# robo-alex/gs-dynamics

Measured on AMD Instinct MI355X. Metric: fwd+bwd Mpix/s at 100k Gaussians, 4x800^2 views, higher is better.
Workload: dtype f32

## Files before the change

### gs-dynamics_amd/csrc/gsr_api.hip

```cpp
#include <atomic>
#include <chrono>
#include <sched.h>
#include <stdarg.h>
#include <stdio.h>
#include <string.h>
#include <vector>
#include "gsr_common.h"

static thread_local char g_err[512] = "";

namespace {
struct ProfRec { const char* name; hipEvent_t a, b; };
bool g_prof_on = false;
std::vector<ProfRec> g_prof;
}
#include <dlfcn.h>
namespace {
typedef int (*roctx_push_fn)(const char*);
typedef int (*roctx_pop_fn)(void);
roctx_push_fn g_roctx_push = nullptr;
roctx_pop_fn g_roctx_pop = nullptr;
bool roctx_ready() {
  static const bool ok = [] {
    const char* e = getenv("GSR_ROCTX");
    if (e && *e && atoi(e) == 0) return false;
    for (const char* lib : {"librocprofiler-sdk-roctx.so", "librocprofiler-sdk-roctx.so.1", "libroctx64.so", "libroctx64.so.4"}) {
      void* h = dlopen(lib, RTLD_LAZY | RTLD_GLOBAL);
      if (!h) continue;
      g_roctx_push = (roctx_push_fn)dlsym(h, "roctxRangePushA");
      g_roctx_pop = (roctx_pop_fn)dlsym(h, "roctxRangePop");
      if (g_roctx_push && g_roctx_pop) return true;
    }
    return false;
  }();
  return ok;
}
}
GsrRange::GsrRange(const char* name) : on(roctx_ready()) { if (on) g_roctx_push(name); }
GsrRange::~GsrRange() { if (on) g_roctx_pop(); }

GsrProfScope::GsrProfScope(const char* name, hipStream_t s) : slot(-1), st(s), range(name) {
  if (!g_prof_on) return;
  ProfRec r; r.name = name;
  if (hipEventCreate(&r.a) != hipSuccess || hipEventCreate(&r.b) != hipSuccess) return;
  (void)hipEventRecord(r.a, st);
  g_prof.push_back(r);
  slot = (int)g_prof.size() - 1;
}
GsrProfScope::~GsrProfScope() {
  if (slot >= 0) (void)hipEventRecord(g_prof[slot].b, st);
}

void gsr_set_error(const char* fmt, ...) {
  va_list ap;
  va_start(ap, fmt);
  vsnprintf(g_err, sizeof g_err, fmt, ap);
  va_end(ap);
}

static int make_cam(const gsr_settings* s, GsrCam* c) {
  if (!s) { gsr_set_error("gsr: settings is NULL"); return -2; }
  if (s->image_height <= 0 || s->image_width <= 0) { gsr_set_error("gsr: image size must be positive"); return -2; }
  if (!s->bg || !s->viewmatrix || !s->projmatrix || !s->campos) {
    gsr_set_error("gsr: bg/viewmatrix/projmatrix/campos must be device pointers");
    return -2;
  }
  c->H = s->image_height; c->W = s->image_width;
  c->gx = (c->W + GSR_TILE - 1) / GSR_TILE; c->gy = (c->H + GSR_TILE - 1) / GSR_TILE;
  c->T = c->gx * c->gy;
  if (c->gx > 65535 || c->gy > 65535) { gsr_set_error("gsr: image too large (tile grid exceeds 65535)"); return -2; }
  c->tanfovx = s->tanfovx; c->tanfovy = s->tanfovy; c->scale_modifier = s->scale_modifier;
  c->sh_degree = s->sh_degree; c->M = s->sh_coeffs;
  c->bg = s->bg; c->view = s->viewmatrix; c->proj = s->projmatrix; c->campos = s->campos;
  if (s->prefiltered & ~(int32_t)(1 | GSR_SETTINGS_ANTIALIASING)) {
    gsr_set_error("gsr: unknown bits 0x%x in settings.prefiltered (bit 0: prefiltered, bit 1: GSR_SETTINGS_ANTIALIASING)", (unsigned)s->prefiltered);
    return -2;
  }
  c->antialiasing = (s->prefiltered & GSR_SETTINGS_ANTIALIASING) ? 1 : 0;
  return 0;
}

extern "C" {

int gsr_version(void) { return GSR_VERSION; }
const char* gsr_last_error(void) { return g_err; }

size_t gsr_geom_bytes(int32_t P) { GeomState g; return gsr_carve_geom(nullptr, P, &g); }
size_t gsr_image_bytes(int32_t H, int32_t W) { ImageState im; return gsr_carve_image(nullptr, H, W, &im); }
size_t gsr_binning_bytes(uint32_t D, int32_t, int32_t) { BinningState b; return gsr_carve_binning(nullptr, D, &b); }
size_t gsr_backward_scratch_bytes(int32_t, uint32_t D) { return gsr_align((size_t)(D ? D : 1) * GSR_PARTIAL_FLOATS * 4); }
size_t gsr_backward_scratch_bytes_depth(int32_t, uint32_t D) { return gsr_depth_scratch_offset(D) + gsr_align((size_t)(D ? D : 1) * 4); }

}
namespace {
void fill_pre_view(GsrPreView& o, const GsrCam& cam, const GeomState& g, int32_t* radii, uint32_t* block_sums,
                   const float* colors) {
  o.colors = colors;
  o.view = cam.view; o.proj = cam.proj; o.campos = cam.campos; o.tanfovx = cam.tanfovx; o.tanfovy = cam.tanfovy;
  o.rec = g.rec; o.rect = g.rect; o.tiles_touched = g.tiles_touched; o.clamped = g.clamped; o.radii = radii;
  o.block_sums = block_sums; o.ekey = g.ekey; o.block_hash = nullptr; o.cmp_rec = nullptr; o.cmp_rect = nullptr; o.cmp_ekey = nullptr; o.cmp_tiles = nullptr; o.skip = 0;
  o.used = g.used; o.tracked = g.counters + 1;
}

struct ArmedCuts { int V = 0; const uint32_t* in[GSR_MAX_BATCH]; uint32_t* out[GSR_MAX_BATCH]; uint32_t* redo = nullptr; float margin = 1.0f; };
thread_local ArmedCuts t_cuts;
void fill_bin_view(GsrBinView& o, int P, uint32_t D, const GeomState& g, const BinningState& bs, const ImageState& im,
                   const uint32_t* block_sums) {
  o.shares_lists = 0; o.fused_alias = 0; o.D_dev = nullptr; o.owner = 0;
  o.ekey = g.ekey; o.rec_w = g.rec; o.tile_rows = nullptr; o.depth_cut = nullptr;
  o.rec = g.rec; o.rect = g.rect; o.tiles_touched = g.tiles_touched; o.block_sums = block_sums;
  o.block_offsets = gsr_host_block_scan(P) ? nullptr : g.block_offsets;
  o.offsets = g.offsets;
  o.tkey[0] = bs.tkey[0]; o.tkey[1] = bs.tkey[1]; o.dg[0] = bs.dg[0]; o.dg[1] = bs.dg[1];
  o.point_list = bs.point_list; o.block_hist = bs.block_hist; o.ranges = im.ranges;
  o.D = D; o.nblocks = D ? gsr_radix_blocks(D) : 0u;
}
void fill_render_view(GsrRenderView& o, const GsrCam& cam, const GeomState& g, const BinningState& bs, const ImageState& im,
                      float* out_color, float* out_depth, const float* dL_dcolor, float4* partials) {
  o.point_list = bs.point_list; o.rec = g.rec; o.bg = cam.bg; o.final_T = im.final_T; o.n_contrib = im.n_contrib;
  o.out_color = out_color; o.out_depth = out_depth; o.dL_dcolor = dL_dcolor; o.rect = g.rect; o.offsets = g.offsets;
  o.partials = partials; o.ranges = im.ranges; o.dL_dalpha = nullptr; o.partner = -1; o.fused_alias = 0; o.colors = nullptr; o.contrib = bs.contrib;
  o.used = g.used; o.tracked = g.counters + 1;
  o.cut_in = nullptr; o.cut_out = nullptr; o.redo = nullptr; o.cut_margin = 1.0f;
}

void pair_up(int V, const int32_t* geometry_of, const uint32_t* num_rendered, int partner[GSR_MAX_BATCH], int fused[GSR_MAX_BATCH]) {
  static const bool off = [] { const char* e = getenv("GSR_NO_PAIR_FUSION"); return e && *e && atoi(e) != 0; }();
  for (int v = 0; v < V; ++v) { partner[v] = -1; fused[v] = 0; }
  if (!geometry_of || off) return;
  for (int v = 0; v < V; ++v) {
    const int u = geometry_of[v];
    if (u != v && partner[u] < 0 && num_rendered[u] > 0) { partner[u] = v; fused[v] = 1; }
  }
}
void skippable_aliases(int V, const int32_t* geometry_of, const float* const* colors_views, int flags, int skip[GSR_MAX_BATCH]) {
  static const bool off = [] { const char* e = getenv("GSR_NO_PAIR_FUSION"); return e && *e && atoi(e) != 0; }();
  int taken[GSR_MAX_BATCH];
  for (int v = 0; v < V; ++v) { skip[v] = 0; taken[v] = 0; }
  if (!geometry_of || !colors_views || off || !(flags & GSR_FORWARD_ONLY)) return;
  for (int v = 0; v < V; ++v) {
    const int u = geometry_of[v];
    if (u != v && !taken[u]) { taken[u] = 1; skip[v] = 1; }
  }
}
void render_header(GsrRenderViews& t, int V, const GsrCam& cam, const uint4* order, uint32_t* queue) {
  t.V = V; t.W = cam.W; t.H = cam.H; t.gx = cam.gx; t.T = cam.T; t.order = order; t.queue = queue; t.no_colour_grad = 0; t.prio_frac256 = 0; t.pc_error_out = nullptr; t.track = 1; t.avg_list = 1u << 20;
}

uint32_t* pinned_sums() {
  static thread_local uint32_t* p = nullptr;
  if (!p && hipHostMalloc((void**)&p, sizeof(uint32_t) * 2 * GSR_MAX_BATCH * GSR_HOST_SCAN_MAX_BLOCKS, hipHostMallocMapped | hipHostMallocCoherent) != hipSuccess)
    p = nullptr;
  return p;
}

int check_inputs(const char* who, const float* means3D, const float* opacities, const float* colors_precomp, const float* shs,
                 const float* scales, const float* rotations, const float* cov3D_precomp, const GsrCam& cam) {
  if (!means3D || !opacities) { gsr_set_error("%s: NULL argument", who); return -2; }
  if ((colors_precomp == nullptr) == (shs == nullptr)) {
    gsr_set_error("%s: provide exactly one of colors_precomp / shs", who);
    return -2;
  }
  if (((scales == nullptr) || (rotations == nullptr)) == (cov3D_precomp == nullptr)) {
    gsr_set_error("%s: provide exactly one of scales+rotations / cov3D_precomp", who);
    return -2;
  }
  if (shs && (cam.M < (cam.sh_degree + 1) * (cam.sh_degree + 1) || cam.sh_degree > 3 || cam.sh_degree < 0 || cam.M > 16)) {
    gsr_set_error("%s: sh_degree %d needs (deg+1)^2 <= sh_coeffs (%d) <= 16", who, cam.sh_degree, cam.M);
    return -2;
  }
  return 0;
}

int stage1(int V, const gsr_settings* s, int32_t P, const float* means3D, const float* scales, const float* rotations,
           const float* opacities, const float* colors_precomp, const float* const* colors_views, const float* shs,
           const float* cov3D_precomp, void* const* geom_states, int32_t* const* radii, uint32_t* sums,
           uint32_t* num_rendered_host, hipStream_t st, const gsr_raw_params* raw = nullptr, int32_t* same_host = nullptr,
           const int* skip = nullptr, const int32_t* geometry_of = nullptr, const void* prev_geom = nullptr,
           uint32_t* differs_pinned = nullptr) {
  if (colors_views) {
    if (shs || colors_precomp) { gsr_set_error("gsr forward: per-view colours exclude colors_precomp / shs"); return -2; }
    for (int v = 0; v < V; ++v) if (!colors_views[v]) { gsr_set_error("gsr forward: NULL per-view colour pointer"); return -2; }
    colors_precomp = colors_views[0];
  }
  GsrPreViews tab;
  tab.V = V;
  tab.raw_rot = tab.raw_op = tab.raw_sc = nullptr;
  tab.rot_out = tab.op_out = tab.sc_out = nullptr;
  if (raw) {
    if (!raw->unnorm_rotations || !raw->logit_opacities || !raw->log_scales || !raw->rotations_out || !raw->opacities_out || !raw->scales_out ||
        raw->rotations_out != rotations || raw->opacities_out != opacities || raw->scales_out != scales || cov3D_precomp) {
      gsr_set_error("gsr forward (raw parameters): NULL pointer, cov3D_precomp given, or rotations / opacities / scales are not the *_out buffers");
      return -2;
    }
    tab.raw_rot = raw->unnorm_rotations; tab.raw_op = raw->logit_opacities; tab.raw_sc = raw->log_scales;
    tab.rot_out = raw->rotations_out; tab.op_out = raw->opacities_out; tab.sc_out = raw->scales_out;
  }
  GsrCam cam0;
  const uint32_t nblk = (uint32_t)((P + GSR_BLOCK - 1) / GSR_BLOCK);
  for (int v = 0; v < V; ++v) {
    GsrCam cam;
    if (int rc = make_cam(&s[v], &cam)) return rc;
    if (v == 0) {
      cam0 = cam;
      if (int rc = check_inputs("gsr forward", means3D, opacities, colors_precomp, shs, scales, rotations, cov3D_precomp, cam)) return rc;
    } else if (cam.W != cam0.W || cam.H != cam0.H || cam.sh_degree != cam0.sh_degree || cam.M != cam0.M ||
               cam.scale_modifier != cam0.scale_modifier) {
      gsr_set_error("gsr batch: all views must share image size, sh_degree and scale_modifier");
      return -2;
    }
    if (!geom_states[v] || !radii[v]) { gsr_set_error("gsr forward: NULL geom_state / radii"); return -2; }
    GeomState g;
    gsr_carve_geom(geom_states[v], P, &g);
    fill_pre_view(tab.v[v], cam, g, radii[v], sums + (size_t)v * nblk, colors_views ? colors_views[v] : nullptr);
    uint32_t* own_words = (num_rendered_host && gsr_host_block_scan(P) && !(skip && skip[v])) ? pinned_sums() : nullptr;
    if (differs_pinned && V == 1 && gsr_host_block_scan(P)) tab.v[v].block_hash = reinterpret_cast<uint2*>(differs_pinned);
    else if (own_words) {
      uint32_t* w = own_words + (size_t)v * 2 * GSR_HOST_SCAN_MAX_BLOCKS;
      for (uint32_t b = 0; b < nblk; ++b) w[2 * b + 1] = 0xffffffffu;
      tab.v[v].block_hash = reinterpret_cast<uint2*>(w);
    }
    if (V == 1 && tab.v[v].block_hash && (differs_pinned || same_host) && prev_geom) {
      {
        GeomState pg;
        gsr_carve_geom(const_cast<void*>(prev_geom), P, &pg);
        tab.v[v].cmp_rec = pg.rec; tab.v[v].cmp_rect = pg.rect; tab.v[v].cmp_ekey = pg.ekey; tab.v[v].cmp_tiles = pg.tiles_touched;
      }
    }
    if (skip && skip[v]) tab.v[v].skip = 1;
  }
  if (int rc = gsr_launch_preprocess(tab, cam0, P, means3D, scales, rotations, opacities, colors_precomp, shs, cov3D_precomp, st))
    return rc;
  if (!num_rendered_host) {
    if (!gsr_host_block_scan(P))
      for (int v = 0; v < V; ++v) {
        GeomState g;
        gsr_carve_geom(geom_states[v], P, &g);
        if (int rc = gsr_launch_scan_exclusive(sums + (size_t)v * nblk, g.block_offsets, nblk, g.counters, st)) return rc;
      }
    return 0;
  }
  uint32_t* host = pinned_sums();
  if (!host) { gsr_set_error("gsr forward: pinned host allocation failed"); return -1; }
  if (same_host) *same_host = 0;
  if (gsr_host_block_scan(P)) {
    for (int v = 0; v < V; ++v) {
      uint64_t tot = 0;
      if (skip && skip[v]) {
        tot = num_rendered_host[geometry_of[v]];
      } else {
        const volatile uint32_t* w = host + (size_t)v * 2 * GSR_HOST_SCAN_MAX_BLOCKS;
        int32_t any = 1;
        int64_t got = gsr_wait_block_counts(w, (int32_t)nblk, 2000, 30ll * 1000 * 1000, &any);
        if (got < 0) {
          GSR_HIP_CHECK(hipStreamSynchronize(st));
          got = gsr_wait_block_counts(w, (int32_t)nblk, 0, 1000, &any);
          if (got < 0) { gsr_set_error("gsr forward: the preprocess kernel's per-block counts never reached the host"); return -1; }
        }
        tot = (uint64_t)got;
        if (v == 0 && same_host && tab.v[0].cmp_rec) *same_host = any ? 0 : 1;
      }
      if (tot > 0xffffffffull) { gsr_set_error("gsr forward: %llu tile entries overflow 32 bits", (unsigned long long)tot); return -3; }
      num_rendered_host[v] = (uint32_t)tot;
    }
  } else {
    for (int v = 0; v < V; ++v) {
      GeomState g;
      gsr_carve_geom(geom_states[v], P, &g);
      if (int rc = gsr_launch_scan_exclusive(sums + (size_t)v * nblk, g.block_offsets, nblk, g.counters, st)) return rc;
      GSR_HIP_CHECK(hipMemcpyAsync(host + v, g.counters, sizeof(uint32_t), hipMemcpyDeviceToHost, st));
    }
    GSR_HIP_CHECK(hipStreamSynchronize(st));
    for (int v = 0; v < V; ++v) num_rendered_host[v] = (skip && skip[v]) ? host[geometry_of[v]] : host[v];
  }
  return 0;
}

int check_geometry_of(int V, const int32_t* geometry_of) {
  if (!geometry_of) return 0;
  for (int v = 0; v < V; ++v) {
    const int u = geometry_of[v];
    if (u < 0 || u > v || geometry_of[u] != u) { gsr_set_error("gsr batch: geometry_of[%d] = %d is not an earlier primary view", v, u); return -2; }
  }
  return 0;
}
int stage2(int V, const gsr_settings* s, int32_t P, const uint32_t* num_rendered, void* const* geom_states,
           void* const* binning_states, void* const* image_states, float* const* out_color, float* const* out_depth,
           const uint32_t* sums, uint4* order, uint32_t* queue, const int32_t* geometry_of, hipStream_t st,
           uint32_t* counts_dev = nullptr, uint32_t* tile_rows = nullptr, int flags = 0, const float* const* colors_views = nullptr) {
  if (int rc = check_geometry_of(V, geometry_of)) return rc;
  GsrBinViews bt;
  bt.vlong_out = nullptr; bt.vlong_launch = 0;
  bt.cut_lds = 0;
  GsrRenderViews rt;
  int partner[GSR_MAX_BATCH], fused[GSR_MAX_BATCH], skip[GSR_MAX_BATCH];
  pair_up(V, geometry_of, num_rendered, partner, fused);
  skippable_aliases(V, geometry_of, colors_views, flags, skip);
  const uint32_t nblk = (uint32_t)(((P > 0 ? P : 1) + GSR_BLOCK - 1) / GSR_BLOCK);
  for (int v = 0; v < V; ++v) {
    GsrCam cam;
    if (int rc = make_cam(&s[v], &cam)) return rc;
    if (!image_states[v] || !out_color[v] || !out_depth[v]) { gsr_set_error("gsr forward render: NULL argument"); return -2; }
    const int owner = geometry_of ? geometry_of[v] : v;
    if (num_rendered[v] > 0 && (!geom_states[v] || !binning_states[owner])) { gsr_set_error("gsr forward render: NULL state"); return -2; }
    if (owner != v && num_rendered[owner] != num_rendered[v]) { gsr_set_error("gsr batch: view %d shares view %d's camera but not its entry count", v, owner); return -2; }
    GeomState g; ImageState im, im_owner; BinningState bs;
    gsr_carve_geom(geom_states[v], P, &g);
    gsr_carve_image(image_states[v], cam.H, cam.W, &im);
    gsr_carve_image(image_states[owner], cam.H, cam.W, &im_owner);
    gsr_carve_binning(binning_states[owner], num_rendered[owner], &bs);
    if (v == 0) {
      bt.V = V; bt.T = cam.T; bt.gx = cam.gx; bt.counts_out = counts_dev; bt.P = P;
      bt.rows = tile_rows ? gsr_bin_rows(P) : 0;
      bt.forward_only = (flags & GSR_FORWARD_ONLY) ? 1 : 0;
      bt.order = order ? order : im.tile_order;
      bt.queue = queue ? queue : im.queue;
      render_header(rt, V, cam, bt.order, bt.queue);
    } else if (cam.W != rt.W || cam.H != rt.H) {
      gsr_set_error("gsr batch: all views must share the image size");
      return -2;
    }
    fill_bin_view(bt.v[v], P, num_rendered[v], g, bs, im, sums ? sums + (size_t)v * nblk : g.block_sums);
    if (tile_rows) bt.v[v].tile_rows = tile_rows + (size_t)v * (gsr_bin_rows(P) + 1) * (size_t)gsr_bin_stride(cam.T);
    bt.v[v].owner = owner;
    fill_render_view(rt.v[v], cam, g, bs, im, out_color[v], out_depth[v], nullptr, nullptr);
    if (owner != v) {
      bt.v[v].shares_lists = 1; bt.v[v].D = 0; bt.v[v].nblocks = 0; bt.v[v].ranges = im_owner.ranges;
      rt.v[v].ranges = im_owner.ranges;
    }
    bt.v[v].fused_alias = (uint32_t)fused[v];
    rt.v[v].partner = partner[v]; rt.v[v].fused_alias = fused[v];
    if (skip[v]) {
      if (!fused[v] && num_rendered[v] > 0) { gsr_set_error("gsr batch: view %d was not preprocessed but is not fused", v); return -2; }
      rt.v[v].colors = colors_views[v];
    }
    if (counts_dev && owner == v) bt.v[v].D_dev = g.offsets + P;
  }
  if (t_cuts.V) {
    const ArmedCuts ac = t_cuts;
    t_cuts.V = 0;
    if (ac.V != V || !(flags & GSR_FORWARD_ONLY) || !tile_rows) {
      gsr_set_error("gsr_arm_depth_cuts: the armed cuts need a forward-only call of %d views on the tile-row binning path", ac.V);
      return -2;
    }
    for (int v = 0; v < V; ++v) {
      if (bt.v[v].shares_lists || rt.v[v].partner >= 0 || rt.v[v].fused_alias) { gsr_set_error("gsr_arm_depth_cuts: views that share tile lists cannot be cut"); return -2; }
      bt.v[v].depth_cut = ac.in[v];
      rt.v[v].cut_in = ac.in[v]; rt.v[v].cut_out = ac.out[v]; rt.v[v].redo = ac.redo ? ac.redo + v : nullptr; rt.v[v].cut_margin = ac.margin;
    }
  }
  if (int rc = gsr_launch_binning(bt, P, st)) return rc;
  rt.track = (flags & GSR_FORWARD_ONLY) ? 0 : 1;
  return gsr_launch_render_fwd(rt, st);
}
}
extern "C" {

int gsr_forward_preprocess(const gsr_settings* s, int32_t P, const float* means3D, const float* scales,
                           const float* rotations, const float* opacities, const float* colors_precomp,
                           const float* shs, const float* cov3D_precomp, void* geom_state, int32_t* radii,
                           uint32_t* num_rendered_host, void* stream) {
  return gsr_forward_preprocess_same(s, P, means3D, scales, rotations, opacities, colors_precomp, shs, cov3D_precomp, geom_state, radii,
                                     num_rendered_host, nullptr, nullptr, stream);
}

int gsr_forward_preprocess_same(const gsr_settings* s, int32_t P, const float* means3D, const float* scales,
                                const float* rotations, const float* opacities, const float* colors_precomp,
                                const float* shs, const float* cov3D_precomp, void* geom_state, int32_t* radii,
                                uint32_t* num_rendered_host, const void* prev_geom_state, int32_t* same_host, void* stream) {
  GsrRange _range("gsr_forward_preprocess");
  if (same_host) *same_host = 0;
  GsrCam cam;
  if (int rc = make_cam(s, &cam)) return rc;
  if (num_rendered_host) *num_rendered_host = 0;
  if (P <= 0) return 0;
  if (!geom_state || !radii) { gsr_set_error("gsr_forward_preprocess: NULL argument"); return -2; }
  if (prev_geom_state == geom_state) { gsr_set_error("gsr_forward_preprocess_same: a forward cannot be compared with the state it writes"); return -2; }
  GeomState g;
  gsr_carve_geom(geom_state, P, &g);
  uint32_t D = 0;
  if (int rc = stage1(1, s, P, means3D, scales, rotations, opacities, colors_precomp, nullptr, shs, cov3D_precomp, &geom_state,
                      &radii, g.block_sums, &D, (hipStream_t)stream, nullptr, same_host, nullptr, nullptr, prev_geom_state))
    return rc;
  if (num_rendered_host) *num_rendered_host = D;
  return 0;
}

int gsr_forward_render(const gsr_settings* s, int32_t P, uint32_t num_rendered, const void* geom_state,
                       void* binning_state, void* image_state, float* out_color, float* out_depth, void* stream) {
  return gsr_forward_render_ex(s, P, num_rendered, geom_state, binning_state, image_state, out_color, out_depth, 0u, stream);
}
int gsr_forward_render_ex(const gsr_settings* s, int32_t P, uint32_t num_rendered, const void* geom_state, void* binning_state,
                          void* image_state, float* out_color, float* out_depth, uint32_t flags, void* stream) {
  GsrRange _range("gsr_forward_render");
  if (!s) { gsr_set_error("gsr: settings is NULL"); return -2; }
  void* geom = const_cast<void*>(geom_state);
  GeomState g;
  gsr_carve_geom(geom, P, &g);
  GsrCam cam;
  if (int rc = make_cam(s, &cam)) return rc;
  return stage2(1, s, P, &num_rendered, &geom, &binning_state, &image_state, &out_color, &out_depth, nullptr, nullptr,
                nullptr, nullptr, (hipStream_t)stream, nullptr, (geom && P > 0 && gsr_rows_path_ok(cam.T)) ? g.tile_rows : nullptr,
                (int)(flags & GSR_FORWARD_ONLY));
}

int gsr_forward_capacity(const gsr_settings* s, int32_t P, const float* means3D, const float* scales, const float* rotations,
                         const float* opacities, const float* colors_precomp, const float* shs, const float* cov3D_precomp,
                         void* geom_state, int32_t* radii, void* binning_state, uint32_t capacity_entries, void* image_state,
                         float* out_color, float* out_depth, const void* prev_geom_state, uint32_t* block_words_pinned,
                         int32_t* count_pinned, uint32_t flags, void* stream) {
  GsrRange _range("gsr_forward_capacity");
  GsrCam cam;
  if (int rc = make_cam(s, &cam)) return rc;
  if (P <= 0) { gsr_set_error("gsr_forward_capacity: P must be positive (use gsr_forward_preprocess / gsr_forward_render)"); return -2; }
  if (!geom_state || !radii || !binning_state || !image_state || !out_color || !out_depth || capacity_entries == 0) {
    gsr_set_error("gsr_forward_capacity: NULL argument or no capacity");
    return -2;
  }
  if (block_words_pinned && (reinterpret_cast<uintptr_t>(block_words_pinned) & 7u)) {
    gsr_set_error("gsr_forward_capacity: block_words_pinned must be 8-byte aligned (every block stores its word pair with one 8-byte store)");
    return -2;
  }
  const bool words = block_words_pinned && gsr_host_block_scan(P);
  if (!count_pinned && !words) { gsr_set_error("gsr_forward_capacity: count_pinned is needed (no block_words_pinned, or P > 512 Ki)"); return -2; }
  if (prev_geom_state == geom_state) { gsr_set_error("gsr_forward_capacity: a forward cannot be compared with the state it writes"); return -2; }
  GeomState g;
  gsr_carve_geom(geom_state, P, &g);
  if (int rc = stage1(1, s, P, means3D, scales, rotations, opacities, colors_precomp, nullptr, shs, cov3D_precomp, &geom_state, &radii,
                      g.block_sums, nullptr, (hipStream_t)stream, nullptr, nullptr, nullptr, nullptr,
                      words ? prev_geom_state : nullptr, words ? block_words_pinned : nullptr))
    return rc;
  uint32_t* late_count = count_pinned ? reinterpret_cast<uint32_t*>(count_pinned) : g.counters + 8;
  return stage2(1, s, P, &capacity_entries, &geom_state, &binning_state, &image_state, &out_color, &out_depth, nullptr, nullptr, nullptr,
                nullptr, (hipStream_t)stream, late_count, gsr_rows_path_ok(cam.T) ? g.tile_rows : nullptr, (int)(flags & GSR_FORWARD_ONLY));
}

int gsr_forward_render_shared_ex(const gsr_settings* s, int32_t P, uint32_t num_rendered, void* geom_state, void* owner_binning_state,
                                 const void* owner_image_state, void* image_state, float* out_color, float* out_depth, uint32_t flags,
                                 void* stream) {
  GsrRange _range("gsr_forward_render_shared");
  GsrCam cam;
  if (int rc = make_cam(s, &cam)) return rc;
  if (P <= 0 || num_rendered == 0 || !geom_state || !owner_binning_state || !owner_image_state || !image_state || !out_color || !out_depth) {
    gsr_set_error("gsr_forward_render_shared: NULL argument, or nothing rendered (use gsr_forward_render)");
    return -2;
  }
  hipStream_t st = (hipStream_t)stream;
  GeomState g; ImageState im, im_owner; BinningState bs;
  gsr_carve_geom(geom_state, P, &g);
  gsr_carve_image(image_state, cam.H, cam.W, &im);
  gsr_carve_image(const_cast<void*>(owner_image_state), cam.H, cam.W, &im_owner);
  gsr_carve_binning(const_cast<void*>(owner_binning_state), num_rendered, &bs);
  GsrBinViews bt;
  bt.vlong_out = nullptr; bt.vlong_launch = 0;
  bt.V = 1; bt.T = cam.T; bt.gx = cam.gx; bt.counts_out = nullptr; bt.P = P; bt.rows = 0; bt.forward_only = 0; bt.wave_cap = 512; bt.cut_lds = 0;
  bt.order = im.tile_order; bt.queue = im.queue;
  fill_bin_view(bt.v[0], P, num_rendered, g, bs, im, g.block_sums);
  if (int rc = gsr_launch_shared_lists(bt, P, num_rendered, im_owner.ranges, im_owner.tile_order, im_owner.queue, im.ranges, im.tile_order,
                                       im.queue, st))
    return rc;
  GsrRenderViews rt;
  render_header(rt, 1, cam, im.tile_order, im.queue);
  rt.track = (flags & GSR_FORWARD_ONLY) ? 0 : 1;
  fill_render_view(rt.v[0], cam, g, bs, im, out_color, out_depth, nullptr, nullptr);
  return gsr_launch_render_fwd(rt, st);
}

}
static void camera_header(GsrCamViews& cv, int V, int32_t P, const GsrCam& cam, const uint32_t* bwd_error, const float* means3D,
                          const float* scales, const float* rotations, const float* cov3D_precomp, const float* shs) {
  cv.V = V; cv.P = P; cv.nblk = gsr_camera_blocks(P, cam.H, cam.W); cv.sh_degree = cam.sh_degree; cv.M = cam.M;
  cv.mod = cam.scale_modifier; cv.bwd_error = bwd_error;
  cv.means3D = means3D; cv.scales = scales; cv.rotations = rotations; cv.cov3D = cov3D_precomp; cv.shs = shs;
}
static void camera_view(GsrCamView& w, const GsrCam& cam, const gsr_camera_grads& cg, double* slab, const int32_t* radii, const GeomState* g,
                        const float4* partials, const float* dL_dz, const float* final_T, const uint32_t* clamped, uint32_t cap,
                        const float* dL_dcolor) {
  w.view = cam.view; w.proj = cam.proj; w.campos = cam.campos;
  w.radii = radii; w.used = g ? g->used : nullptr; w.tracked = g ? g->counters + 1 : nullptr; w.offsets = g ? g->offsets : nullptr;
  w.partials = partials; w.dL_dz = dL_dz; w.rec = g ? g->rec : nullptr; w.clamped = clamped;
  w.final_T = final_T; w.dL_dcolor = cg.dL_dbg ? dL_dcolor : nullptr; w.slab = slab;
  w.out_view = cg.dL_dviewmatrix; w.out_proj = cg.dL_dprojmatrix; w.out_campos = cg.dL_dcampos; w.out_bg = cg.dL_dbg;
  w.cap = cap; w.W = cam.W; w.H = cam.H; w.tanfovx = cam.tanfovx; w.tanfovy = cam.tanfovy;
}
extern "C" size_t gsr_camera_scratch_bytes(int32_t V, int32_t P, int32_t H, int32_t W) {
  return gsr_align((size_t)(V > 0 ? V : 1) * (size_t)gsr_camera_blocks(P, H, W) * GSR_CAM_ROW * sizeof(double));
}

static int check_batch(const char* who, int32_t V, const gsr_settings* s, const void* batch_state) {
  if (V <= 0 || V > GSR_MAX_BATCH) { gsr_set_error("%s: V must be in 1..%d", who, GSR_MAX_BATCH); return -2; }
  if (!s || !batch_state) { gsr_set_error("%s: NULL settings / batch_state", who); return -2; }
  for (int v = 1; v < V; ++v)
    if ((s[v].prefiltered & GSR_SETTINGS_ANTIALIASING) != (s[0].prefiltered & GSR_SETTINGS_ANTIALIASING)) {
      gsr_set_error("%s: view %d's GSR_SETTINGS_ANTIALIASING differs from view 0's: all views of a call must agree", who, v);
      return -2;
    }
  return 0;
}

static const gsr_backward_extras kNoExtras = {};
static int backward_one(const gsr_settings* s, int32_t P, uint32_t num_rendered, const float* means3D,
                        const float* scales, const float* rotations, const float* colors_precomp, const float* shs,
                        const float* cov3D_precomp, const int32_t* radii, const void* geom_state,
                        const void* binning_state, const void* image_state, const float* dL_dcolor, void* scratch,
                        float* dL_dmeans3D, float* dL_dmeans2D, float* dL_dcolors, float* dL_dopacity,
                        float* dL_dscales, float* dL_drotations, float* dL_dcov3D, float* dL_dsh, const gsr_backward_extras& ex,
                        void* stream) {
  GsrRange _range(ex.cam ? "gsr_backward_cam" : (ex.dL_ddepth ? "gsr_backward_depth" : (ex.dL_dalpha ? "gsr_backward_alpha" : "gsr_backward")));
  GsrCam cam;
  if (int rc = make_cam(s, &cam)) return rc;
  hipStream_t st = (hipStream_t)stream;
  if (ex.cam && (!ex.cam_scratch || !dL_dcolor)) { gsr_set_error("gsr_backward (camera gradients): NULL cam_scratch / dL_dcolor"); return -2; }
  if (P <= 0) {
    if (!ex.cam) return 0;
    GsrCamViews cv;
    camera_header(cv, 1, 0, cam, nullptr, nullptr, nullptr, nullptr, nullptr, nullptr);
    camera_view(cv.v[0], cam, *ex.cam, (double*)ex.cam_scratch, nullptr, nullptr, nullptr, nullptr, nullptr, nullptr, 0, dL_dcolor);
    return gsr_launch_camera_bwd(cv, false, st);
  }
  if (!means3D || !radii || !geom_state || !image_state || !dL_dcolor || !dL_dmeans3D || !dL_dmeans2D || !dL_dopacity) {
    gsr_set_error("gsr_backward: NULL argument");
    return -2;
  }
  if (num_rendered > 0 && (!binning_state || !scratch)) { gsr_set_error("gsr_backward: NULL binning/scratch"); return -2; }
  GeomState g; ImageState im; BinningState bs;
  gsr_carve_geom(const_cast<void*>(geom_state), P, &g);
  gsr_carve_image(const_cast<void*>(image_state), cam.H, cam.W, &im);
  gsr_carve_binning(const_cast<void*>(binning_state), num_rendered, &bs);
  float4* partials = (float4*)scratch;
  float* dL_dz = (ex.dL_ddepth && num_rendered > 0) ? (float*)((char*)scratch + gsr_depth_scratch_offset(num_rendered)) : nullptr;
  if (num_rendered > 0) {
    GsrRenderViews rt;
    render_header(rt, 1, cam, im.tile_order, im.queue);
    rt.no_colour_grad = (!shs && !dL_dcolors) ? 1 : 0;
    rt.avg_list = num_rendered / (uint32_t)(cam.T > 0 ? cam.T : 1);
    fill_render_view(rt.v[0], cam, g, bs, im, nullptr, nullptr, dL_dcolor, partials);
    rt.v[0].dL_dalpha = ex.dL_dalpha;
    GsrDepthViews dv;
    if (dL_dz) { dv.dL_ddepth[0] = ex.dL_ddepth; dv.dL_dz[0] = dL_dz; }
    if (int rc = gsr_launch_render_bwd(rt, st, dL_dz ? &dv : nullptr)) return rc;
  }
  const uint32_t* bwd_error = num_rendered > 0 ? im.queue + GSR_QUEUE_BWD_ERROR : nullptr;
  if (int rc = gsr_launch_preprocess_bwd(cam, P, means3D, scales, rotations, colors_precomp, shs, cov3D_precomp, radii, g,
                                         partials, dL_dmeans3D, dL_dmeans2D, dL_dcolors, dL_dopacity, dL_dscales,
                                         dL_drotations, dL_dcov3D, dL_dsh, bwd_error, st, dL_dz))
    return rc;
  if (!ex.cam) return 0;
  GsrCamViews cv;
  camera_header(cv, 1, P, cam, bwd_error, means3D, scales, rotations, cov3D_precomp, shs);
  camera_view(cv.v[0], cam, *ex.cam, (double*)ex.cam_scratch, radii, &g, partials, dL_dz, im.final_T, g.clamped, num_rendered, dL_dcolor);
  return gsr_launch_camera_bwd(cv, cam.antialiasing != 0, st);
}

static const gsr_backward_batch_extras kNoBatchExtras = {};
static int backward_batch(int32_t V, const gsr_settings* s, int32_t P, const uint32_t* num_rendered, const float* means3D,
                          const float* scales, const float* rotations, const float* colors_precomp,
                          const float* cov3D_precomp, const int32_t* const* radii, void* const* geom_states,
                          void* const* binning_states, void* const* image_states, void* batch_state,
                          const int32_t* geometry_of, const float* const* dL_dcolor, void* const* scratch, float* dL_dmeans3D,
                          float* const* dL_dmeans2D, float* dL_dcolors, float* const* dL_dcolors_views, float* dL_dopacity,
                          float* dL_dscales, float* dL_drotations, float* dL_dcov3D, const gsr_backward_batch_extras& ex,
                          void* stream) {
  GsrRange _range(ex.cams ? "gsr_backward_batch_cam" : (ex.dL_ddepth_views ? "gsr_backward_batch_depth"
                                                                     : (ex.dL_dalpha_views ? "gsr_backward_batch_alpha" : "gsr_backward_batch")));
  if (int rc = check_batch("gsr_backward_batch", V, s, batch_state)) return rc;
  if (ex.cams && (!ex.cam_scratch || ex.raw)) { gsr_set_error("gsr_backward_batch (camera gradients): NULL cam_scratch, or raw parameters"); return -2; }
  if (ex.raw && (ex.dL_ddepth_views || ex.dL_dalpha_views)) {
    gsr_set_error("gsr_backward_batch (raw parameters): a depth / alpha gradient table cannot be combined with raw parameters");
    return -2;
  }
  if (int rc = check_geometry_of(V, geometry_of)) return rc;
  if (!num_rendered || !radii || !geom_states || !binning_states || !image_states || !dL_dcolor || !scratch ||
      !dL_dmeans3D || !dL_dmeans2D || (!dL_dopacity && !ex.raw) || !means3D) {
    gsr_set_error("gsr_backward_batch: NULL argument");
    return -2;
  }
  if (ex.raw && (!ex.raw->unnorm_rotations || !ex.raw->d_unnorm_rotations || !ex.raw->d_logit_opacities || !ex.raw->d_log_scales || !scales || !rotations ||
              !ex.raw->opacities_out || cov3D_precomp)) {
    gsr_set_error("gsr_backward_batch (raw parameters): NULL pointer or cov3D_precomp given");
    return -2;
  }
  if (P <= 0) {
// ... 22 lines not shown
  GsrRenderViews rt;
  GsrBinViews bt;
  bt.vlong_out = nullptr; bt.vlong_launch = 0;
  bt.cut_lds = 0;
  bool any = false;
  int partner[GSR_MAX_BATCH], fused[GSR_MAX_BATCH];
  pair_up(V, geometry_of, num_rendered, partner, fused);
  bool pairs_fwd = false;
  for (int v = 0; v < V; ++v) pairs_fwd = pairs_fwd || fused[v];
  bool depth = false;
  for (int v = 0; ex.dL_ddepth_views && v < V; ++v) depth = depth || ex.dL_ddepth_views[v] != nullptr;
  GsrDepthViews dv;
  GsrAaViews av;
  const bool aa = (s[0].prefiltered & GSR_SETTINGS_ANTIALIASING) != 0;
  const bool fuse_bwd = pairs_fwd && !dL_dcolors && !dL_dcolors_views && !depth && !ex.cams;
  if (!fuse_bwd)
    for (int v = 0; v < V; ++v) { partner[v] = -1; fused[v] = 0; }
  for (int v = 0; v < V; ++v) {
    GsrCam cam;
    if (int rc = make_cam(&s[v], &cam)) return rc;
    const int owner = geometry_of ? geometry_of[v] : v;
    GeomState g; ImageState im, im_owner; BinningState bs;
    gsr_carve_geom(geom_states[v], P, &g);
    gsr_carve_image(image_states[v], cam.H, cam.W, &im);
    gsr_carve_image(image_states[owner], cam.H, cam.W, &im_owner);
    gsr_carve_binning(binning_states[owner], num_rendered[owner], &bs);
    if (num_rendered[v] > 0 && (!binning_states[owner] || !scratch[v])) { gsr_set_error("gsr_backward_batch: NULL binning/scratch"); return -2; }
    if (v == 0) { render_header(rt, V, cam, b.order, b.queue); rt.no_colour_grad = (!dL_dcolors && !dL_dcolors_views) ? 1 : 0; }
    fill_render_view(rt.v[v], cam, g, bs, im, nullptr, nullptr, dL_dcolor[v], (float4*)scratch[v]);
    rt.v[v].ranges = im_owner.ranges;
    rt.v[v].dL_dalpha = ex.dL_dalpha_views ? ex.dL_dalpha_views[v] : nullptr;
    rt.v[v].partner = partner[v]; rt.v[v].fused_alias = fused[v];
    if (v == 0) { bt.V = V; bt.T = cam.T; bt.gx = cam.gx; bt.order = b.order; bt.queue = b.queue; bt.counts_out = nullptr; bt.P = P; bt.wave_cap = 512; bt.rows = 0; bt.forward_only = 0; }
    bt.v[v].ranges = im_owner.ranges; bt.v[v].fused_alias = (uint32_t)fused[v]; bt.v[v].shares_lists = owner != v;
    any = any || num_rendered[v] > 0;
    GsrBwdView& w = vw.v[v];
    w.view = cam.view; w.proj = cam.proj; w.radii = radii[v]; w.offsets = g.offsets;
    w.used = g.used; w.tracked = g.counters + 1;
    w.partials = (const float4*)scratch[v]; w.dL_dmeans2D = dL_dmeans2D[v];
    w.dL_dcolors = dL_dcolors_views ? dL_dcolors_views[v] : nullptr;
    w.partner_dL_dmeans2D = partner[v] >= 0 ? dL_dmeans2D[partner[v]] : nullptr;
    w.fused_alias = fused[v];
    w.cap = num_rendered[v];
    w.W = cam.W; w.H = cam.H; w.tanfovx = cam.tanfovx; w.tanfovy = cam.tanfovy;
    av.rec[v] = g.rec;
    if (depth) {
      dv.dL_ddepth[v] = ex.dL_ddepth_views[v];
      dv.dL_dz[v] = num_rendered[v] > 0 ? (float*)((char*)scratch[v] + gsr_depth_scratch_offset(num_rendered[v])) : nullptr;
    }
  }
  GsrDepthViews dvp = dv;
  for (int v = 0; depth && v < V; ++v) if (!dv.dL_ddepth[v]) dvp.dL_dz[v] = nullptr;
  if (any) {
    { uint64_t tot = 0; for (int v = 0; v < V; ++v) tot += num_rendered[v]; rt.avg_list = (uint32_t)(tot / ((uint64_t)V * (uint64_t)(rt.T > 0 ? rt.T : 1))); }
    const bool rebuild = pairs_fwd && !fuse_bwd;
    if (rebuild)
      if (int rc = gsr_launch_tile_order(bt, st)) return rc;
    if (int rc = gsr_launch_render_bwd(rt, st, depth ? &dv : nullptr)) return rc;
    vw.bwd_error = rt.queue + GSR_QUEUE_BWD_ERROR;
    if (rebuild) {
      pair_up(V, geometry_of, num_rendered, partner, fused);
      for (int v = 0; v < V; ++v) bt.v[v].fused_alias = (uint32_t)fused[v];
      if (int rc = gsr_launch_tile_order(bt, st)) return rc;
    }
  }
  (void)colors_precomp;
  if (int rc = gsr_launch_preprocess_bwd_views(vw, P, s[0].scale_modifier, means3D, scales, rotations, cov3D_precomp, dL_dmeans3D,
                                               dL_dcolors, dL_dopacity, dL_dscales, dL_drotations, dL_dcov3D, st,
                                               (depth && any) ? &dvp : nullptr, aa ? &av : nullptr))
    return rc;
  if (!ex.cams) return 0;
  GsrCamViews cv;
  GsrCam cam0;
  if (int rc = make_cam(&s[0], &cam0)) return rc;
  camera_header(cv, V, P, cam0, vw.bwd_error, means3D, scales, rotations, cov3D_precomp, nullptr);
  double* slab = (double*)ex.cam_scratch;
  for (int v = 0; v < V; ++v) {
    GsrCam cam;
    if (int rc = make_cam(&s[v], &cam)) return rc;
    GeomState g; ImageState im;
    gsr_carve_geom(geom_states[v], P, &g);
    gsr_carve_image(image_states[v], cam.H, cam.W, &im);
    camera_view(cv.v[v], cam, ex.cams[v], slab + (size_t)v * cv.nblk * GSR_CAM_ROW, radii[v], &g, vw.v[v].partials,
                depth ? dvp.dL_dz[v] : nullptr, im.final_T, nullptr, num_rendered[v], dL_dcolor[v]);
  }
  return gsr_launch_camera_bwd(cv, aa, st);
}

extern "C" {
int gsr_backward_ex(const gsr_settings* s, int32_t P, uint32_t num_rendered, const float* means3D,
                    const float* scales, const float* rotations, const float* colors_precomp, const float* shs,
                    const float* cov3D_precomp, const int32_t* radii, const void* geom_state,
                    const void* binning_state, const void* image_state, const float* dL_dcolor, void* scratch,
                    float* dL_dmeans3D, float* dL_dmeans2D, float* dL_dcolors, float* dL_dopacity,
                    float* dL_dscales, float* dL_drotations, float* dL_dcov3D, float* dL_dsh, const gsr_backward_extras* ex,
                    void* stream) {
  return backward_one(s, P, num_rendered, means3D, scales, rotations, colors_precomp, shs, cov3D_precomp, radii, geom_state, binning_state,
                      image_state, dL_dcolor, scratch, dL_dmeans3D, dL_dmeans2D, dL_dcolors, dL_dopacity, dL_dscales, dL_drotations,
                      dL_dcov3D, dL_dsh, ex ? *ex : kNoExtras, stream);
}
int gsr_backward(const gsr_settings* s, int32_t P, uint32_t num_rendered, const float* means3D,
                 const float* scales, const float* rotations, const float* colors_precomp, const float* shs,
                 const float* cov3D_precomp, const int32_t* radii, const void* geom_state,
                 const void* binning_state, const void* image_state, const float* dL_dcolor, void* scratch,
                 float* dL_dmeans3D, float* dL_dmeans2D, float* dL_dcolors, float* dL_dopacity,
                 float* dL_dscales, float* dL_drotations, float* dL_dcov3D, float* dL_dsh, void* stream) {
  return gsr_backward_ex(s, P, num_rendered, means3D, scales, rotations, colors_precomp, shs, cov3D_precomp, radii, geom_state, binning_state,
                         image_state, dL_dcolor, scratch, dL_dmeans3D, dL_dmeans2D, dL_dcolors, dL_dopacity, dL_dscales, dL_drotations,
                         dL_dcov3D, dL_dsh, nullptr, stream);
}
int gsr_alpha_views(int32_t V, int32_t H, int32_t W, void* const* image_states, float* out_alpha, void* stream) {
  GsrRange _range("gsr_alpha_views");
  if (V <= 0 || V > GSR_MAX_BATCH || H <= 0 || W <= 0) { gsr_set_error("gsr_alpha_views: V must be in 1..%d and H, W positive", GSR_MAX_BATCH); return -2; }
  if (!image_states || !out_alpha) { gsr_set_error("gsr_alpha_views: NULL argument"); return -2; }
  GsrAlphaViews tab;
  tab.V = V; tab.N = H * W;
  for (int v = 0; v < V; ++v) {
    if (!image_states[v]) { gsr_set_error("gsr_alpha_views: NULL image state"); return -2; }
    ImageState im;
    gsr_carve_image(image_states[v], H, W, &im);
    tab.final_T[v] = im.final_T;
    tab.out[v] = out_alpha + (size_t)v * H * W;
  }
  return gsr_launch_alpha(tab, (hipStream_t)stream);
}

size_t gsr_batch_state_bytes(int32_t V, int32_t P, int32_t H, int32_t W) { BatchState b; return gsr_carve_batch(nullptr, V, P, H, W, &b); }


int gsr_arm_depth_cuts(int32_t V, const uint32_t* const* cut_in, uint32_t* const* cut_out, uint32_t* redo_flags, float margin) {
  if (V == 0) { t_cuts.V = 0; return 0; }
  if (V < 1 || V > GSR_MAX_BATCH || !cut_out || !redo_flags || !(margin >= 1.0f) || !(margin < 1e6f)) { gsr_set_error("gsr_arm_depth_cuts: bad argument (margin >= 1)"); return -2; }
  t_cuts.V = V; t_cuts.redo = redo_flags; t_cuts.margin = margin;
  for (int v = 0; v < V; ++v) {
    if (!cut_out[v]) { t_cuts.V = 0; gsr_set_error("gsr_arm_depth_cuts: cut_out[%d] is NULL", v); return -2; }
    t_cuts.in[v] = cut_in ? cut_in[v] : nullptr;
    t_cuts.out[v] = cut_out[v];
  }
  return 0;
}
int gsr_forward_preprocess_batch(int32_t V, const gsr_settings* s, int32_t P, const float* means3D, const float* scales,
                                 const float* rotations, const float* opacities, const float* colors_precomp,
                                 const float* const* colors_views, const float* shs, const float* cov3D_precomp,
                                 void* const* geom_states,
                                 int32_t* const* radii, void* batch_state, uint32_t* num_rendered_host, void* stream) {
  GsrRange _range("gsr_forward_preprocess_batch");
  if (int rc = check_batch("gsr_forward_preprocess_batch", V, s, batch_state)) return rc;
  if (!geom_states || !radii || !num_rendered_host) { gsr_set_error("gsr_forward_preprocess_batch: NULL argument"); return -2; }
  for (int v = 0; v < V; ++v) num_rendered_host[v] = 0;
  if (P <= 0) return 0;
  BatchState b;
  gsr_carve_batch(batch_state, V, P, s[0].image_height, s[0].image_width, &b);
  return stage1(V, s, P, means3D, scales, rotations, opacities, colors_precomp, colors_views, shs, cov3D_precomp, geom_states,
                radii, b.sums, num_rendered_host, (hipStream_t)stream);
}

int gsr_forward_render_batch(int32_t V, const gsr_settings* s, int32_t P, const uint32_t* num_rendered,
                             void* const* geom_states, void* const* binning_states, void* const* image_states,
                             void* batch_state, const int32_t* geometry_of, const float* const* colors_views, float* const* out_color,
                             float* const* out_depth, int32_t flags, void* stream) {
  GsrRange _range("gsr_forward_render_batch");
  if (int rc = check_batch("gsr_forward_render_batch", V, s, batch_state)) return rc;
  if (!num_rendered || !geom_states || !binning_states || !image_states || !out_color || !out_depth) {
    gsr_set_error("gsr_forward_render_batch: NULL argument");
    return -2;
  }
  BatchState b;
  gsr_carve_batch(batch_state, V, P, s[0].image_height, s[0].image_width, &b);
  return stage2(V, s, P, num_rendered, geom_states, binning_states, image_states, out_color, out_depth, b.sums, b.order,
                b.queue, geometry_of, (hipStream_t)stream, nullptr, b.tile_rows, flags, colors_views);
}

int gsr_forward_batch(int32_t V, const gsr_settings* s, int32_t P, const float* means3D, const float* scales,
                      const float* rotations, const float* opacities, const float* colors_precomp,
                      const float* const* colors_views, const float* shs, const float* cov3D_precomp,
                      void* const* geom_states, int32_t* const* radii,
                      void* const* binning_states, const size_t* binning_bytes, void* const* image_states,
                      void* batch_state, const int32_t* geometry_of, float* const* out_color, float* const* out_depth,
                      uint32_t* num_rendered_host, int32_t flags, void* stream) {
  GsrRange _range("gsr_forward_batch");
  if (int rc = check_batch("gsr_forward_batch", V, s, batch_state)) return rc;
  if (int rc = check_geometry_of(V, geometry_of)) return rc;
  if (!geom_states || !radii || !num_rendered_host || !image_states || !out_color || !out_depth) {
    gsr_set_error("gsr_forward_batch: NULL argument");
    return -2;
  }
  for (int v = 0; v < V; ++v) num_rendered_host[v] = 0;
  if (P <= 0) return 1;
  BatchState b;
  gsr_carve_batch(batch_state, V, P, s[0].image_height, s[0].image_width, &b);
  int skip[GSR_MAX_BATCH];
  skippable_aliases(V, geometry_of, colors_views, flags, skip);
  if (int rc = stage1(V, s, P, means3D, scales, rotations, opacities, colors_precomp, colors_views, shs, cov3D_precomp,
                      geom_states, radii, b.sums, num_rendered_host, (hipStream_t)stream, nullptr, nullptr, skip, geometry_of))
    return rc;
  bool fits = binning_states != nullptr && binning_bytes != nullptr;
  for (int v = 0; fits && v < V; ++v) {
    if (geometry_of && geometry_of[v] != v) continue;
    fits = num_rendered_host[v] == 0 || (binning_states[v] && binning_bytes[v] >= gsr_binning_bytes(num_rendered_host[v], 0, 0));
  }
  if (!fits) return 1;
  return stage2(V, s, P, num_rendered_host, geom_states, binning_states, image_states, out_color, out_depth, b.sums, b.order,
                b.queue, geometry_of, (hipStream_t)stream, nullptr, b.tile_rows, flags, colors_views);
}

int gsr_forward_batch_capacity_raw(int32_t V, const gsr_settings* s, int32_t P, const float* means3D, const float* scales,
                                   const float* rotations, const float* opacities, const float* colors_precomp,
                                   const float* const* colors_views, const float* shs, const float* cov3D_precomp,
                                   void* const* geom_states, int32_t* const* radii, void* const* binning_states,
                                   const uint32_t* capacity_entries, void* const* image_states, void* batch_state,
                                   const int32_t* geometry_of, float* const* out_color, float* const* out_depth,
                                   uint32_t* counts_dev, const gsr_raw_params* raw, void* stream) {
  GsrRange _range("gsr_forward_batch_capacity");
  if (int rc = check_batch("gsr_forward_batch_capacity", V, s, batch_state)) return rc;
  if (int rc = check_geometry_of(V, geometry_of)) return rc;
  if (!geom_states || !radii || !binning_states || !capacity_entries || !image_states || !out_color || !out_depth || !counts_dev) {
    gsr_set_error("gsr_forward_batch_capacity: NULL argument");
    return -2;
  }
  if (P <= 0) { gsr_set_error("gsr_forward_batch_capacity: P must be positive (use gsr_forward_batch)"); return -2; }
  for (int v = 0; v < V; ++v) {
    const bool owner = !geometry_of || geometry_of[v] == v;
    if (capacity_entries[v] == 0 || (owner && !binning_states[v])) { gsr_set_error("gsr_forward_batch_capacity: view %d has no capacity / binning state", v); return -2; }
    if (!owner && capacity_entries[v] != capacity_entries[geometry_of[v]]) { gsr_set_error("gsr_forward_batch_capacity: view %d must have its owner's capacity", v); return -2; }
  }
  BatchState b;
  gsr_carve_batch(batch_state, V, P, s[0].image_height, s[0].image_width, &b);
  if (int rc = stage1(V, s, P, means3D, scales, rotations, opacities, colors_precomp, colors_views, shs, cov3D_precomp,
                      geom_states, radii, b.sums, nullptr, (hipStream_t)stream, raw, nullptr, nullptr, geometry_of))
    return rc;
  return stage2(V, s, P, capacity_entries, geom_states, binning_states, image_states, out_color, out_depth, b.sums, b.order,
                b.queue, geometry_of, (hipStream_t)stream, counts_dev, b.tile_rows);
}

int gsr_backward_batch_ex(int32_t V, const gsr_settings* s, int32_t P, const uint32_t* num_rendered, const float* means3D,
                          const float* scales, const float* rotations, const float* colors_precomp,
                          const float* cov3D_precomp, const int32_t* const* radii, void* const* geom_states,
                          void* const* binning_states, void* const* image_states, void* batch_state,
                          const int32_t* geometry_of, const float* const* dL_dcolor, void* const* scratch, float* dL_dmeans3D,
                          float* const* dL_dmeans2D, float* dL_dcolors, float* const* dL_dcolors_views, float* dL_dopacity,
                          float* dL_dscales, float* dL_drotations, float* dL_dcov3D, const gsr_backward_batch_extras* ex,
                          void* stream) {
  return backward_batch(V, s, P, num_rendered, means3D, scales, rotations, colors_precomp, cov3D_precomp, radii, geom_states,
                        binning_states, image_states, batch_state, geometry_of, dL_dcolor, scratch, dL_dmeans3D, dL_dmeans2D, dL_dcolors,
                        dL_dcolors_views, dL_dopacity, dL_dscales, dL_drotations, dL_dcov3D, ex ? *ex : kNoBatchExtras, stream);
}
int gsr_backward_batch(int32_t V, const gsr_settings* s, int32_t P, const uint32_t* num_rendered, const float* means3D,
                       const float* scales, const float* rotations, const float* colors_precomp,
                       const float* cov3D_precomp, const int32_t* const* radii, void* const* geom_states,
                       void* const* binning_states, void* const* image_states, void* batch_state,
                       const int32_t* geometry_of, const float* const* dL_dcolor, void* const* scratch, float* dL_dmeans3D,
                       float* const* dL_dmeans2D, float* dL_dcolors, float* const* dL_dcolors_views, float* dL_dopacity,
                       float* dL_dscales, float* dL_drotations, float* dL_dcov3D, void* stream) {
  return gsr_backward_batch_ex(V, s, P, num_rendered, means3D, scales, rotations, colors_precomp, cov3D_precomp, radii, geom_states,
                               binning_states, image_states, batch_state, geometry_of, dL_dcolor, scratch, dL_dmeans3D, dL_dmeans2D,
                               dL_dcolors, dL_dcolors_views, dL_dopacity, dL_dscales, dL_drotations, dL_dcov3D, nullptr, stream);
}

int gsr_sh_backward_views(int32_t V, const gsr_settings* s, int32_t P, const float* means3D, const float* shs,
                          const int32_t* const* radii, void* const* geom_states,
                          const float* const* dL_dcolors_views, float* dL_dsh, float* dL_dmeans3D, void* stream) {
  GsrRange _range("gsr_sh_backward_views");
  if (V <= 0 || V > GSR_MAX_BATCH) { gsr_set_error("gsr_sh_backward_views: V must be in 1..%d", GSR_MAX_BATCH); return -2; }
  if (!s) { gsr_set_error("gsr_sh_backward_views: NULL settings"); return -2; }
  const int deg = s[0].sh_degree, M = s[0].sh_coeffs;
  if (deg < 0 || deg > 3 || M < (deg + 1) * (deg + 1) || M > 16) {
    gsr_set_error("gsr_sh_backward_views: sh_degree %d needs (deg+1)^2 <= sh_coeffs (%d) <= 16", deg, M);
    return -2;
  }
  for (int v = 1; v < V; ++v)
    if (s[v].sh_degree != deg || s[v].sh_coeffs != M) {
      gsr_set_error("gsr_sh_backward_views: view %d's sh_degree / sh_coeffs differ from view 0's", v);
      return -2;
    }
  if (P <= 0) return 0;
  if (!means3D || !shs || !radii || !geom_states || !dL_dcolors_views || !dL_dsh || !dL_dmeans3D) {
    gsr_set_error("gsr_sh_backward_views: NULL argument");
    return -2;
  }
  GsrShViews t;
  t.V = V; t.P = P; t.M = M; t.deg = deg;
  t.vec4 = (((uintptr_t)shs | (uintptr_t)dL_dsh) & 15u) == 0 ? 1 : 0;
  t.means3D = means3D; t.shs = shs; t.dL_dsh = dL_dsh; t.dL_dmeans3D = dL_dmeans3D;
  for (int v = 0; v < V; ++v) {
    if (!radii[v] || !geom_states[v] || !dL_dcolors_views[v] || !s[v].campos) {
      gsr_set_error("gsr_sh_backward_views: NULL radii / geom_state / dL_dcolors_views / campos of view %d", v);
      return -2;
    }
    GeomState g;
    gsr_carve_geom(geom_states[v], P, &g);
    t.v[v].campos = s[v].campos; t.v[v].radii = radii[v]; t.v[v].clamped = g.clamped; t.v[v].dcol = dL_dcolors_views[v];
  }
  for (int v = V; v < GSR_MAX_BATCH; ++v) t.v[v] = GsrShView{nullptr, nullptr, nullptr, nullptr};
  return gsr_launch_sh_bwd_views(t, (hipStream_t)stream);
}

int32_t gsr_rigidity_blocks(int32_t n_fg) { return gsr_rigidity_fwd_blocks(n_fg); }

int gsr_rigidity_forward(int32_t n_fg, int32_t K, const float* means3D, const float* rotations, const int64_t* fg_idx,
                         const int64_t* neighbor_indices, const float* neighbor_weight, const float* neighbor_dist,
                         const float* prev_inv_rot_fg, const float* prev_offset, float* block_partials, void* stream) {
  GsrRange _range("gsr_rigidity_forward");
  if (n_fg < 0 || K <= 0 || (n_fg > 0 && (!means3D || !rotations || !fg_idx || !neighbor_indices || !neighbor_weight || !neighbor_dist ||
                                          !prev_inv_rot_fg || !prev_offset || !block_partials))) {
    gsr_set_error("gsr_rigidity_forward: bad argument");
    return -2;
  }
  return gsr_launch_rigidity_fwd(n_fg, K, means3D, rotations, fg_idx, neighbor_indices, neighbor_weight, neighbor_dist, prev_inv_rot_fg,
                                 prev_offset, nullptr, block_partials, (hipStream_t)stream);
}

int gsr_rigidity_backward(int32_t n_fg, int32_t K, const float* means3D, const float* rotations, const int64_t* fg_idx,
                          const int64_t* neighbor_indices, const float* neighbor_weight, const float* neighbor_dist,
                          const float* prev_inv_rot_fg, const float* prev_offset, const float* grad3, const int32_t* rev_ptr,
                          const int32_t* rev_edge, float* scratch, float* d_means3D, float* d_rotations, void* stream) {
  GsrRange _range("gsr_rigidity_backward");
  if (n_fg < 0 || K <= 0 || (n_fg > 0 && (!means3D || !rotations || !fg_idx || !neighbor_indices || !neighbor_weight || !neighbor_dist ||
                                          !prev_inv_rot_fg || !prev_offset || !grad3 || !rev_ptr || !rev_edge || !scratch || !d_means3D ||
                                          !d_rotations))) {
    gsr_set_error("gsr_rigidity_backward: bad argument");
    return -2;
  }
  float* self7 = scratch;
  float* edge7 = scratch + (size_t)7 * n_fg;
  return gsr_launch_rigidity_bwd(n_fg, K, means3D, rotations, fg_idx, neighbor_indices, neighbor_weight, neighbor_dist, prev_inv_rot_fg,
                                 prev_offset, grad3, 1, 1.0f, 1.0f, 1.0f, rev_ptr, rev_edge, nullptr, 0, self7, edge7, d_means3D, d_rotations, 0, (hipStream_t)stream);
}

int gsr_activate_forward(int32_t P, const float* unnorm_rotations, const float* logit_opacities, const float* log_scales,
                         float* rotations, float* opacities, float* scales, void* stream) {
  GsrRange _range("gsr_activate_forward");
  if (P < 0 || (P > 0 && (!unnorm_rotations || !logit_opacities || !log_scales || !rotations || !opacities || !scales))) {
    gsr_set_error("gsr_activate_forward: bad argument");
    return -2;
  }
  return gsr_launch_activate_fwd(P, unnorm_rotations, logit_opacities, log_scales, rotations, opacities, scales, (hipStream_t)stream);
}

int gsr_activate_backward(int32_t P, const float* unnorm_rotations, const float* opacities, const float* scales,
                          const float* d_rotations, const float* d_opacities, const float* d_scales, float* d_unnorm_rotations,
                          float* d_logit_opacities, float* d_log_scales, void* stream) {
  GsrRange _range("gsr_activate_backward");
  if (P < 0 || (P > 0 && (!unnorm_rotations || !opacities || !scales || !d_unnorm_rotations || !d_logit_opacities || !d_log_scales))) {
    gsr_set_error("gsr_activate_backward: bad argument");
    return -2;
  }
  return gsr_launch_activate_bwd(P, unnorm_rotations, opacities, scales, d_rotations, d_opacities, d_scales, d_unnorm_rotations,
                                 d_logit_opacities, d_log_scales, (hipStream_t)stream);
}

int32_t gsr_shared_terms_scratch(int32_t n_fg, int32_t K) {
  const int64_t n = n_fg > 0 ? n_fg : 0;
  return (int32_t)(16 * n + 8 * (n + n * (K > 0 ? K : 0)));
}

int32_t gsr_shared_terms_partials(int32_t n_fg, int32_t n_bg) {
  return 16 * (n_fg > 0 ? n_fg : 0) + 3 * (gsr_rigidity_fwd_blocks(n_fg) + gsr_shared_terms_point_blocks(n_fg, n_bg));
}

static int shared_terms_check(const char* who, int32_t n_fg, int32_t K, int32_t n_bg, const void* const* ptrs, int n) {
  if (n_fg < 0 || n_bg < 0 || K <= 0) { gsr_set_error("%s: bad sizes", who); return -2; }
  const unsigned fg_arrays = 1u << 2 | 1u << 4 | 1u << 5 | 1u << 6 | 1u << 7 | 1u << 8 | (n > 14 ? 1u << 14 : 0u);
  const unsigned bg_arrays = 1u << 3 | 1u << 9 | 1u << 10;
  for (int i = 0; i < n; ++i) {
    if ((n_fg == 0 && (fg_arrays >> i & 1u)) || (n_bg == 0 && (bg_arrays >> i & 1u))) continue;
    if (!ptrs[i]) { gsr_set_error("%s: NULL argument (#%d)", who, i); return -2; }
  }
  return 0;
}

int gsr_shared_terms_forward(int32_t n_fg, int32_t K, int32_t n_bg, const float* means3D, const float* rotations, const int64_t* fg_idx,
                             const int64_t* bg_idx, const int64_t* neighbor_indices, const float* neighbor_weight,
                             const float* neighbor_dist, const float* prev_inv_rot_fg, const float* prev_offset,
                             const float* init_bg_pts, const float* init_bg_rot, const float* weights5_host, float* partials,
                             float* terms6, void* stream) {
  GsrRange _range("gsr_shared_terms_forward");
  const void* ptrs[] = {means3D, rotations, fg_idx, bg_idx, neighbor_indices, neighbor_weight, neighbor_dist, prev_inv_rot_fg,
                        prev_offset, init_bg_pts, init_bg_rot, weights5_host, partials, terms6};
  if (int e = shared_terms_check("gsr_shared_terms_forward", n_fg, K, n_bg, ptrs, 14)) return e;
  return gsr_launch_shared_terms_fwd(n_fg, K, n_bg, means3D, rotations, fg_idx, bg_idx, neighbor_indices, neighbor_weight,
                                     neighbor_dist, prev_inv_rot_fg, prev_offset, init_bg_pts, init_bg_rot, weights5_host, partials,
                                     terms6, (hipStream_t)stream);
// ... 468 lines not shown
```

### gs-dynamics_amd/csrc/gsr_binning.hip

```cpp
#include "gsr_common.h"

namespace gsr_binning {

#define SCAN_THREADS 1024
#define SCAN_ITEMS 8
__global__ __launch_bounds__(SCAN_THREADS) void scan_exclusive_kernel(const uint32_t* __restrict__ in,
                                                                      uint32_t* __restrict__ out, uint32_t n,
                                                                      uint32_t* __restrict__ total_out) {
  __shared__ uint32_t wave_tot[SCAN_THREADS / GSR_WAVE];
  __shared__ uint32_t carry_s;
  const int tid = threadIdx.x, lane = tid & 63, wv = tid >> 6;
  if (tid == 0) carry_s = 0;
  __syncthreads();
  const uint32_t per_round = SCAN_THREADS * SCAN_ITEMS;
  for (uint32_t base = 0; base < n; base += per_round) {
    uint32_t v[SCAN_ITEMS];
    uint32_t first = base + (uint32_t)tid * SCAN_ITEMS;
    uint32_t sum = 0;
#pragma unroll
    for (int k = 0; k < SCAN_ITEMS; ++k) {
      uint32_t idx = first + k;
      v[k] = idx < n ? in[idx] : 0u;
      sum += v[k];
    }
    uint32_t inc = sum;
#pragma unroll
    for (int d = 1; d < 64; d <<= 1) {
      uint32_t o = __shfl_up(inc, d, 64);
      if (lane >= d) inc += o;
    }
    if (lane == 63) wave_tot[wv] = inc;
    __syncthreads();
    uint32_t wave_off = 0;
    for (int w = 0; w < wv; ++w) wave_off += wave_tot[w];
    uint32_t carry = carry_s;
    uint32_t run = carry + wave_off + inc - sum;
#pragma unroll
    for (int k = 0; k < SCAN_ITEMS; ++k) {
      uint32_t idx = first + k;
      if (idx < n) out[idx] = run;
      run += v[k];
    }
    __syncthreads();
    if (tid == SCAN_THREADS - 1) carry_s = run;
    __syncthreads();
  }
  if (tid == 0) {
    uint32_t tot = carry_s;
    out[n] = tot;
    if (total_out) *total_out = tot;
  }
}

__device__ __forceinline__ uint32_t bin_entries(const GsrBinView& vw) { return vw.D_dev ? min(vw.D_dev[0], vw.D) : vw.D; }
__device__ __forceinline__ uint32_t bin_blocks(const GsrBinView& vw, uint32_t D) {
  return vw.D_dev ? (D == 0 ? 1u : (D + GSR_RADIX_EPB - 1) / GSR_RADIX_EPB) : vw.nblocks;
}

#define EMIT_MAX_GBLOCKS GSR_HOST_SCAN_MAX_BLOCKS
#define EMIT_G (4 * GSR_BLOCK)
__global__ __launch_bounds__(GSR_BLOCK) void emit_entries_kernel(int P, GsrBinViews tab, int shift, int bits) {
  const GsrBinView& vw = tab.v[blockIdx.y];
  const int gx = tab.gx, T = tab.T;
  float4* __restrict__ rec = const_cast<float4*>(vw.rec);
  const uint2* __restrict__ rect = vw.rect;
  const uint32_t* __restrict__ tiles_touched = vw.tiles_touched;
  const uint32_t* __restrict__ block_sums = vw.block_sums;
  const uint32_t* __restrict__ block_offsets = vw.block_offsets;
  uint32_t* __restrict__ offsets = vw.offsets;
  uint32_t* __restrict__ tkey = vw.tkey[0];
  uint64_t* __restrict__ dg = vw.dg[0];
  uint2* __restrict__ ranges = vw.ranges;
  __shared__ uint32_t sS[EMIT_MAX_GBLOCKS + 1];
  __shared__ uint32_t soff[EMIT_G + 1];
  __shared__ uint32_t swave[GSR_BLOCK / GSR_WAVE];
  __shared__ uint32_t hist[256];
  const int tid = threadIdx.x, lane = tid & 63, wv = tid >> 6;
  const int nblk = (P + GSR_BLOCK - 1) / GSR_BLOCK;
  for (int t = (int)blockIdx.x * GSR_BLOCK + tid; t < T; t += (int)gridDim.x * GSR_BLOCK) ranges[t] = make_uint2(0xffffffffu, 0u);
  hist[tid] = 0;
  if (!block_offsets) {
    uint32_t v[8], sum = 0;
#pragma unroll
    for (int k = 0; k < 8; ++k) { const int j = tid * 8 + k; v[k] = j < nblk ? block_sums[j] : 0u; sum += v[k]; }
    uint32_t inc = sum;
#pragma unroll
    for (int d = 1; d < 64; d <<= 1) {
      const uint32_t o = __shfl_up(inc, d, 64);
      if (lane >= d) inc += o;
    }
    if (lane == 63) swave[wv] = inc;
    __syncthreads();
    uint32_t run = inc - sum;
    for (int w = 0; w < wv; ++w) run += swave[w];
#pragma unroll
    for (int k = 0; k < 8; ++k) { const int j = tid * 8 + k; if (j <= nblk) sS[j] = run; run += v[k]; }
    if (tid == GSR_BLOCK - 1) sS[8 * GSR_BLOCK] = run;
    __syncthreads();
  }
  auto S = [&](int j) -> uint32_t { return block_offsets ? block_offsets[j] : sS[j]; };
  const uint32_t D_total = S(nblk);
  if (blockIdx.x == 0 && tid == 0) offsets[P] = D_total;
  const uint32_t E0 = blockIdx.x * GSR_RADIX_EPB, Elim = E0 + GSR_RADIX_EPB;
  if (E0 > D_total) return;
  uint32_t E1 = min(D_total, Elim);
  if (vw.D_dev) E1 = min(E1, vw.D);
  int lo = 0, hi = nblk;
  while (lo < hi) { const int mid = (lo + hi) >> 1; if (S(mid + 1) >= E0) hi = mid; else lo = mid + 1; }
  const int jb0 = lo;
  lo = 0; hi = nblk;
  while (lo < hi) { const int mid = (lo + hi) >> 1; if (S(mid) >= Elim) hi = mid; else lo = mid + 1; }
  const int jb1 = lo - 1;
  const uint32_t mask = (1u << bits) - 1u;
  const int g_lo = jb0 * GSR_BLOCK, g_hi = min(P, (min(jb1, nblk - 1) + 1) * GSR_BLOCK);
  uint32_t chunk_base = S(jb0);
  for (int g0 = g_lo; g0 < g_hi; g0 += EMIT_G) {
    uint32_t mine[4], sum = 0;
#pragma unroll
    for (int q = 0; q < 4; ++q) { const int g = g0 + tid * 4 + q; mine[q] = g < g_hi ? tiles_touched[g] : 0u; sum += mine[q]; }
    uint32_t inc = sum;
#pragma unroll
    for (int d = 1; d < 64; d <<= 1) {
      const uint32_t o = __shfl_up(inc, d, 64);
      if (lane >= d) inc += o;
    }
    __syncthreads();
    if (lane == 63) swave[wv] = inc;
    __syncthreads();
    uint32_t run = chunk_base + inc - sum;
    for (int w = 0; w < wv; ++w) run += swave[w];
    const uint32_t chunk_total = swave[0] + swave[1] + swave[2] + swave[3];
#pragma unroll
    for (int q = 0; q < 4; ++q) {
      const int g = g0 + tid * 4 + q;
      soff[tid * 4 + q] = run;
      if (g < g_hi && run >= E0 && run < Elim) {
        offsets[g] = run;
        reinterpret_cast<uint32_t*>(rec + GSR_REC_F4 * (size_t)g + 3)[2] = run;
      }
      run += mine[q];
    }
    if (tid == GSR_BLOCK - 1) soff[EMIT_G] = run;
    __syncthreads();
    chunk_base += chunk_total;
    if (vw.shares_lists) continue;
    const uint32_t begin = max(soff[0], E0), end = min(soff[EMIT_G], E1);
    for (uint32_t e = begin + tid; e < end; e += GSR_BLOCK) {
      int l2 = 0, h2 = EMIT_G;
#pragma unroll
      for (int it = 0; it < 10; ++it) {
        const int mid = (l2 + h2) >> 1;
        if (soff[mid] <= e) l2 = mid; else h2 = mid;
      }
      const int g = g0 + l2;
      const uint32_t k = e - soff[l2];
      const uint2 r = rect[g];
      const uint32_t minx = r.x & 0xffffu, miny = r.x >> 16, maxx = r.y & 0xffffu, maxy = r.y >> 16;
      const uint32_t w = maxx - minx;
      uint32_t b = k;
      if (w * (maxy - miny) <= 32u) {
        uint32_t m = __float_as_uint(rec[GSR_REC_F4 * g + 3].w);
        for (uint32_t t = 0; t < k; ++t) m &= m - 1u;
        b = (uint32_t)__ffs((int)m) - 1u;
      }
      const uint32_t ty = miny + b / w, tx = minx + b % w;
      const uint32_t key = ty * (uint32_t)gx + tx;
      tkey[e] = key;
      dg[e] = ((uint64_t)__float_as_uint(rec[GSR_REC_F4 * g + 2].y) << 32) | (uint32_t)g;
      atomicAdd(&hist[(key >> shift) & mask], 1u);
    }
  }
  __syncthreads();
  if (!vw.shares_lists && E0 < E1 && tid < (1 << bits)) vw.block_hist[blockIdx.x * (uint32_t)(1 << bits) + tid] = hist[tid];
}

__device__ __forceinline__ uint64_t match_peers(uint32_t digit, bool valid, int bits) {
  uint64_t peers = __ballot(valid);
  for (int b = 0; b < bits; ++b) {
    const bool bit = (digit >> b) & 1u;
    const uint64_t m = __ballot(valid && bit);
    peers &= bit ? m : ~m;
  }
  return peers;
}

__global__ __launch_bounds__(GSR_BLOCK) void radix_hist_kernel(GsrBinViews tab, int cur, int shift, int bits) {
  const GsrBinView& vw = tab.v[blockIdx.y];
  if (vw.D == 0) return;
  const uint32_t D = bin_entries(vw);
  if (D == 0 || blockIdx.x >= bin_blocks(vw, D)) return;
  const uint32_t* __restrict__ tkey = vw.tkey[cur];
  uint32_t* __restrict__ block_hist = vw.block_hist;
  __shared__ uint32_t hist[256];
  const int tid = threadIdx.x;
  hist[tid] = 0;
  __syncthreads();
  const uint32_t mask = (1u << bits) - 1u;
  const uint32_t start = blockIdx.x * GSR_RADIX_EPB;
  const uint32_t stop = min(D, start + GSR_RADIX_EPB);
  uint32_t k[GSR_RADIX_ITEMS];
#pragma unroll
  for (int u = 0; u < GSR_RADIX_ITEMS; ++u) { const uint32_t i = start + (uint32_t)u * GSR_BLOCK + tid; k[u] = i < stop ? tkey[i] : 0u; }
#pragma unroll
  for (int u = 0; u < GSR_RADIX_ITEMS; ++u)
    if (start + (uint32_t)u * GSR_BLOCK + tid < stop) atomicAdd(&hist[(k[u] >> shift) & mask], 1u);
  __syncthreads();
  if (tid < (1 << bits)) block_hist[blockIdx.x * (uint32_t)(1 << bits) + tid] = hist[tid];
}

// ... 37 lines not shown
  if (D == 0 || blockIdx.x >= nblocks) return;
  const uint32_t* __restrict__ tkey_in = vw.tkey[cur];
  const uint64_t* __restrict__ dg_in = vw.dg[cur];
  uint32_t* __restrict__ tkey_out = vw.tkey[cur ^ 1];
  uint64_t* __restrict__ dg_out = vw.dg[cur ^ 1];
  const uint32_t* __restrict__ block_hist = vw.block_hist;
  __shared__ uint32_t wcount[4][256];
  __shared__ uint32_t s_tot[4][256];
  __shared__ uint32_t s_pre[4][256];
  __shared__ uint32_t s_binbase[256];
  __shared__ uint32_t s_local[256];
  __shared__ uint32_t s_delta[256];
  __shared__ uint32_t s_key[GSR_RADIX_EPB];
  __shared__ uint64_t s_pay[GSR_RADIX_EPB];
  volatile uint32_t(*wbase)[256] = wcount;
  const int tid = threadIdx.x, lane = tid & 63, wv = tid >> 6;
  const uint32_t mask = (1u << bits) - 1u;
  const int nb = 1 << bits;
  for (int i = tid; i < 4 * 256; i += GSR_BLOCK) (&wcount[0][0])[i] = 0;
  const uint32_t chunk0 = blockIdx.x * GSR_RADIX_EPB;
  constexpr uint32_t per_wave = GSR_RADIX_EPB / 4;
  constexpr int STEPS = per_wave / 64;
  const uint32_t wstart = chunk0 + wv * per_wave;
  const uint32_t wstop = min(D, wstart + per_wave);
  uint32_t key[STEPS];
  uint64_t pay[STEPS];
#pragma unroll
  for (int k = 0; k < STEPS; ++k) {
    const uint32_t i = wstart + (uint32_t)k * 64u + lane;
    key[k] = 0; pay[k] = 0;
    if (i < wstop) { key[k] = tkey_in[i]; pay[k] = dg_in[i]; }
  }
  for (int bin = lane; bin < nb; bin += 64) {
    uint32_t tot = 0, pre = 0;
    uint32_t b = wv;
    if (prescanned) {
      if (wv == 0) { tot = block_hist[(size_t)nblocks * nb + bin]; pre = block_hist[(size_t)blockIdx.x * nb + bin]; }
      b = nblocks;
    }
    for (; b + 28 < nblocks; b += 32) {
      uint32_t v[8];
#pragma unroll
      for (int u = 0; u < 8; ++u) v[u] = block_hist[(b + 4 * u) * (uint32_t)nb + bin];
#pragma unroll
      for (int u = 0; u < 8; ++u) { tot += v[u]; pre += (b + 4 * u < blockIdx.x) ? v[u] : 0u; }
    }
    for (; b < nblocks; b += 4) {
      const uint32_t v = block_hist[b * (uint32_t)nb + bin];
      tot += v;
      pre += (b < blockIdx.x) ? v : 0u;
    }
    s_tot[wv][bin] = tot;
    s_pre[wv][bin] = pre;
  }
  __syncthreads();
  if (wv == 0) {
    uint32_t t4[4], sum = 0;
#pragma unroll
    for (int q = 0; q < 4; ++q) {
      const int bin = lane * 4 + q;
      t4[q] = bin < nb ? (s_tot[0][bin] + s_tot[1][bin] + s_tot[2][bin] + s_tot[3][bin]) : 0u;
      sum += t4[q];
    }
    uint32_t inc = sum;
#pragma unroll
    for (int d = 1; d < 64; d <<= 1) {
      const uint32_t o = __shfl_up(inc, d, 64);
      if (lane >= d) inc += o;
    }
    uint32_t run = inc - sum;
#pragma unroll
    for (int q = 0; q < 4; ++q) {
      const int bin = lane * 4 + q;
      if (bin < nb) s_binbase[bin] = run;
      run += t4[q];
    }
  }
#pragma unroll
  for (int k = 0; k < STEPS; ++k)
    if (wstart + (uint32_t)k * 64u + lane < wstop) atomicAdd(&wcount[wv][(key[k] >> shift) & mask], 1u);
  __syncthreads();
  if (wv == 0) {
    uint32_t t4[4], sum = 0;
#pragma unroll
    for (int q = 0; q < 4; ++q) {
      const int bin = lane * 4 + q;
      t4[q] = bin < nb ? (wcount[0][bin] + wcount[1][bin] + wcount[2][bin] + wcount[3][bin]) : 0u;
      sum += t4[q];
    }
    uint32_t inc = sum;
#pragma unroll
    for (int d = 1; d < 64; d <<= 1) {
      const uint32_t o = __shfl_up(inc, d, 64);
      if (lane >= d) inc += o;
    }
    uint32_t run = inc - sum;
#pragma unroll
    for (int q = 0; q < 4; ++q) {
      const int bin = lane * 4 + q;
      if (bin < nb) s_local[bin] = run;
      run += t4[q];
    }
  }
  __syncthreads();
  if (tid < nb) {
    const uint32_t gbase = s_binbase[tid] + s_pre[0][tid] + s_pre[1][tid] + s_pre[2][tid] + s_pre[3][tid];
    uint32_t lbase = s_local[tid];
    s_delta[tid] = gbase - lbase;
#pragma unroll
    for (int w = 0; w < 4; ++w) {
      const uint32_t c = wcount[w][tid];
      wcount[w][tid] = lbase;
      lbase += c;
    }
  }
  __syncthreads();
#pragma unroll
  for (int k = 0; k < STEPS; ++k) {
    const bool valid = wstart + (uint32_t)k * 64u + lane < wstop;
    const uint32_t digit = (key[k] >> shift) & mask;
    const uint64_t peers = match_peers(digit, valid, bits);
    const uint32_t rank = (uint32_t)__popcll(peers & gsr_lanemask_lt());
    uint32_t pos = 0;
    if (valid) pos = wbase[wv][digit] + rank;
    __builtin_amdgcn_wave_barrier();
    if (valid && rank == 0) wbase[wv][digit] = pos + (uint32_t)__popcll(peers);
    __builtin_amdgcn_wave_barrier();
    if (valid) { s_key[pos] = key[k]; s_pay[pos] = pay[k]; }
  }
  __syncthreads();
  const uint32_t nvalid = min(D, chunk0 + GSR_RADIX_EPB) - chunk0;
#pragma unroll
  for (int j = 0; j < GSR_RADIX_ITEMS; ++j) {
    const uint32_t l = (uint32_t)j * GSR_BLOCK + tid;
    if (l < nvalid) {
      const uint32_t kk = s_key[l];
      const uint32_t pos = l + s_delta[(kk >> shift) & mask];
      dg_out[pos] = s_pay[l];
      if (last_pass) {
        if (l == 0 || s_key[l - 1] != kk) atomicMin(&vw.ranges[kk].x, pos);
        if (l + 1 == nvalid || s_key[l + 1] != kk) atomicMax(&vw.ranges[kk].y, pos + 1u);
      } else {
        tkey_out[pos] = kk;
      }
    }
  }
}


#define GSR_COLSCAN_MIN_BLOCKS 768u
#define ORD_CHUNK 12
#define ORD_WAVES 16
#define ORD_MAX_WG 32
struct TileOrderLds {
  uint32_t h_before[ORD_WAVES][256];
  uint32_t h_rest[ORD_WAVES][256];
  uint32_t start[256];
  uint32_t empty_before_s, n_busy_s, n_long_s, n_empty_s;
};
__device__ __forceinline__ void tile_order_body(const GsrBinViews& tab, int items_per_wg, int bid, TileOrderLds& L) {
  auto& h_before = L.h_before; auto& h_rest = L.h_rest; auto& start = L.start;
  uint32_t& empty_before_s = L.empty_before_s; uint32_t& n_busy_s = L.n_busy_s; uint32_t& n_long_s = L.n_long_s; uint32_t& n_empty_s = L.n_empty_s;
  const int tid = threadIdx.x, lane = tid & 63, wv = tid >> 6;
  const int T = tab.T;
  uint4* __restrict__ tile_order = tab.order;
  uint32_t* __restrict__ queue = tab.queue;
  for (int i = tid; i < ORD_WAVES * 256; i += 1024) { (&h_before[0][0])[i] = 0; (&h_rest[0][0])[i] = 0; }
  if (tid == 0) { empty_before_s = 0; n_empty_s = 0; }
  if (bid == 0) {
    if (tid < 9) queue[tid] = 0;
    if (tab.counts_out && tid < tab.V)
      __hip_atomic_store(&tab.counts_out[tid], tab.v[tid].offsets[tab.P], __ATOMIC_RELAXED, __HIP_MEMORY_SCOPE_SYSTEM);
  }
  __syncthreads();
  const int n_it = (T + 1023) / 1024, n_items = tab.V * n_it;
  const int k_lo = bid * items_per_wg, k_hi = min(n_items, k_lo + items_per_wg);
  uint32_t empties_before = 0, empties_all = 0;
  for (int k0 = 0; k0 < n_items; k0 += ORD_CHUNK) {
    uint2 r[ORD_CHUNK];
    bool live[ORD_CHUNK];
#pragma unroll
    for (int u = 0; u < ORD_CHUNK; ++u) {
      const int k = k0 + u, t = (k % n_it) * 1024 + tid;
      r[u] = make_uint2(0u, 0u);
      live[u] = k < n_items && t < T && !tab.v[k / n_it].fused_alias;
      if (live[u]) r[u] = tab.v[k / n_it].ranges[t];
    }
#pragma unroll
    for (int u = 0; u < ORD_CHUNK; ++u) {
      const int k = k0 + u;
      const uint32_t len = r[u].y > r[u].x ? r[u].y - r[u].x : 0u;
      const uint32_t bucket = 255u - min((len + 7u) >> 3, 255u);
      if (bucket != 255u) atomicAdd(k < k_lo ? &h_before[wv][bucket] : &h_rest[wv][bucket], 1u);
      const uint32_t ne = (uint32_t)__popcll(__ballot(live[u] && bucket == 255u));
      empties_all += ne;
      if (k < k_lo) empties_before += ne;
    }
  }
  if (lane == 0) { atomicAdd(&empty_before_s, empties_before); atomicAdd(&n_empty_s, empties_all); }
  __syncthreads();
  uint32_t tot = 0, bef = 0;
  if (tid < 256) {
#pragma unroll
    for (int w = 0; w < ORD_WAVES; ++w) { bef += h_before[w][tid]; tot += h_rest[w][tid]; }
    tot += bef;
  }
  __syncthreads();
  if (tid < 256) { h_rest[0][tid] = tot; h_before[0][tid] = bef; }
  __syncthreads();
  if (tid < 64) {
    uint32_t c4[4], sum = 0;
#pragma unroll
    for (int q = 0; q < 4; ++q) { c4[q] = h_rest[0][lane * 4 + q]; sum += c4[q]; }
    uint32_t inc = sum;
#pragma unroll
    for (int d = 1; d < 64; d <<= 1) {
      const uint32_t o = __shfl_up(inc, d, 64);
      if (lane >= d) inc += o;
    }
    uint32_t run = inc - sum;
    uint32_t st4[4];
#pragma unroll
    for (int q = 0; q < 4; ++q) { st4[q] = run; run += c4[q]; }
    if (lane == 63) n_busy_s = run;
    if (bid == 0 && lane == 32) {
      queue[2] = st4[0];
      if (tab.vlong_out) __hip_atomic_store(tab.vlong_out, st4[0], __ATOMIC_RELAXED, __HIP_MEMORY_SCOPE_SYSTEM);
    }
    if (tab.wave_cap == 2048) {
      if (lane == 0) n_long_s = st4[0] + c4[0];
      if (bid == 0 && lane == 31) queue[3] = st4[0] + c4[0] + c4[1] + c4[2];
    } else if (lane == (tab.wave_cap == 1024 ? 31 : 47)) n_long_s = st4[0] + c4[0] + c4[1] + c4[2];
#pragma unroll
    for (int q = 0; q < 4; ++q) start[lane * 4 + q] = st4[q] + h_before[0][lane * 4 + q];
  }
  __syncthreads();
  const uint32_t n_busy = n_busy_s;
  if (tid == 0) start[255] = n_busy + empty_before_s;
  __syncthreads();
  for (int k0 = k_lo; k0 < k_hi; k0 += ORD_CHUNK) {
    uint2 r[ORD_CHUNK];
#pragma unroll
    for (int u = 0; u < ORD_CHUNK; ++u) {
      const int k = k0 + u, t = (k % n_it) * 1024 + tid;
      r[u] = make_uint2(0u, 0u);
      if (k < k_hi && t < T && !tab.v[k / n_it].fused_alias) r[u] = tab.v[k / n_it].ranges[t];
    }
#pragma unroll
    for (int u = 0; u < ORD_CHUNK; ++u) {
      const int k = k0 + u, t = (k % n_it) * 1024 + tid;
      if (k < k_hi && t < T && !tab.v[k / n_it].fused_alias) {
        if (r[u].y <= r[u].x) {
          r[u] = make_uint2(0u, 0u);
          if (!tab.v[k / n_it].shares_lists) tab.v[k / n_it].ranges[t] = r[u];
        }
        const uint32_t bucket = 255u - min((r[u].y - r[u].x + 7u) >> 3, 255u);
        uint32_t slot;
        if (bucket != 255u) slot = atomicAdd(&start[bucket], 1u);
        else {
          const uint64_t m = __ballot(1);
          const int leader = __ffsll((long long)m) - 1;
          uint32_t base = 0;
          if (lane == leader) base = atomicAdd(&start[255], (uint32_t)__popcll(m));
          base = __shfl(base, leader, 64);
          slot = base + (uint32_t)__popcll(m & gsr_lanemask_lt());
        }
        tile_order[slot] = make_uint4((uint32_t)t, r[u].x, r[u].y, (uint32_t)(k / n_it));
      }
    }
  }
  if (bid == 0 && tid == 0) { queue[4] = n_busy; queue[6] = n_long_s; queue[7] = n_busy + n_empty_s; }
}

__global__ __launch_bounds__(1024) void tile_order_kernel(GsrBinViews tab, int items_per_wg) {
  __shared__ TileOrderLds L;
  tile_order_body(tab, items_per_wg, (int)blockIdx.x, L);
}

__global__ __launch_bounds__(BIN_THREADS) void bin_count_kernel(int P, GsrBinViews tab) {
  extern __shared__ uint32_t s_cnt[];
  __shared__ uint32_t s_red[BIN_THREADS / 64];
  __shared__ uint32_t s_wave[BIN_THREADS / 64];
  __shared__ uint2 s_big[BIN_BIG_MAX];
  __shared__ uint32_t s_bigdepth[BIN_BIG_MAX];
  __shared__ uint32_t s_nbig;
  const GsrBinView& vw = tab.v[blockIdx.y];
  const int T = tab.T, Ts = gsr_bin_stride(T), gx = tab.gx, tid = threadIdx.x, lane = tid & 63, wv = tid >> 6;
  const int g0 = (int)blockIdx.x * GSR_BIN_G;
  const bool lists = !vw.shares_lists;
  const uint32_t* __restrict__ cut = vw.depth_cut;
  const bool cut_l = cut && tab.cut_lds;
  const uint32_t* s_cut = s_cnt + T;
  const uint32_t* s_cc = s_cnt + 2 * T;
  const int gxc = (gx + 3) >> 2;
  if (cut_l)
    for (int t = tid; t < T; t += BIN_THREADS) s_cnt[T + t] = cut[t];
  auto cut_at = [&](uint32_t t) { return cut_l ? s_cut[t] : cut[t]; };
  auto behind_all = [&](uint2 r, uint32_t dbits) {
    const uint32_t x0 = (r.x & 0xffffu) >> 2, y0 = (r.x >> 16) >> 2, x1 = ((r.y & 0xffffu) - 1u) >> 2, y1 = ((r.y >> 16) - 1u) >> 2;
    uint32_t m = 0u;
    for (uint32_t y = y0; y <= y1; ++y)
      for (uint32_t x = x0; x <= x1; ++x) m = max(m, s_cc[y * gxc + x]);
    return dbits > m;
  };
  const bool want_offsets = !tab.forward_only;
  if (!lists && !want_offsets) {
    if (blockIdx.x == 0 && tid == 0) vw.offsets[P] = 0;
    return;
  }
  uint32_t tt[BIN_PER_THREAD];
  uint2 rc[BIN_PER_THREAD], ek[BIN_PER_THREAD];
#pragma unroll
  for (int q = 0; q < BIN_PER_THREAD; ++q) {
    const int g = g0 + tid * BIN_PER_THREAD + q;
    tt[q] = 0; rc[q] = make_uint2(0u, 0u); ek[q] = rc[q];
    if (g < P) { tt[q] = vw.tiles_touched[g]; if (lists) { rc[q] = vw.rect[g]; ek[q] = vw.ekey[g]; } }
  }
  const int jb = g0 / GSR_BLOCK;
  uint32_t part = 0;
  if (vw.block_offsets) { if (tid == 0) part = vw.block_offsets[jb]; }
  else for (int j = tid; j < jb; j += BIN_THREADS) part += vw.block_sums[j];
  if (lists) for (int t = tid; t < T; t += BIN_THREADS) s_cnt[t] = 0;
  if (tid == 0) s_nbig = 0;
  uint32_t sum = 0;
#pragma unroll
  for (int q = 0; q < BIN_PER_THREAD; ++q) sum += tt[q];
  uint32_t inc = sum;
#pragma unroll
  for (int d = 1; d < 64; d <<= 1) {
    const uint32_t o = __shfl_up(inc, d, 64);
    if (lane >= d) inc += o;
  }
#pragma unroll
  for (int m = 32; m >= 1; m >>= 1) part += __shfl_xor(part, m, 64);
  if (lane == 63) s_wave[wv] = inc;
  if (lane == 0) s_red[wv] = part;
  __syncthreads();
  uint32_t run = inc - sum;
#pragma unroll
  for (int w = 0; w < BIN_THREADS / 64; ++w) { run += s_red[w]; if (w < wv) run += s_wave[w]; }
#pragma unroll
  for (int q = 0; q < BIN_PER_THREAD; ++q) {
    const int g = g0 + tid * BIN_PER_THREAD + q;
    if (g < P && want_offsets) {
      vw.offsets[g] = run;
      reinterpret_cast<uint32_t*>(vw.rec_w + GSR_REC_F4 * (size_t)g + 3)[2] = run;
    }
    run += tt[q];
  }
  if (g0 + GSR_BIN_G >= P && tid == BIN_THREADS - 1) vw.offsets[P] = run;
  if (!lists) return;
  if (cut_l) {
    const int gyc = (T / gx + 3) >> 2;
    for (int c = tid; c < gxc * gyc; c += BIN_THREADS) {
      const int cx = c % gxc, cy = c / gxc;
      uint32_t m = 0u;
      for (int y = 4 * cy; y < min(4 * cy + 4, T / gx); ++y)
        for (int x = 4 * cx; x < min(4 * cx + 4, gx); ++x) m = max(m, s_cut[y * gx + x]);
      s_cnt[2 * T + c] = m;
    }
    __syncthreads();
  }
#pragma unroll
  for (int q = 0; q < BIN_PER_THREAD; ++q) {
    if (!tt[q]) continue;
    if (cut_l && behind_all(rc[q], ek[q].x)) continue;
    const BinGauss b = bin_gauss(rc[q], ek[q].y);
    if (b.area > BIN_BIG_AREA) {
      const uint32_t slot = atomicAdd(&s_nbig, 1u);
      if (slot < BIN_BIG_MAX) { s_big[slot] = rc[q]; s_bigdepth[slot] = ek[q].x; continue; }
    }
    const uint32_t dbits = ek[q].x;
    if (cut) bin_for_tiles(b, gx, [&](uint32_t t) { if (dbits <= cut_at(t)) atomicAdd(&s_cnt[t], 1u); });
    else bin_for_tiles(b, gx, [&](uint32_t t) { atomicAdd(&s_cnt[t], 1u); });
  }
  __syncthreads();
  const uint32_t nbig = min(s_nbig, (uint32_t)BIN_BIG_MAX);
  for (uint32_t i = wv; i < nbig; i += BIN_THREADS / 64) {
    const BinGauss b = bin_gauss(s_big[i], 0u);
    const uint32_t dbits = s_bigdepth[i];
    for (uint32_t k = lane; k < b.area; k += 64) {
      const uint32_t t = bin_tile_of(b, k, gx);
      if (!cut || dbits <= cut_at(t)) atomicAdd(&s_cnt[t], 1u);
    }
  }
  if (nbig) __syncthreads();
  uint32_t* __restrict__ row = vw.tile_rows + (size_t)blockIdx.x * Ts;
  for (int t = tid; t < Ts; t += BIN_THREADS) row[t] = t < T ? s_cnt[t] : 0u;
  if (blockIdx.x == 0 && tid < 64) vw.block_hist[tid] = 0u;
}

__global__ __launch_bounds__(GSR_BLOCK) void bin_colprefix_kernel(GsrBinViews tab) {
  const GsrBinView& vw = tab.v[blockIdx.y];
  if (vw.shares_lists) return;
  const int Ts = gsr_bin_stride(tab.T), rows = tab.rows, t = blockIdx.x * GSR_BLOCK + threadIdx.x;
  if (t >= Ts) return;
  uint32_t* __restrict__ m = vw.tile_rows;
  uint32_t run = 0;
  int r = 0;
  for (; r + 8 <= rows; r += 8) {
    uint32_t v[8];
#pragma unroll
    for (int u = 0; u < 8; ++u) v[u] = m[(size_t)(r + u) * Ts + t];
#pragma unroll
    for (int u = 0; u < 8; ++u) { m[(size_t)(r + u) * Ts + t] = run; run += v[u]; }
  }
  for (; r < rows; ++r) { const uint32_t v = m[(size_t)r * Ts + t]; m[(size_t)r * Ts + t] = run; run += v; }
  m[(size_t)rows * Ts + t] = run;
}

__global__ __launch_bounds__(GSR_BLOCK) void bin_colprefix_scan_kernel(GsrBinViews tab) {
  const GsrBinView& vw = tab.v[blockIdx.y];
  if (vw.shares_lists) return;
  __shared__ uint32_t s_w[GSR_BLOCK / 64];
  __shared__ uint32_t s_base;
  const int T = tab.T, Ts = gsr_bin_stride(T), rows = tab.rows, tid = threadIdx.x, lane = tid & 63, wv = tid >> 6;
  const int t = blockIdx.x * GSR_BLOCK + tid;
  uint32_t* __restrict__ m = vw.tile_rows;
  uint32_t run = 0;
  if (t < Ts) {
    int r = 0;
    for (; r + 8 <= rows; r += 8) {
      uint32_t v[8];
#pragma unroll
      for (int u = 0; u < 8; ++u) v[u] = m[(size_t)(r + u) * Ts + t];
#pragma unroll
      for (int u = 0; u < 8; ++u) { m[(size_t)(r + u) * Ts + t] = run; run += v[u]; }
    }
    for (; r < rows; ++r) { const uint32_t v = m[(size_t)r * Ts + t]; m[(size_t)r * Ts + t] = run; run += v; }
    m[(size_t)rows * Ts + t] = run;
  }
  uint32_t inc = run;
#pragma unroll
  for (int d = 1; d < 64; d <<= 1) {
    const uint32_t o = __shfl_up(inc, d, 64);
    if (lane >= d) inc += o;
  }
  if (lane == 63) s_w[wv] = inc;
  __syncthreads();
  uint32_t before = 0, total = 0;
#pragma unroll
  for (int w = 0; w < GSR_BLOCK / 64; ++w) { if (w < wv) before += s_w[w]; total += s_w[w]; }
  uint32_t* __restrict__ words = vw.block_hist;
  if (tid == 0) __hip_atomic_store(&words[blockIdx.x], 0x80000000u | total, __ATOMIC_RELAXED, __HIP_MEMORY_SCOPE_AGENT);
  if (wv == 0) {
    uint32_t mine = 0;
    if (lane < (int)blockIdx.x) {
      uint32_t w;
      do { w = __hip_atomic_load(&words[lane], __ATOMIC_RELAXED, __HIP_MEMORY_SCOPE_AGENT); } while (!(w & 0x80000000u));
      mine = w & 0x7fffffffu;
    }
#pragma unroll
    for (int k = 32; k >= 1; k >>= 1) mine += __shfl_xor(mine, k, 64);
    if (lane == 0) s_base = mine;
  }
  __syncthreads();
  const uint32_t start = s_base + before + inc - run, cap = vw.D;
  if (t < T) vw.ranges[t] = make_uint2(min(start, cap), min(start + run, cap));
}

__device__ __forceinline__ void bin_scan_view(const GsrBinViews& tab, const GsrBinView& vw, int prefixed, uint32_t* s_wave, uint32_t* s_carry) {
  const int T = tab.T, Ts = gsr_bin_stride(T), rows = tab.rows, tid = threadIdx.x, lane = tid & 63, wv = tid >> 6;
  uint32_t* __restrict__ m = vw.tile_rows;
  const uint32_t cap = vw.D;
  if (tid == 0) *s_carry = 0;
  __syncthreads();
  for (int q0 = 0; q0 < Ts / 4; q0 += BIN_THREADS) {
    const int q = q0 + tid;
    const bool live = q < Ts / 4;
    uint4 tot = make_uint4(0u, 0u, 0u, 0u);
    if (live) {
      if (prefixed) tot = *reinterpret_cast<const uint4*>(m + (size_t)rows * Ts + 4 * q);
      else {
        for (int r0 = 0; r0 < rows; r0 += BIN_ROW_CHUNK) {
          uint4 v[BIN_ROW_CHUNK];
#pragma unroll
          for (int r = 0; r < BIN_ROW_CHUNK; ++r)
            v[r] = r0 + r < rows ? *reinterpret_cast<const uint4*>(m + (size_t)(r0 + r) * Ts + 4 * q) : make_uint4(0u, 0u, 0u, 0u);
#pragma unroll
          for (int r = 0; r < BIN_ROW_CHUNK; ++r)
            if (r0 + r < rows) {
              *reinterpret_cast<uint4*>(m + (size_t)(r0 + r) * Ts + 4 * q) = tot;
              tot.x += v[r].x; tot.y += v[r].y; tot.z += v[r].z; tot.w += v[r].w;
            }
        }
      }
    }
    const uint32_t mine = tot.x + tot.y + tot.z + tot.w;
    uint32_t inc = mine;
#pragma unroll
    for (int d = 1; d < 64; d <<= 1) {
      const uint32_t o = __shfl_up(inc, d, 64);
      if (lane >= d) inc += o;
    }
    if (lane == 63) s_wave[wv] = inc;
    __syncthreads();
    uint32_t start = *s_carry + inc - mine;
    for (int w = 0; w < wv; ++w) start += s_wave[w];
    if (live) {
      const uint32_t c[4] = {tot.x, tot.y, tot.z, tot.w};
      uint32_t st_ = start;
#pragma unroll
      for (int k = 0; k < 4; ++k) {
        if (4 * q + k < T) vw.ranges[4 * q + k] = make_uint2(min(st_, cap), min(st_ + c[k], cap));
        st_ += c[k];
      }
    }
    __syncthreads();
    if (tid == BIN_THREADS - 1) *s_carry = start + mine;
    __syncthreads();
  }
}

__global__ __launch_bounds__(BIN_THREADS) void bin_scan_kernel(GsrBinViews tab, int prefixed) {
  __shared__ uint32_t s_wave[BIN_THREADS / 64];
  __shared__ uint32_t s_carry;
  const GsrBinView& vw = tab.v[blockIdx.x];
  if (vw.shares_lists) return;
  bin_scan_view(tab, vw, prefixed, s_wave, &s_carry);
}

__global__ __launch_bounds__(BIN_THREADS) void bin_emit_kernel(int P, GsrBinViews tab, int order_wgs, int items_per_wg) {
  extern __shared__ uint32_t s_cur[];
  if ((int)blockIdx.x >= tab.rows) {
    __shared__ TileOrderLds L;
    if (blockIdx.y == 0) tile_order_body(tab, items_per_wg, (int)blockIdx.x - tab.rows, L);
    return;
  }
  (void)order_wgs;
  __shared__ uint2 s_big[BIN_BIG_MAX];
  __shared__ uint64_t s_bigkey[BIN_BIG_MAX];
  __shared__ uint32_t s_nbig;
  const GsrBinView& vw = tab.v[blockIdx.y];
  const int T = tab.T, Ts = gsr_bin_stride(T), gx = tab.gx, tid = threadIdx.x, lane = tid & 63, wv = tid >> 6;
  const int g0 = (int)blockIdx.x * GSR_BIN_G;
  if (vw.shares_lists) return;
  const uint32_t cap = vw.D;
  const uint32_t* __restrict__ row = vw.tile_rows + (size_t)blockIdx.x * Ts;
  const uint32_t* __restrict__ cut = vw.depth_cut;
  const bool cut_l = cut && tab.cut_lds;
  const uint32_t* s_cut = s_cur + T;
  const uint32_t* s_cc = s_cur + 2 * T;
  const int gxc = (gx + 3) >> 2;
  if (cut_l)
    for (int t = tid; t < T; t += BIN_THREADS) s_cur[T + t] = cut[t];
  auto cut_at = [&](uint32_t t) { return cut_l ? s_cut[t] : cut[t]; };
  auto behind_all = [&](uint2 r, uint32_t dbits) {
    const uint32_t x0 = (r.x & 0xffffu) >> 2, y0 = (r.x >> 16) >> 2, x1 = ((r.y & 0xffffu) - 1u) >> 2, y1 = ((r.y >> 16) - 1u) >> 2;
    uint32_t m = 0u;
    for (uint32_t y = y0; y <= y1; ++y)
      for (uint32_t x = x0; x <= x1; ++x) m = max(m, s_cc[y * gxc + x]);
    return dbits > m;
  };
  uint64_t* __restrict__ dg = vw.dg[0];
  uint2 rc[BIN_PER_THREAD], ek[BIN_PER_THREAD];
#pragma unroll
  for (int q = 0; q < BIN_PER_THREAD; ++q) {
    const int g = g0 + tid * BIN_PER_THREAD + q;
    rc[q] = make_uint2(0u, 0u); ek[q] = rc[q];
    if (g < P) { rc[q] = vw.rect[g]; ek[q] = vw.ekey[g]; }
  }
  if (tid == 0) s_nbig = 0;
  for (int t = tid; t < T; t += BIN_THREADS) s_cur[t] = vw.ranges[t].x + row[t];
  __syncthreads();
  if (cut_l) {
    const int gyc = (T / gx + 3) >> 2;
    for (int c = tid; c < gxc * gyc; c += BIN_THREADS) {
      const int cx = c % gxc, cy = c / gxc;
      uint32_t m = 0u;
      for (int y = 4 * cy; y < min(4 * cy + 4, T / gx); ++y)
        for (int x = 4 * cx; x < min(4 * cx + 4, gx); ++x) m = max(m, s_cut[y * gx + x]);
      s_cur[2 * T + c] = m;
    }
    __syncthreads();
  }
#pragma unroll
  for (int q = 0; q < BIN_PER_THREAD; ++q) {
    const BinGauss b = bin_gauss(rc[q], ek[q].y);
    if (b.area == 0u) continue;
    if (cut_l && behind_all(rc[q], ek[q].x)) continue;
    const uint64_t key = ((uint64_t)ek[q].x << 32) | (uint32_t)(g0 + tid * BIN_PER_THREAD + q);
    if (b.area > BIN_BIG_AREA) {
      const uint32_t slot = atomicAdd(&s_nbig, 1u);
      if (slot < BIN_BIG_MAX) { s_big[slot] = rc[q]; s_bigkey[slot] = key; continue; }
    }
    const uint32_t dbits = ek[q].x;
    bin_for_tiles(b, gx, [&](uint32_t t) {
      if (cut && dbits > cut_at(t)) return;
      const uint32_t slot = atomicAdd(&s_cur[t], 1u);
      if (slot < cap) dg[slot] = key;
    });
  }
  __syncthreads();
  const uint32_t nbig = min(s_nbig, (uint32_t)BIN_BIG_MAX);
  for (uint32_t i = wv; i < nbig; i += BIN_THREADS / 64) {
    const BinGauss b = bin_gauss(s_big[i], 0u);
    const uint64_t key = s_bigkey[i];
    for (uint32_t k = lane; k < b.area; k += 64) {
      const uint32_t t = bin_tile_of(b, k, gx);
      if (cut && (uint32_t)(key >> 32) > cut_at(t)) continue;
      const uint32_t slot = atomicAdd(&s_cur[t], 1u);
      if (slot < cap) dg[slot] = key;
    }
  }
}

__global__ __launch_bounds__(GSR_BLOCK) void tile_ranges_kernel(GsrBinViews tab, int cur) {
  const GsrBinView& vw = tab.v[blockIdx.y];
  const uint32_t* __restrict__ tkey = vw.tkey[cur];
  uint2* __restrict__ ranges = vw.ranges;
  const uint32_t D = bin_entries(vw);
  uint32_t i = blockIdx.x * GSR_BLOCK + threadIdx.x;
  if (i >= D) return;
  uint32_t t = tkey[i];
  if (i == 0) ranges[t].x = 0;
  else {
    uint32_t pt = tkey[i - 1];
    if (pt != t) { ranges[pt].y = i; ranges[t].x = i; }
  }
  if (i == D - 1) ranges[t].y = D;
}


template <typename PTR>
__device__ __forceinline__ void tile_sort_network(PTR a, uint32_t n, int tid, const uint32_t NT = GSR_BLOCK) {
  uint32_t lg = 1;
  while ((1u << lg) < n) ++lg;
  const uint32_t npairs = (1u << lg) >> 1;
  for (uint32_t lk = 1; lk <= lg; ++lk) {
    const uint32_t k = 1u << lk, hk = k >> 1;
    for (uint32_t p = tid; p < npairs; p += NT) {
      const uint32_t base = (p >> (lk - 1)) << lk, off = p & (hk - 1);
      const uint32_t l = base + off, r = base + (k - 1 - off);
      if (r < n) {
        uint64_t x = a[l], y = a[r];
        if (y < x) { a[l] = y; a[r] = x; }
      }
    }
    __syncthreads();
    for (int lj = (int)lk - 2; lj >= 0; --lj) {
      const uint32_t j = 1u << lj;
      for (uint32_t p = tid; p < npairs; p += NT) {
        const uint32_t l = ((p >> lj) << (lj + 1)) + (p & (j - 1)), r = l + j;
        if (r < n) {
          uint64_t x = a[l], y = a[r];
          if (y < x) { a[l] = y; a[r] = x; }
        }
      }
      __syncthreads();
    }
  }
}

template <int M>
__device__ __forceinline__ uint32_t gsr_lane_xor(uint32_t v) {
  if constexpr (M == 1) return (uint32_t)__builtin_amdgcn_update_dpp(0, (int)v, 0xB1, 0xf, 0xf, true);
  else if constexpr (M == 2) return (uint32_t)__builtin_amdgcn_update_dpp(0, (int)v, 0x4E, 0xf, 0xf, true);
  else if constexpr (M == 3) return (uint32_t)__builtin_amdgcn_update_dpp(0, (int)v, 0x1B, 0xf, 0xf, true);
  else if constexpr (M == 7) return (uint32_t)__builtin_amdgcn_update_dpp(0, (int)v, 0x141, 0xf, 0xf, true);
  else if constexpr (M == 15) return (uint32_t)__builtin_amdgcn_update_dpp(0, (int)v, 0x140, 0xf, 0xf, true);
  else if constexpr (M == 8) return (uint32_t)__builtin_amdgcn_update_dpp(0, (int)v, 0x128, 0xf, 0xf, true);
  else if constexpr (M < 32) return (uint32_t)__builtin_amdgcn_ds_swizzle((int)v, (M << 10) | 0x1F);
  else return (uint32_t)__shfl_xor((int)v, M, 64);
}
template <int V> struct gsr_log2 { static constexpr int value = 1 + gsr_log2<(V >> 1)>::value; };
template <> struct gsr_log2<1> { static constexpr int value = 0; };
template <int MASK, int NR>
__device__ __forceinline__ void wave_sort_step(uint64_t (&x)[NR], int lane) {
  constexpr int LR = gsr_log2<NR>::value;
  constexpr int R = MASK & (NR - 1), L = MASK >> LR;
  constexpr int HB = MASK >= 1024 ? 1024 : MASK >= 512 ? 512 : MASK >= 256 ? 256 : MASK >= 128 ? 128 : MASK >= 64 ? 64 : MASK >= 32 ? 32 : MASK >= 16 ? 16 : MASK >= 8 ? 8 : MASK >= 4 ? 4 : MASK >= 2 ? 2 : 1;
  if constexpr (L == 0) {
#pragma unroll
    for (int r = 0; r < NR; ++r) {
      if ((r & HB) == 0) {
        const uint64_t a = x[r], b = x[r ^ R];
        const bool sw = b < a;
        x[r] = sw ? b : a;
        x[r ^ R] = sw ? a : b;
      }
    }
  } else {
    uint64_t y[NR];
#pragma unroll
    for (int r = 0; r < NR; ++r) {
      const uint64_t src = x[r ^ R];
      y[r] = ((uint64_t)gsr_lane_xor<L>((uint32_t)(src >> 32)) << 32) | gsr_lane_xor<L>((uint32_t)src);
    }
    const bool upper = (lane & (HB >> LR)) != 0;
#pragma unroll
    for (int r = 0; r < NR; ++r) {
      const bool take = (y[r] < x[r]) != upper;
      x[r] = take ? y[r] : x[r];
    }
  }
}
template <int LK, int NR>
__device__ __forceinline__ void wave_sort_stage(uint64_t (&x)[NR], int lane) {
  static_assert(LK <= 11, "the half-cleaner steps below stop at stride 512");
  wave_sort_step<(1 << LK) - 1, NR>(x, lane);
  if constexpr (LK >= 11) wave_sort_step<512, NR>(x, lane);
  if constexpr (LK >= 10) wave_sort_step<256, NR>(x, lane);
  if constexpr (LK >= 9) wave_sort_step<128, NR>(x, lane);
  if constexpr (LK >= 8) wave_sort_step<64, NR>(x, lane);
  if constexpr (LK >= 7) wave_sort_step<32, NR>(x, lane);
  if constexpr (LK >= 6) wave_sort_step<16, NR>(x, lane);
  if constexpr (LK >= 5) wave_sort_step<8, NR>(x, lane);
  if constexpr (LK >= 4) wave_sort_step<4, NR>(x, lane);
  if constexpr (LK >= 3) wave_sort_step<2, NR>(x, lane);
  if constexpr (LK >= 2) wave_sort_step<1, NR>(x, lane);
}
template <int NR>
__device__ __forceinline__ void wave_sort_tile(const uint64_t* __restrict__ seg, uint32_t* __restrict__ out, uint32_t n, int lane) {
  uint64_t x[NR];
#pragma unroll
  for (int r = 0; r < NR; ++r) { const uint32_t e = (uint32_t)(r * 64 + lane); x[r] = e < n ? seg[e] : ~0ull; }
// ... 161 lines not shown
  if (n == 1) {
    if (tid == 0) point_list[rg.x] = (uint32_t)seg[0];
  } else if (n <= (uint32_t)RCAP) {
    if (tid == 0) L.diff = 0;
    __syncthreads();
    const uint32_t k0 = (uint32_t)(seg[0] >> 32);
    uint32_t d = 0;
    for (uint32_t i = tid; i < n; i += NT) {
      const uint64_t e = seg[i];
      const uint32_t k = (uint32_t)(e >> 32);
      L.r.key[0][i] = k; L.r.val[0][i] = (uint32_t)e;
      d |= k ^ k0;
    }
    if (d) atomicOr(&L.diff, d);
    __syncthreads();
    const int cur = tile_radix_sort(L, n, tid);
    {
      uint32_t* __restrict__ kk = L.r.key[cur];
      uint32_t* __restrict__ vv = L.r.val[cur];
      bool long_run = false;
      for (uint32_t i = tid; i + 1 < n; i += NT) {
        if (kk[i] == kk[i + 1] && (i == 0 || kk[i - 1] != kk[i])) {
          uint32_t j = i + 1;
          while (j + 1 < n && kk[j + 1] == kk[i] && j - i < 32u) ++j;
          if (j + 1 < n && kk[j + 1] == kk[i]) { long_run = true; continue; }
          for (uint32_t a = i + 1; a <= j; ++a) {
            const uint32_t x = vv[a];
            uint32_t b = a;
            while (b > i && vv[b - 1] > x) { vv[b] = vv[b - 1]; --b; }
            vv[b] = x;
          }
        }
      }
      if (__syncthreads_or(long_run ? 1 : 0)) {
        uint64_t e[(RCAP + NT - 1) / NT];
#pragma unroll
        for (int u = 0; u < (RCAP + NT - 1) / NT; ++u) {
          const uint32_t i = (uint32_t)u * NT + tid;
          e[u] = i < n ? (((uint64_t)kk[i] << 32) | vv[i]) : 0ull;
        }
        __syncthreads();
#pragma unroll
        for (int u = 0; u < (RCAP + NT - 1) / NT; ++u) {
          const uint32_t i = (uint32_t)u * NT + tid;
          if (i < n) L.net[i] = e[u];
        }
        __syncthreads();
        tile_sort_network(L.net, n, tid, NT);
        for (uint32_t i = tid; i < n; i += NT) point_list[rg.x + i] = (uint32_t)L.net[i];
        return;
      }
    }
    for (uint32_t i = tid; i < n; i += NT) point_list[rg.x + i] = L.r.val[cur][i];
  } else if (n <= 2u * (uint32_t)RCAP) {
    for (uint32_t i = tid; i < n; i += NT) L.net[i] = seg[i];
    __syncthreads();
    tile_sort_network(L.net, n, tid, NT);
    for (uint32_t i = tid; i < n; i += NT) point_list[rg.x + i] = (uint32_t)L.net[i];
  } else {
    __syncthreads();
    tile_sort_network((volatile uint64_t*)seg, n, tid, NT);
    for (uint32_t i = tid; i < n; i += NT) point_list[rg.x + i] = (uint32_t)seg[i];
  }
}

__global__ __launch_bounds__(GSR_BLOCK) void copy_tile_state_kernel(int T, int n_order, const uint2* __restrict__ src_ranges,
                                                                    const uint4* __restrict__ src_order, const uint32_t* __restrict__ src_queue,
                                                                    uint2* __restrict__ ranges, uint4* __restrict__ order, uint32_t* __restrict__ queue) {
  const int i = blockIdx.x * GSR_BLOCK + threadIdx.x;
  if (i < T) ranges[i] = src_ranges[i];
  if (i < n_order) order[i] = src_order[i];
  if (i < 9) queue[i] = (i == 4 || i == 6 || i == 7) ? src_queue[i] : 0u;
}

}
using namespace gsr_binning;

int gsr_launch_shared_lists(const GsrBinViews& tab_in, int P, uint32_t D, const uint2* owner_ranges, const uint4* owner_order,
                            const uint32_t* owner_queue, uint2* ranges, uint4* order, uint32_t* queue, hipStream_t st) {
  GsrBinViews tab = tab_in;
  tab.v[0].shares_lists = 1;
  { GSR_PROF("emit_entries", st);
    hipLaunchKernelGGL(emit_entries_kernel, dim3(D / GSR_RADIX_EPB + 1u, 1), dim3(GSR_BLOCK), 0, st, P, tab, 0, 1); }
  GSR_HIP_CHECK(hipGetLastError());
  { GSR_PROF("copy_tile_state", st);
    hipLaunchKernelGGL(copy_tile_state_kernel, dim3((tab.T + GSR_BLOCK - 1) / GSR_BLOCK), dim3(GSR_BLOCK), 0, st, tab.T, tab.T, owner_ranges,
                       owner_order, owner_queue, ranges, order, queue); }
  GSR_HIP_CHECK(hipGetLastError());
  return 0;
}

int gsr_launch_scan_exclusive(const uint32_t* in, uint32_t* out, uint32_t n, uint32_t* total_out, hipStream_t st) {
  { GSR_PROF("scan", st);
  hipLaunchKernelGGL(scan_exclusive_kernel, dim3(1), dim3(SCAN_THREADS), 0, st, in, out, n, total_out); }
  GSR_HIP_CHECK(hipGetLastError());
  return 0;
}

static int ceil_log2_u32(uint32_t n) {
  int b = 0;
  while (((uint64_t)1 << b) < n) ++b;
  return b;
}

static size_t bin_lds_limit() {
  static const size_t v = [] {
    int dev = 0, a = 0;
    if (hipGetDevice(&dev) == hipSuccess && hipDeviceGetAttribute(&a, hipDeviceAttributeMaxSharedMemoryPerBlock, dev) == hipSuccess && a > 0) return (size_t)a;
    return (size_t)(64 << 10);
  }();
  return v;
}
static size_t bin_lds_static() {
  static const size_t v = [] {
    hipFuncAttributes a{}, b{};
    size_t m = 0;
    if (hipFuncGetAttributes(&a, reinterpret_cast<const void*>(bin_emit_kernel)) == hipSuccess) m = a.sharedSizeBytes;
    if (hipFuncGetAttributes(&b, reinterpret_cast<const void*>(bin_count_kernel)) == hipSuccess && b.sharedSizeBytes > m) m = b.sharedSizeBytes;
    return m ? m : (size_t)(52 << 10);
  }();
  return v;
}
bool gsr_rows_path_ok(int T) {
  const char* e = getenv("GSR_RADIX_BINNING");
  const bool radix_only = e && *e && atoi(e) != 0;
  return !radix_only && T > 0 && T <= GSR_BIN_MAX_T && bin_lds_static() + sizeof(uint32_t) * (size_t)T <= bin_lds_limit();
}
int gsr_launch_binning(const GsrBinViews& tab_in, int P, hipStream_t st) {
  if (tab_in.V <= 0 || tab_in.T <= 0) return 0;
  GsrBinViews tab = tab_in;
  uint32_t maxD = 0, maxblk = 0;
  for (int v = 0; v < tab.V; ++v) { maxD = tab.v[v].D > maxD ? tab.v[v].D : maxD; maxblk = tab.v[v].nblocks > maxblk ? tab.v[v].nblocks : maxblk; }
  const char* force = getenv("GSR_TILE_SORT_RCAP");
  const bool big = force ? (force[0] == '4') : (maxD / (uint32_t)tab.T > 600u);
  tab.wave_cap = big ? 2048 : 512;
  {
    static uint32_t* hint = [] { uint32_t* p = nullptr; if (hipHostMalloc((void**)&p, 64, hipHostMallocMapped | hipHostMallocCoherent) != hipSuccess) return (uint32_t*)nullptr; *p = 1u; return p; }();
    tab.vlong_out = hint;
    tab.vlong_launch = (!hint || __atomic_load_n(hint, __ATOMIC_RELAXED) != 0u) ? 1 : 0;
  }
  int cur = 0;
  bool order_done = false;
  bool any_cut = false;
  for (int v = 0; v < tab.V; ++v) any_cut = any_cut || tab.v[v].depth_cut != nullptr;
  const size_t coarse = (size_t)((tab.gx + 3) / 4) * (size_t)((tab.T / tab.gx + 3) / 4);
  tab.cut_lds = (any_cut && bin_lds_static() + sizeof(uint32_t) * (2 * (size_t)tab.T + coarse) <= bin_lds_limit()) ? 1 : 0;
  const size_t lds = sizeof(uint32_t) * (tab.cut_lds ? 2 * (size_t)tab.T + coarse : (size_t)tab.T);
  const bool rows_path = tab.rows > 0 && gsr_rows_path_ok(tab.T) && maxD > 0 && P > 0;
  if (rows_path) {
    { GSR_PROF("bin_count", st);
      hipLaunchKernelGGL(bin_count_kernel, dim3(tab.rows, tab.V), dim3(BIN_THREADS), lds, st, P, tab);
    }
    GSR_HIP_CHECK(hipGetLastError());
    const int prefixed = tab.rows > BIN_DIRECT_ROWS ? 1 : 0;
    const int col_wgs = (gsr_bin_stride(tab.T) + GSR_BLOCK - 1) / GSR_BLOCK;
    const bool chained = prefixed && col_wgs <= 64;
    if (chained) {
      GSR_PROF("bin_colprefix", st);
      hipLaunchKernelGGL(bin_colprefix_scan_kernel, dim3(col_wgs, tab.V), dim3(GSR_BLOCK), 0, st, tab);
    } else if (prefixed) {
      GSR_PROF("bin_colprefix", st);
      hipLaunchKernelGGL(bin_colprefix_kernel, dim3(col_wgs, tab.V), dim3(GSR_BLOCK), 0, st, tab);
    }
    GSR_HIP_CHECK(hipGetLastError());
    const int n_items = tab.V * ((tab.T + 1023) / 1024);
    if (!chained) {
      GSR_PROF("bin_scan", st);
      hipLaunchKernelGGL(bin_scan_kernel, dim3(tab.V), dim3(BIN_THREADS), 0, st, tab, prefixed);
    }
    GSR_HIP_CHECK(hipGetLastError());
    int order_wgs = 0, per_wg = 1;
    {
      order_wgs = n_items < ORD_MAX_WG ? n_items : ORD_MAX_WG;
      if (order_wgs < 1) order_wgs = 1;
      per_wg = (n_items + order_wgs - 1) / order_wgs;
      if (per_wg < 1) per_wg = 1;
      order_wgs = (n_items + per_wg - 1) / per_wg;
      if (order_wgs < 1) order_wgs = 1;
      order_done = true;
    }
    { GSR_PROF("bin_emit", st);
      hipLaunchKernelGGL(bin_emit_kernel, dim3(tab.rows + order_wgs, tab.V), dim3(BIN_THREADS), lds, st, P, tab, order_wgs, per_wg); }
    GSR_HIP_CHECK(hipGetLastError());
  } else if (maxD == 0 || P <= 0) {
    for (int v = 0; v < tab.V; ++v) GSR_HIP_CHECK(hipMemsetAsync(tab.v[v].ranges, 0, sizeof(uint2) * (size_t)tab.T, st));
  } else {
    const int tbits = ceil_log2_u32((uint32_t)tab.T);
    const int npass = (tbits + 7) / 8;
    const int bpp = npass ? (tbits + npass - 1) / npass : 0;
    { GSR_PROF("emit_entries", st);
    const int bits0 = npass ? (tbits < bpp ? tbits : bpp) : 1;
    hipLaunchKernelGGL(emit_entries_kernel, dim3(maxD / GSR_RADIX_EPB + 1u, tab.V), dim3(GSR_BLOCK), 0, st, P, tab, 0, bits0); }
    GSR_HIP_CHECK(hipGetLastError());
    for (int pass = 0; pass < npass; ++pass) {
      const int shift = pass * bpp;
      const int bits = (tbits - shift) < bpp ? (tbits - shift) : bpp;
      if (pass > 0) {
        GSR_PROF("radix_hist", st);
        hipLaunchKernelGGL(radix_hist_kernel, dim3(maxblk, tab.V), dim3(GSR_BLOCK), 0, st, tab, cur, shift, bits);
      }
      GSR_HIP_CHECK(hipGetLastError());
      const int prescanned = maxblk >= GSR_COLSCAN_MIN_BLOCKS ? 1 : 0;
      if (prescanned) {
        GSR_PROF("radix_colscan", st);
        hipLaunchKernelGGL(radix_colscan_kernel, dim3(1u << bits, tab.V), dim3(1024), 0, st, tab, bits);
      }
      GSR_HIP_CHECK(hipGetLastError());
      { GSR_PROF("radix_scatter", st);
      hipLaunchKernelGGL(radix_scatter_kernel, dim3(maxblk, tab.V), dim3(GSR_BLOCK), 0, st, tab, cur, shift, bits, prescanned,
                         pass == npass - 1 ? 1 : 0); }
      GSR_HIP_CHECK(hipGetLastError());
      cur ^= 1;
    }
    if (npass == 0) {
      GSR_PROF("tile_ranges", st);
      hipLaunchKernelGGL(tile_ranges_kernel, dim3((maxD + GSR_BLOCK - 1) / GSR_BLOCK, tab.V), dim3(GSR_BLOCK), 0, st, tab, cur);
    }
    GSR_HIP_CHECK(hipGetLastError());
  }
  if (!order_done)
    if (int rc = gsr_launch_tile_order(tab, st)) return rc;
  if (maxD > 0 && P > 0) {
    { GSR_PROF("tile_sort", st);
    if (big) {
      hipLaunchKernelGGL((tile_sort_kernel<2048, 2>), dim3((tab.V * tab.T + 3) / 4), dim3(GSR_BLOCK), 0, st, tab, cur);
      if (tab.wave_cap == 2048) hipLaunchKernelGGL((tile_sort_kernel<2048, 3>), dim3((tab.V * tab.T + 3) / 4), dim3(GSR_BLOCK), 0, st, tab, cur);
      const int g1 = tab.V * tab.T < 512 ? tab.V * tab.T : 512;
      hipLaunchKernelGGL((tile_sort_kernel<4096, 1, 8>), dim3(g1), dim3(512), 0, st, tab, cur);
    } else
      {
        const bool small_lds = !(force && force[0] == '2');
        if (small_lds) {
          hipLaunchKernelGGL(tile_sort_kernel<1024>, dim3(tab.V * tab.T), dim3(GSR_BLOCK), 0, st, tab, cur);
          if (tab.vlong_launch) hipLaunchKernelGGL((tile_sort_kernel<4096, 1, 16>), dim3(64), dim3(1024), 0, st, tab, cur);
        } else hipLaunchKernelGGL(tile_sort_kernel<2048>, dim3(tab.V * tab.T), dim3(GSR_BLOCK), 0, st, tab, cur);
      } }
    GSR_HIP_CHECK(hipGetLastError());
  }
  return 0;
}

int gsr_launch_tile_order(const GsrBinViews& tab, hipStream_t st) {
  { GSR_PROF("tile_order", st);
    const int n_items = tab.V * ((tab.T + 1023) / 1024);
    int wgs = n_items < ORD_MAX_WG ? n_items : ORD_MAX_WG;
    if (wgs < 1) wgs = 1;
    const int per_wg = (n_items + wgs - 1) / wgs;
    wgs = per_wg > 0 ? (n_items + per_wg - 1) / per_wg : 1;
    hipLaunchKernelGGL(tile_order_kernel, dim3(wgs < 1 ? 1 : wgs), dim3(1024), 0, st, tab, per_wg > 0 ? per_wg : 1); }
  GSR_HIP_CHECK(hipGetLastError());
  return 0;
}
```

### gs-dynamics_amd/csrc/gsr_common.h

```cpp
#pragma once
#include <hip/hip_runtime.h>
#include <stdint.h>
#include <stddef.h>
#include "../../include/gsr.h"

#define GSR_WAVE 64
#define GSR_BLOCK 256
#define GSR_NEAR_Z 0.2f
#define GSR_ALPHA_MIN (1.0f / 255.0f)
#define GSR_ALPHA_MAX 0.99f
#define GSR_T_EPS 0.0001f

#define GSR_REC_F4 4
#ifndef GSR_BIN_G
#define GSR_BIN_G 2048
#endif
#define GSR_BIN_MAX_T 10240
struct GeomState {
  float4* rec;
  uint2* rect;
  uint32_t* tiles_touched;
  uint32_t* offsets;
  uint32_t* block_sums;
  uint32_t* block_offsets;
  uint32_t* clamped;
  uint32_t* counters;
  uint2* ekey;
  uint2* block_hash;
  uint32_t* tile_rows;
  uint8_t* used;
};
struct ImageState {
  float* final_T;
  uint32_t* n_contrib;
  uint2* ranges;
  uint4* tile_order;
  uint32_t* queue;
};
struct BinningState {
  uint32_t* tkey[2];
  uint64_t* dg[2];
  uint32_t* point_list;
  uint32_t* block_hist;
  uint8_t* contrib;
};

static inline __host__ __device__ size_t gsr_align(size_t x, size_t a = 256) { return (x + a - 1) / a * a; }

#define GSR_RADIX_ITEMS 8
#define GSR_RADIX_EPB (GSR_BLOCK * GSR_RADIX_ITEMS)

static inline uint32_t gsr_radix_blocks(uint32_t D) { return D == 0 ? 1u : (D + GSR_RADIX_EPB - 1) / GSR_RADIX_EPB; }

static inline size_t gsr_carve_geom(void* base, int32_t P, GeomState* g) {
  size_t off = 0, Pn = (size_t)(P > 0 ? P : 1);
  char* b = (char*)base;
  auto take = [&](size_t bytes) { char* p = b ? b + off : nullptr; off += gsr_align(bytes); return p; };
  g->rec = (float4*)take(Pn * 16 * GSR_REC_F4);
  g->rect = (uint2*)take(Pn * 8);
  g->tiles_touched = (uint32_t*)take(Pn * 4);
  g->offsets = (uint32_t*)take((Pn + 1) * 4);
  const size_t nblk = (Pn + GSR_BLOCK - 1) / GSR_BLOCK;
  g->block_sums = (uint32_t*)take(nblk * 4);
  g->block_offsets = (uint32_t*)take((nblk + 1) * 4);
  g->clamped = (uint32_t*)take(Pn * 4);
  g->counters = (uint32_t*)take(64);
  g->ekey = (uint2*)take(Pn * 8);
  g->block_hash = (uint2*)take(nblk * 8);
  g->tile_rows = (uint32_t*)take(((Pn + GSR_BIN_G - 1) / GSR_BIN_G + 1) * (size_t)GSR_BIN_MAX_T * 4);
  g->used = (uint8_t*)take(Pn);
  return off;
}
static inline size_t gsr_carve_image(void* base, int32_t H, int32_t W, ImageState* im) {
  size_t off = 0, N = (size_t)H * W;
  size_t T = (size_t)((H + GSR_TILE - 1) / GSR_TILE) * ((W + GSR_TILE - 1) / GSR_TILE);
  char* b = (char*)base;
  auto take = [&](size_t bytes) { char* p = b ? b + off : nullptr; off += gsr_align(bytes); return p; };
  im->final_T = (float*)take((N ? N : 1) * 4);
  im->n_contrib = (uint32_t*)take((N ? N : 1) * 4);
  im->ranges = (uint2*)take((T ? T : 1) * 8);
  im->tile_order = (uint4*)take((T ? T : 1) * 16);
  im->queue = (uint32_t*)take(64);
  return off;
}
static inline size_t gsr_carve_binning(void* base, uint32_t D, BinningState* bs) {
  size_t off = 0, Dn = D ? D : 1;
  size_t nb = gsr_radix_blocks(D);
  char* b = (char*)base;
  auto take = [&](size_t bytes) { char* p = b ? b + off : nullptr; off += gsr_align(bytes); return p; };
  bs->tkey[0] = (uint32_t*)take(Dn * 4);
  bs->tkey[1] = (uint32_t*)take(Dn * 4);
  bs->dg[0] = (uint64_t*)take(Dn * 8);
  bs->dg[1] = (uint64_t*)take(Dn * 8);
  bs->point_list = (uint32_t*)take(Dn * 4);
  bs->block_hist = (uint32_t*)take(256 * (nb + 1) * 4);
  bs->contrib = (uint8_t*)take(Dn);
  return off;
}

#define GSR_PARTIAL_FLOATS 9
#define GSR_HOST_SCAN_MAX_BLOCKS 2048
static inline bool gsr_host_block_scan(int P) { return (P + GSR_BLOCK - 1) / GSR_BLOCK <= GSR_HOST_SCAN_MAX_BLOCKS; }

int gsr_launch_gnn_aggregate(int N, int n_sum, int H, const float* rew1, const float* a23, const long long* send, const long long* row_start, float* agg, hipStream_t st,
                             const float* res_a = nullptr, const float* res_b = nullptr, float* res_out = nullptr);
int gsr_launch_gnn_rel_inputs(int E, int A, int G, int S, const float* nodes, const long long* recv, const long long* send, float* out, hipStream_t st);

void gsr_set_error(const char* fmt, ...);
#define GSR_HIP_CHECK(expr)                                                                   \
  do {                                                                                        \
    hipError_t _e = (expr);                                                                   \
    if (_e != hipSuccess) {                                                                   \
      gsr_set_error("%s failed: %s (%s:%d)", #expr, hipGetErrorString(_e), __FILE__, __LINE__); \
      return (int)_e ? (int)_e : -1;                                                          \
    }                                                                                         \
  } while (0)

struct GsrRange {
  explicit GsrRange(const char* name);
  ~GsrRange();
  bool on;
};
struct GsrProfScope {
  GsrProfScope(const char* name, hipStream_t st);
  ~GsrProfScope();
  int slot;
  hipStream_t st;
  GsrRange range;
};
#define GSR_PROF_CAT2(a, b) a##b
#define GSR_PROF_CAT(a, b) GSR_PROF_CAT2(a, b)
#define GSR_PROF(name, st) GsrProfScope GSR_PROF_CAT(_gsr_prof_, __LINE__)(name, st)

struct GsrCam {
  int H, W, gx, gy, T;
  float tanfovx, tanfovy, scale_modifier;
  int sh_degree, M;
  const float *bg, *view, *proj, *campos;
  int antialiasing;
};

struct GsrPreView {
  const float *view, *proj, *campos;
  const float* colors;
  float tanfovx, tanfovy;
  float4* rec; uint2* rect; uint32_t* tiles_touched; uint32_t* clamped; int32_t* radii; uint32_t* block_sums;
  uint2* ekey;
  uint2* block_hash;
  const float4* cmp_rec; const uint2* cmp_rect; const uint2* cmp_ekey; const uint32_t* cmp_tiles;
  uint8_t* used; uint32_t* tracked;
  int skip;
};
struct GsrPreViews {
  int V;
  const float *raw_rot, *raw_op, *raw_sc;
  float *rot_out, *op_out, *sc_out;
  GsrPreView v[GSR_MAX_BATCH];
};
struct GsrBinView {
  const float4* rec; const uint2* rect; const uint32_t* tiles_touched;
  const uint32_t* block_sums; const uint32_t* block_offsets;
  uint32_t* offsets;
  uint32_t* tkey[2]; uint64_t* dg[2]; uint32_t* point_list; uint32_t* block_hist;
  uint2* ranges;
  uint32_t D, nblocks;
  const uint32_t* D_dev;
  uint32_t shares_lists;
  int32_t owner;
  uint32_t fused_alias;
  const uint2* ekey;
  float4* rec_w;
  uint32_t* tile_rows;
  const uint32_t* depth_cut;
};
struct GsrBinViews {
  int V, T, gx; uint4* order; uint32_t* queue;
  uint32_t* counts_out; int P;
  int wave_cap;
  int rows;
  uint32_t* vlong_out;
  int vlong_launch;
  int forward_only;
  int cut_lds;
  GsrBinView v[GSR_MAX_BATCH];
};
struct GsrRenderView {
  const uint32_t* point_list; const float4* rec; const float* bg;
  float* final_T; uint32_t* n_contrib; float* out_color; float* out_depth;
  const float* dL_dcolor; const uint2* rect; const uint32_t* offsets; float4* partials;
  const uint2* ranges;
  const float* dL_dalpha;
  const float* colors;
  uint8_t* contrib;
  uint8_t* used; uint32_t* tracked;
  int partner;
  int fused_alias;
  float cut_margin;
  const uint32_t* cut_in; uint32_t* cut_out; uint32_t* redo;
};
struct GsrRenderViews {
  int V, W, H, gx, T; const uint4* order; uint32_t* queue;
  int no_colour_grad;
  uint32_t* pc_error_out;
  int prio_frac256;
  int track;
  uint32_t avg_list;
  GsrRenderView v[GSR_MAX_BATCH];
};

static inline int gsr_bin_rows(int P) { return ((P > 0 ? P : 1) + GSR_BIN_G - 1) / GSR_BIN_G; }
static inline __host__ __device__ int gsr_bin_stride(int T) { return (T + 3) & ~3; }
struct BatchState {
  uint32_t* sums;
  uint4* order;
  uint32_t* queue;
  uint32_t* tile_rows;
};
static inline size_t gsr_carve_batch(void* base, int V, int32_t P, int32_t H, int32_t W, BatchState* b) {
  size_t off = 0;
  const size_t nblk = ((size_t)(P > 0 ? P : 1) + GSR_BLOCK - 1) / GSR_BLOCK;
  const size_t T = (size_t)((H + GSR_TILE - 1) / GSR_TILE) * ((W + GSR_TILE - 1) / GSR_TILE);
  char* p0 = (char*)base;
  auto take = [&](size_t bytes) { char* p = p0 ? p0 + off : nullptr; off += gsr_align(bytes); return p; };
  b->sums = (uint32_t*)take((size_t)V * nblk * 4);
  b->order = (uint4*)take((size_t)V * (T ? T : 1) * 16);
  b->queue = (uint32_t*)take(64);
  b->tile_rows = nullptr;
  if (T <= GSR_BIN_MAX_T) b->tile_rows = (uint32_t*)take((size_t)V * (gsr_bin_rows(P) + 1) * (size_t)gsr_bin_stride((int)(T ? T : 1)) * 4);
  return off;
}

int gsr_launch_preprocess(const GsrPreViews& tab, const GsrCam& cam, int P, const float* means3D, const float* scales,
                          const float* rotations, const float* opacities, const float* colors_precomp,
                          const float* shs, const float* cov3D_precomp, hipStream_t st);
bool gsr_rows_path_ok(int T);
int gsr_launch_scan_exclusive(const uint32_t* in, uint32_t* out, uint32_t n, uint32_t* total_out, hipStream_t st);
int gsr_launch_binning(const GsrBinViews& tab, int P, hipStream_t st);
int gsr_launch_tile_order(const GsrBinViews& tab, hipStream_t st);
int gsr_launch_shared_lists(const GsrBinViews& tab, int P, uint32_t D, const uint2* owner_ranges, const uint4* owner_order,
                            const uint32_t* owner_queue, uint2* ranges, uint4* order, uint32_t* queue, hipStream_t st);
int gsr_launch_gather_counts(const GsrBinViews& tab, int P, uint32_t* counts_dev, hipStream_t st);
int gsr_launch_render_fwd(const GsrRenderViews& tab, hipStream_t st);
struct GsrDepthViews { const float* dL_ddepth[GSR_MAX_BATCH]; float* dL_dz[GSR_MAX_BATCH]; };
static inline size_t gsr_depth_scratch_offset(uint32_t D) { return gsr_align((size_t)(D ? D : 1) * GSR_PARTIAL_FLOATS * 4); }
int gsr_launch_render_bwd(const GsrRenderViews& tab, hipStream_t st, const GsrDepthViews* depth = nullptr);
static_assert(sizeof(GsrRenderViews) + sizeof(GsrDepthViews) <= 4096, "render_bwd kernel arguments above 4 KB");
struct GsrAlphaViews { int V, N; const float* final_T[GSR_MAX_BATCH]; float* out[GSR_MAX_BATCH]; };
int gsr_launch_alpha(const GsrAlphaViews& tab, hipStream_t st);
int gsr_launch_preprocess_bwd(const GsrCam& cam, int P, const float* means3D, const float* scales,
                              const float* rotations, const float* colors_precomp, const float* shs,
                              const float* cov3D_precomp, const int32_t* radii, const GeomState& g,
                              const float4* partials, float* dL_dmeans3D, float* dL_dmeans2D, float* dL_dcolors,
                              float* dL_dopacity, float* dL_dscales, float* dL_drotations, float* dL_dcov3D,
                              float* dL_dsh, const uint32_t* bwd_error, hipStream_t st, const float* dL_dz = nullptr);
struct GsrBwdView {
  const float *view, *proj;
  const int32_t* radii;
  const uint8_t* used; const uint32_t* tracked;
  const uint32_t* offsets;
  const float4* partials;
  float* dL_dmeans2D;
  float* dL_dcolors;
  float* partner_dL_dmeans2D;
  int fused_alias;
  uint32_t cap;
  int W, H;
  float tanfovx, tanfovy;
};
#define GSR_QUEUE_BWD_ERROR 8
struct GsrBwdViews {
  int V;
  const uint32_t* bwd_error;
  const float *raw_rot, *act_op, *act_sc;
  float *d_raw_rot, *d_raw_op, *d_raw_sc;
  GsrBwdView v[GSR_MAX_BATCH];
};
struct GsrAaViews { const float4* rec[GSR_MAX_BATCH]; };
static_assert(sizeof(GsrBwdViews) + sizeof(GsrDepthViews) + sizeof(GsrAaViews) + 128 <= 4096, "preprocess_bwd_views kernel arguments above 4 KB");
int gsr_launch_preprocess_bwd_views(const GsrBwdViews& vw, int P, float scale_modifier, const float* means3D,
                                    const float* scales, const float* rotations, const float* cov3D_precomp,
                                    float* dL_dmeans3D, float* dL_dcolors, float* dL_dopacity, float* dL_dscales,
                                    float* dL_drotations, float* dL_dcov3D, hipStream_t st, const GsrDepthViews* depth = nullptr,
                                    const GsrAaViews* aa = nullptr);
struct GsrCamView {
  const float *view, *proj, *campos;
  const int32_t* radii;
  const uint8_t* used; const uint32_t* tracked;
  const uint32_t* offsets;
  const float4* partials;
  const float* dL_dz;
  const float4* rec;
  const uint32_t* clamped;
  const float* final_T;
  const float* dL_dcolor;
  double* slab;
  float *out_view, *out_proj, *out_campos, *out_bg;
  uint32_t cap;
  int W, H;
  float tanfovx, tanfovy;
};
struct GsrCamViews {
  int V, P, nblk, sh_degree, M;
  float mod;
  const uint32_t* bwd_error;
  const float *means3D, *scales, *rotations, *cov3D, *shs;
  GsrCamView v[GSR_MAX_BATCH];
};
static_assert(sizeof(GsrCamViews) + 64 <= 4096, "camera_bwd kernel arguments above 4 KB");
#define GSR_CAM_ROW 32
static inline int gsr_camera_blocks(int P, int H, int W) {
  const long long g = ((long long)(P > 0 ? P : 0) + GSR_BLOCK - 1) / GSR_BLOCK;
  long long px = ((long long)(H > 0 ? H : 0) * (W > 0 ? W : 0) + GSR_BLOCK - 1) / GSR_BLOCK;
  if (px > 256) px = 256;
  const long long n = g > px ? g : px;
  return (int)(n > 0 ? n : 1);
}
int gsr_launch_camera_bwd(const GsrCamViews& cv, bool antialiasing, hipStream_t st);
struct GsrShView {
  const float* campos;
  const int32_t* radii;
  const uint32_t* clamped;
  const float* dcol;
};
struct GsrShViews {
  int V, P, M, deg;
// ... 135 lines not shown
                                                      float v6, float v7, float v8) {
  const int lane = gsr_lane();
  const bool b0 = lane & 1, b1 = lane & 2;
  float r01, r23, r45, r67;
  asm("s_nop 4\n\t"
      "v_add_f32_dpp %0, %4, %4 row_shl:4 row_mask:0xf bank_mask:0x5\n\t"
      "v_add_f32_dpp %1, %6, %6 row_shl:4 row_mask:0xf bank_mask:0x5\n\t"
      "v_add_f32_dpp %2, %8, %8 row_shl:4 row_mask:0xf bank_mask:0x5\n\t"
      "v_add_f32_dpp %3, %10, %10 row_shl:4 row_mask:0xf bank_mask:0x5\n\t"
      "v_add_f32_dpp %0, %5, %5 row_shr:4 row_mask:0xf bank_mask:0xa\n\t"
      "v_add_f32_dpp %1, %7, %7 row_shr:4 row_mask:0xf bank_mask:0xa\n\t"
      "v_add_f32_dpp %2, %9, %9 row_shr:4 row_mask:0xf bank_mask:0xa\n\t"
      "v_add_f32_dpp %3, %11, %11 row_shr:4 row_mask:0xf bank_mask:0xa"
      : "=&v"(r01), "=&v"(r23), "=&v"(r45), "=&v"(r67)
      : "v"(v0), "v"(v4), "v"(v1), "v"(v5), "v"(v2), "v"(v6), "v"(v3), "v"(v7));
  const float r8 = v8 + gsr_swz_xor4(v8);
  const float q03 = (b0 ? r23 : r01) + gsr_dpp_get<0xB1>(b0 ? r01 : r23);
  const float q47 = (b0 ? r67 : r45) + gsr_dpp_get<0xB1>(b0 ? r45 : r67);
  const float q8 = r8 + gsr_dpp_get<0xB1>(r8);
  const float p07 = (b1 ? q47 : q03) + gsr_dpp_get<0x4E>(b1 ? q03 : q47);
  const float p8 = q8 + gsr_dpp_get<0x4E>(q8);
  float z;
  asm("s_nop 1\n\t"
      "v_add_f32_dpp %0, %1, %1 row_ror:8 row_mask:0xf bank_mask:0x3\n\t"
      "v_add_f32_dpp %0, %2, %2 row_ror:8 row_mask:0xf bank_mask:0xc"
      : "=&v"(z) : "v"(p07), "v"(p8));
  return gsr_rows_sum<PERM>(z);
}


__device__ __forceinline__ float gsr_wave_sum8_packed(float v0, float v1, float v2, float v3, float v4, float v5,
                                                      float v6, float v7) {
  const int lane = gsr_lane();
  const bool b0 = lane & 1, b1 = lane & 2;
  float r01, r23, r45, r67;
  asm("s_nop 4\n\t"
      "v_add_f32_dpp %0, %4, %4 row_shl:4 row_mask:0xf bank_mask:0x5\n\t"
      "v_add_f32_dpp %1, %6, %6 row_shl:4 row_mask:0xf bank_mask:0x5\n\t"
      "v_add_f32_dpp %2, %8, %8 row_shl:4 row_mask:0xf bank_mask:0x5\n\t"
      "v_add_f32_dpp %3, %10, %10 row_shl:4 row_mask:0xf bank_mask:0x5\n\t"
      "v_add_f32_dpp %0, %5, %5 row_shr:4 row_mask:0xf bank_mask:0xa\n\t"
      "v_add_f32_dpp %1, %7, %7 row_shr:4 row_mask:0xf bank_mask:0xa\n\t"
      "v_add_f32_dpp %2, %9, %9 row_shr:4 row_mask:0xf bank_mask:0xa\n\t"
      "v_add_f32_dpp %3, %11, %11 row_shr:4 row_mask:0xf bank_mask:0xa"
      : "=&v"(r01), "=&v"(r23), "=&v"(r45), "=&v"(r67)
      : "v"(v0), "v"(v4), "v"(v1), "v"(v5), "v"(v2), "v"(v6), "v"(v3), "v"(v7));
  const float q03 = (b0 ? r23 : r01) + gsr_dpp_get<0xB1>(b0 ? r01 : r23);
  const float q47 = (b0 ? r67 : r45) + gsr_dpp_get<0xB1>(b0 ? r45 : r67);
  float z = (b1 ? q47 : q03) + gsr_dpp_get<0x4E>(b1 ? q03 : q47);
  z += gsr_dpp_get<0x128>(z);
  return gsr_rows_sum<false>(z);
}

__device__ __forceinline__ int gsr_sum6_slot(int lane) {
  if (lane & 2) return -1;
  if (!(lane & 1)) return 2 * ((lane >> 3) & 1) + ((lane >> 2) & 1);
  return (lane & 8) ? -1 : 4 + ((lane >> 2) & 1);
}
__device__ __forceinline__ float gsr_wave_sum6_packed(float v0, float v1, float v2, float v3, float v4, float v5) {
  const bool b0 = gsr_lane() & 1;
  float r01, r23, r45, q03, q45;
  asm("s_nop 4\n\t"
      "v_add_f32_dpp %0, %3, %3 row_shl:4 row_mask:0xf bank_mask:0x5\n\t"
      "v_add_f32_dpp %1, %5, %5 row_shl:4 row_mask:0xf bank_mask:0x5\n\t"
      "v_add_f32_dpp %2, %7, %7 row_shl:4 row_mask:0xf bank_mask:0x5\n\t"
      "v_add_f32_dpp %0, %4, %4 row_shr:4 row_mask:0xf bank_mask:0xa\n\t"
      "v_add_f32_dpp %1, %6, %6 row_shr:4 row_mask:0xf bank_mask:0xa\n\t"
      "v_add_f32_dpp %2, %8, %8 row_shr:4 row_mask:0xf bank_mask:0xa"
      : "=&v"(r01), "=&v"(r23), "=&v"(r45)
      : "v"(v0), "v"(v1), "v"(v2), "v"(v3), "v"(v4), "v"(v5));
  asm("s_nop 1\n\t"
      "v_add_f32_dpp %0, %2, %2 row_ror:8 row_mask:0xf bank_mask:0x3\n\t"
      "v_add_f32_dpp %1, %4, %4 row_ror:8 row_mask:0xf bank_mask:0xf\n\t"
      "v_add_f32_dpp %0, %3, %3 row_ror:8 row_mask:0xf bank_mask:0xc"
      : "=&v"(q03), "=&v"(q45) : "v"(r01), "v"(r23), "v"(r45));
  float z = (b0 ? q45 : q03) + gsr_dpp_get<0xB1>(b0 ? q03 : q45);
  z += gsr_dpp_get<0x4E>(z);
  return gsr_rows_sum<false>(z);
}

__device__ __forceinline__ float gsr_quat_norm(float4 q) { return sqrtf(fmaf(q.w, q.w, fmaf(q.z, q.z, fmaf(q.y, q.y, q.x * q.x)))); }
__device__ __forceinline__ float4 gsr_act_rotation(float4 q) {
  const float d = fmaxf(gsr_quat_norm(q), 1e-12f);
  return make_float4(q.x / d, q.y / d, q.z / d, q.w / d);
}
__device__ __forceinline__ float gsr_act_opacity(float logit) { return 1.0f / (1.0f + expf(-logit)); }
__device__ __forceinline__ float gsr_act_scale(float logs) { return expf(logs); }
__device__ __forceinline__ float4 gsr_act_rotation_bwd(float4 q, float4 dr) {
  const float n = gsr_quat_norm(q);
  if (n > 1e-12f) {
    const float inv = 1.0f / n;
    const float rx = q.x * inv, ry = q.y * inv, rz = q.z * inv, rw = q.w * inv;
    const float dot = fmaf(rw, dr.w, fmaf(rz, dr.z, fmaf(ry, dr.y, rx * dr.x)));
    return make_float4(fmaf(-rx, dot, dr.x) * inv, fmaf(-ry, dot, dr.y) * inv, fmaf(-rz, dot, dr.z) * inv, fmaf(-rw, dot, dr.w) * inv);
  }
  return make_float4(dr.x * 1e12f, dr.y * 1e12f, dr.z * 1e12f, dr.w * 1e12f);
}

#define GSR_AA_FLOOR 2.5e-5f
__device__ __forceinline__ float gsr_aa_ratio(float A, float B, float C, float det1) {
  const float w = B * B;
  const float e = fmaf(-B, B, w);
  return (fmaf(A, C, -w) + e) / det1;
}
__device__ __forceinline__ float gsr_aa_comp(float r) { return sqrtf(fmaxf(r, GSR_AA_FLOOR)); }

__device__ __forceinline__ float gsr_exp(float x) { return __builtin_amdgcn_exp2f(x * 1.44269502162933349609375f); }
struct GsrF3 { float x, y, z; };
__device__ __forceinline__ void gsr_store_partial(float4* base, size_t e, float4 r0, float4 r1, float r2x) {
  GsrF3* p = reinterpret_cast<GsrF3*>(reinterpret_cast<float*>(base) + e * GSR_PARTIAL_FLOATS);
  p[0] = GsrF3{r0.x, r0.y, r0.z}; p[1] = GsrF3{r0.w, r1.x, r1.y}; p[2] = GsrF3{r1.z, r1.w, r2x};
}
__device__ __forceinline__ void gsr_store_partial6(float4* base, size_t e, float4 r0, float r1x, float r1y) {
  GsrF3* p = reinterpret_cast<GsrF3*>(reinterpret_cast<float*>(base) + e * GSR_PARTIAL_FLOATS);
  p[0] = GsrF3{r0.x, r0.y, r0.z}; p[1] = GsrF3{r0.w, r1x, r1y};
}
__device__ __forceinline__ void gsr_load_partial6(const float4* base, size_t e, float4& r0, float& r1x, float& r1y) {
  const GsrF3* p = reinterpret_cast<const GsrF3*>(reinterpret_cast<const float*>(base) + e * GSR_PARTIAL_FLOATS);
  const GsrF3 a = p[0], b = p[1];
  r0 = make_float4(a.x, a.y, a.z, b.x); r1x = b.y; r1y = b.z;
}
__device__ __forceinline__ void gsr_load_partial(const float4* base, size_t e, float4& r0, float4& r1, float& r2x) {
  const GsrF3* p = reinterpret_cast<const GsrF3*>(reinterpret_cast<const float*>(base) + e * GSR_PARTIAL_FLOATS);
  const GsrF3 a = p[0], b = p[1], c = p[2];
  r0 = make_float4(a.x, a.y, a.z, b.x); r1 = make_float4(b.y, b.z, c.x, c.y); r2x = c.z;
}
__device__ __forceinline__ float qmin_on_vertical_edge(float A, float B, float C, float invC, float dx, float dylo, float dyhi) {
  const float dy = fminf(fmaxf(-B * dx * invC, dylo), dyhi);
  return A * dx * dx + (2.0f * B * dx + C * dy) * dy;
}
__device__ __forceinline__ float qmin_on_horizontal_edge(float A, float B, float C, float invA, float dy, float dxlo, float dxhi) {
  const float dx = fminf(fmaxf(-B * dy * invA, dxlo), dxhi);
  return C * dy * dy + (2.0f * B * dy + A * dx) * dx;
}
__device__ __forceinline__ float gsr_qmin_facing_edges(float A, float B, float C, float invA, float invC, float dxlo, float dxhi, float dylo, float dyhi) {
  const bool in_x = dxlo <= 0.0f && dxhi >= 0.0f, in_y = dylo <= 0.0f && dyhi >= 0.0f;
  const float dxe = dxlo > 0.0f ? dxlo : dxhi, dye = dylo > 0.0f ? dylo : dyhi;
  const float qv = qmin_on_vertical_edge(A, B, C, invC, dxe, dylo, dyhi);
  const float qh = qmin_on_horizontal_edge(A, B, C, invA, dye, dxlo, dxhi);
  const float inf = __builtin_inff();
  return fminf(in_x ? inf : qv, in_y ? inf : qh);
}
__device__ __forceinline__ bool gsr_rect_reachable(float mx, float my, float A, float B, float C, float invA, float invC, float tau2,
                                                   int x0, int y0, int x1, int y1) {
  const float dxlo = (float)x0 - mx, dxhi = (float)x1 - mx, dylo = (float)y0 - my, dyhi = (float)y1 - my;
  if (dxlo <= 0.0f && dxhi >= 0.0f && dylo <= 0.0f && dyhi >= 0.0f) return true;
  return gsr_qmin_facing_edges(A, B, C, invA, invC, dxlo, dxhi, dylo, dyhi) <= tau2;
}
__device__ __forceinline__ uint32_t gsr_tile_rank(uint32_t mask, uint32_t area, uint32_t r) {
  return area <= 32u ? (uint32_t)__popc(mask & ((1u << r) - 1u)) : r;
}
#define BIN_THREADS 1024
#define BIN_PER_THREAD (GSR_BIN_G / BIN_THREADS)
#ifndef BIN_DIRECT_ROWS
#define BIN_DIRECT_ROWS 32
#endif
#ifndef BIN_ROW_CHUNK
#define BIN_ROW_CHUNK 16
#endif
#define BIN_BIG_AREA 64
#define BIN_BIG_MAX 1024

struct BinGauss { uint32_t minx, miny, w, area, mask; float rw; };
__device__ __forceinline__ BinGauss bin_gauss(uint2 r, uint32_t mask) {
  BinGauss b;
  b.minx = r.x & 0xffffu; b.miny = r.x >> 16;
  const uint32_t maxx = r.y & 0xffffu, maxy = r.y >> 16;
  b.w = maxx - b.minx; b.area = b.w * (maxy - b.miny); b.mask = mask;
  b.rw = __builtin_amdgcn_rcpf((float)b.w);
  return b;
}
__device__ __forceinline__ uint32_t bin_tile_of(const BinGauss& b, uint32_t k, int gx) {
  const uint32_t ky = (uint32_t)(((float)k + 0.5f) * b.rw);
  return (b.miny + ky) * (uint32_t)gx + b.minx + (k - ky * b.w);
}
template <typename F>
__device__ __forceinline__ void bin_for_tiles(const BinGauss& b, int gx, F f) {
  if (b.area <= 32u) {
    uint32_t m = b.mask;
    while (m) {
      const uint32_t k = (uint32_t)__ffs((int)m) - 1u;
      m &= m - 1u;
      f(bin_tile_of(b, k, gx));
    }
  } else {
    for (uint32_t k = 0; k < b.area; ++k) f(bin_tile_of(b, k, gx));
  }
}

__device__ __forceinline__ float gsr_wave_sum_shfl(float v) {
  for (int m = 32; m >= 1; m >>= 1) v += __shfl_xor(v, m, 64);
  return v;
}
#endif
```

### gs-dynamics_amd/csrc/gsr_preprocess_fwd_kernel.inc

```
#if GSR_PFWD_AA
#define GSR_PFWD_NAME(k) k##_aa_kernel
#else
#define GSR_PFWD_NAME(k) k##_kernel
#endif

__global__ __launch_bounds__(GSR_BLOCK) void GSR_PFWD_NAME(preprocess_fwd)(
    GsrPreViews tab, int P, int W, int H, int gx, int gy, float mod, int sh_degree, int M,
    const float* __restrict__ means3D, const float* __restrict__ scales, const float* __restrict__ rotations,
    const float* __restrict__ opacities, const float* __restrict__ colors_precomp,
    const float* __restrict__ shs, const float* __restrict__ cov3D_precomp, int tight_lists) {
  const GsrPreView& vw = tab.v[blockIdx.y];
  if (vw.skip) return;
  if (vw.colors) colors_precomp = vw.colors;
  uint32_t* __restrict__ block_sums = vw.block_sums;
  __shared__ uint32_t s_wave_sum[GSR_BLOCK / GSR_WAVE];
  const int i = blockIdx.x * GSR_BLOCK + threadIdx.x;
  __shared__ float4 s_rec[GSR_BLOCK / GSR_WAVE][256];
  const PreOut po = preprocess_gaussian<GSR_PFWD_AA>(tab, vw, i, P, s_rec[threadIdx.x >> 6], blockIdx.y == 0, W, H, gx, gy, mod, sh_degree, M, means3D, scales, rotations,
                                        opacities, colors_precomp, shs, cov3D_precomp, tight_lists);
  const uint32_t tiles = po.tiles;
  const int any = vw.block_hash ? __syncthreads_or(po.differs ? 1 : 0) : 0;
  uint32_t wsum = tiles;
#pragma unroll
  for (int m = 32; m >= 1; m >>= 1) wsum += __shfl_xor(wsum, m, 64);
  if ((threadIdx.x & 63) == 0) s_wave_sum[threadIdx.x >> 6] = wsum;
  __syncthreads();
  if (threadIdx.x == 0) {
    const uint32_t total = s_wave_sum[0] + s_wave_sum[1] + s_wave_sum[2] + s_wave_sum[3];
    block_sums[blockIdx.x] = total;
    if (vw.block_hash) vw.block_hash[blockIdx.x] = make_uint2(any ? 1u : 0u, total);
  }
}

#undef GSR_PFWD_NAME
```

Baseline: 5620.

## Replace binning column-prefix and scan kernels with atomic per-tile totals

bin_count now reserves per-row offsets with atomic fetch-add into a per-tile totals row, which preprocess zeroes beforehand. This removes the separate column-prefix and scan kernel launches. Each emit block then rescans the totals in LDS with DPP wave scans to get tile starts, and block 0 writes the ranges. The tile-order pass derives its ranges from the totals, with a recount fallback when a list overflows its capacity. This cuts launches and passes over the row matrix, but makes row offsets depend on atomic order and repeats the totals scan in every emit block.

```diff
diff --git a/gs-dynamics_amd/csrc/gsr_api.hip b/gs-dynamics_amd/csrc/gsr_api.hip
--- a/gs-dynamics_amd/csrc/gsr_api.hip
+++ b/gs-dynamics_amd/csrc/gsr_api.hip
@@ -99,6 +99,7 @@
   o.view = cam.view; o.proj = cam.proj; o.campos = cam.campos; o.tanfovx = cam.tanfovx; o.tanfovy = cam.tanfovy;
   o.rec = g.rec; o.rect = g.rect; o.tiles_touched = g.tiles_touched; o.clamped = g.clamped; o.radii = radii;
   o.block_sums = block_sums; o.ekey = g.ekey; o.block_hash = nullptr; o.cmp_rec = nullptr; o.cmp_rect = nullptr; o.cmp_ekey = nullptr; o.cmp_tiles = nullptr; o.skip = 0;
+  o.bin_totals = nullptr; o.bin_T = 0;
   o.used = g.used; o.tracked = g.counters + 1;
 }
 
@@ -113,7 +114,7 @@
   o.offsets = g.offsets;
   o.tkey[0] = bs.tkey[0]; o.tkey[1] = bs.tkey[1]; o.dg[0] = bs.dg[0]; o.dg[1] = bs.dg[1];
   o.point_list = bs.point_list; o.block_hist = bs.block_hist; o.ranges = im.ranges;
-  o.D = D; o.nblocks = D ? gsr_radix_blocks(D) : 0u;
+  o.D = D; o.nblocks = D ? gsr_radix_blocks(D) : 0u; o.list_cap = D;
 }
 void fill_render_view(GsrRenderView& o, const GsrCam& cam, const GeomState& g, const BinningState& bs, const ImageState& im,
                       float* out_color, float* out_depth, const float* dL_dcolor, float4* partials) {
@@ -175,7 +176,7 @@
 int stage1(int V, const gsr_settings* s, int32_t P, const float* means3D, const float* scales, const float* rotations,
            const float* opacities, const float* colors_precomp, const float* const* colors_views, const float* shs,
            const float* cov3D_precomp, void* const* geom_states, int32_t* const* radii, uint32_t* sums,
-           uint32_t* num_rendered_host, hipStream_t st, const gsr_raw_params* raw = nullptr, int32_t* same_host = nullptr,
+           uint32_t* num_rendered_host, hipStream_t st, uint32_t* tile_rows, const gsr_raw_params* raw = nullptr, int32_t* same_host = nullptr,
            const int* skip = nullptr, const int32_t* geometry_of = nullptr, const void* prev_geom = nullptr,
            uint32_t* differs_pinned = nullptr) {
   if (colors_views) {
@@ -228,6 +229,11 @@
       }
     }
     if (skip && skip[v]) tab.v[v].skip = 1;
+    if (tile_rows && cam.T <= GSR_BIN_MAX_T && !(geometry_of && geometry_of[v] != v)) {
+      const size_t Ts = (size_t)gsr_bin_stride(cam.T), rows = (size_t)gsr_bin_rows(P);
+      tab.v[v].bin_totals = tile_rows + ((size_t)v * (rows + 1) + rows) * Ts;
+      tab.v[v].bin_T = (int)Ts;
+    }
   }
   if (int rc = gsr_launch_preprocess(tab, cam0, P, means3D, scales, rotations, opacities, colors_precomp, shs, cov3D_precomp, st))
     return rc;
@@ -321,11 +327,11 @@
       return -2;
     }
     fill_bin_view(bt.v[v], P, num_rendered[v], g, bs, im, sums ? sums + (size_t)v * nblk : g.block_sums);
-    if (tile_rows) bt.v[v].tile_rows = tile_rows + (size_t)v * (gsr_bin_rows(P) + 1) * (size_t)gsr_bin_stride(cam.T);
+    if (tile_rows) bt.v[v].tile_rows = tile_rows + (size_t)owner * (gsr_bin_rows(P) + 1) * (size_t)gsr_bin_stride(cam.T);
     bt.v[v].owner = owner;
     fill_render_view(rt.v[v], cam, g, bs, im, out_color[v], out_depth[v], nullptr, nullptr);
     if (owner != v) {
-      bt.v[v].shares_lists = 1; bt.v[v].D = 0; bt.v[v].nblocks = 0; bt.v[v].ranges = im_owner.ranges;
+      bt.v[v].shares_lists = 1; bt.v[v].D = 0; bt.v[v].nblocks = 0; bt.v[v].ranges = im_owner.ranges; bt.v[v].list_cap = num_rendered[owner];
       rt.v[v].ranges = im_owner.ranges;
     }
     bt.v[v].fused_alias = (uint32_t)fused[v];
@@ -380,7 +386,7 @@
   gsr_carve_geom(geom_state, P, &g);
   uint32_t D = 0;
   if (int rc = stage1(1, s, P, means3D, scales, rotations, opacities, colors_precomp, nullptr, shs, cov3D_precomp, &geom_state,
-                      &radii, g.block_sums, &D, (hipStream_t)stream, nullptr, same_host, nullptr, nullptr, prev_geom_state))
+                      &radii, g.block_sums, &D, (hipStream_t)stream, gsr_rows_path_ok(cam.T) ? g.tile_rows : nullptr, nullptr, same_host, nullptr, nullptr, prev_geom_state))
     return rc;
   if (num_rendered_host) *num_rendered_host = D;
   return 0;
@@ -427,7 +433,7 @@
   GeomState g;
   gsr_carve_geom(geom_state, P, &g);
   if (int rc = stage1(1, s, P, means3D, scales, rotations, opacities, colors_precomp, nullptr, shs, cov3D_precomp, &geom_state, &radii,
-                      g.block_sums, nullptr, (hipStream_t)stream, nullptr, nullptr, nullptr, nullptr,
+                      g.block_sums, nullptr, (hipStream_t)stream, gsr_rows_path_ok(cam.T) ? g.tile_rows : nullptr, nullptr, nullptr, nullptr, nullptr,
                       words ? prev_geom_state : nullptr, words ? block_words_pinned : nullptr))
     return rc;
   uint32_t* late_count = count_pinned ? reinterpret_cast<uint32_t*>(count_pinned) : g.counters + 8;
@@ -756,7 +762,7 @@
   BatchState b;
   gsr_carve_batch(batch_state, V, P, s[0].image_height, s[0].image_width, &b);
   return stage1(V, s, P, means3D, scales, rotations, opacities, colors_precomp, colors_views, shs, cov3D_precomp, geom_states,
-                radii, b.sums, num_rendered_host, (hipStream_t)stream);
+                radii, b.sums, num_rendered_host, (hipStream_t)stream, b.tile_rows);
 }
 
 int gsr_forward_render_batch(int32_t V, const gsr_settings* s, int32_t P, const uint32_t* num_rendered,
@@ -796,7 +802,7 @@
   int skip[GSR_MAX_BATCH];
   skippable_aliases(V, geometry_of, colors_views, flags, skip);
   if (int rc = stage1(V, s, P, means3D, scales, rotations, opacities, colors_precomp, colors_views, shs, cov3D_precomp,
-                      geom_states, radii, b.sums, num_rendered_host, (hipStream_t)stream, nullptr, nullptr, skip, geometry_of))
+                      geom_states, radii, b.sums, num_rendered_host, (hipStream_t)stream, b.tile_rows, nullptr, nullptr, skip, geometry_of))
     return rc;
   bool fits = binning_states != nullptr && binning_bytes != nullptr;
   for (int v = 0; fits && v < V; ++v) {
@@ -831,7 +837,7 @@
   BatchState b;
   gsr_carve_batch(batch_state, V, P, s[0].image_height, s[0].image_width, &b);
   if (int rc = stage1(V, s, P, means3D, scales, rotations, opacities, colors_precomp, colors_views, shs, cov3D_precomp,
-                      geom_states, radii, b.sums, nullptr, (hipStream_t)stream, raw, nullptr, nullptr, geometry_of))
+                      geom_states, radii, b.sums, nullptr, (hipStream_t)stream, b.tile_rows, raw, nullptr, nullptr, geometry_of))
     return rc;
   return stage2(V, s, P, capacity_entries, geom_states, binning_states, image_states, out_color, out_depth, b.sums, b.order,
                 b.queue, geometry_of, (hipStream_t)stream, counts_dev, b.tile_rows);
diff --git a/gs-dynamics_amd/csrc/gsr_binning.hip b/gs-dynamics_amd/csrc/gsr_binning.hip
--- a/gs-dynamics_amd/csrc/gsr_binning.hip
+++ b/gs-dynamics_amd/csrc/gsr_binning.hip
@@ -55,6 +55,21 @@
 __device__ __forceinline__ uint32_t bin_entries(const GsrBinView& vw) { return vw.D_dev ? min(vw.D_dev[0], vw.D) : vw.D; }
 __device__ __forceinline__ uint32_t bin_blocks(const GsrBinView& vw, uint32_t D) {
   return vw.D_dev ? (D == 0 ? 1u : (D + GSR_RADIX_EPB - 1) / GSR_RADIX_EPB) : vw.nblocks;
+}
+
+#define BIN_SCAN_MAX (GSR_BIN_MAX_T / BIN_THREADS)
+template <int CTRL, int ROW_MASK = 0xf>
+__device__ __forceinline__ uint32_t bin_dpp_add(uint32_t v) {
+  return v + (uint32_t)__builtin_amdgcn_update_dpp(0, (int)v, CTRL, ROW_MASK, 0xf, false);
+}
+__device__ __forceinline__ uint32_t bin_wave_scan_incl(uint32_t v) {
+  v = bin_dpp_add<0x111>(v);
+  v = bin_dpp_add<0x112>(v);
+  v = bin_dpp_add<0x114>(v);
+  v = bin_dpp_add<0x118>(v);
+  v = bin_dpp_add<0x142, 0xA>(v);
+  v = bin_dpp_add<0x143, 0xC>(v);
+  return v;
 }
 
 #define EMIT_MAX_GBLOCKS GSR_HOST_SCAN_MAX_BLOCKS
@@ -398,12 +413,17 @@
 #define ORD_CHUNK 12
 #define ORD_WAVES 16
 #define ORD_MAX_WG 32
+#define ORD_KEEP 2
+#define ORD_MAX_ITEMS (GSR_MAX_BATCH * (GSR_BIN_MAX_T / 1024))
 struct TileOrderLds {
   uint32_t h_before[ORD_WAVES][256];
   uint32_t h_rest[ORD_WAVES][256];
   uint32_t start[256];
   uint32_t empty_before_s, n_busy_s, n_long_s, n_empty_s;
+  uint32_t overflow_s;
+  uint32_t wt[ORD_MAX_ITEMS][ORD_WAVES];
 };
+template <bool FROM_TOTALS>
 __device__ __forceinline__ void tile_order_body(const GsrBinViews& tab, int items_per_wg, int bid, TileOrderLds& L) {
   auto& h_before = L.h_before; auto& h_rest = L.h_rest; auto& start = L.start;
   uint32_t& empty_before_s = L.empty_before_s; uint32_t& n_busy_s = L.n_busy_s; uint32_t& n_long_s = L.n_long_s; uint32_t& n_empty_s = L.n_empty_s;
@@ -412,7 +432,7 @@
   uint4* __restrict__ tile_order = tab.order;
   uint32_t* __restrict__ queue = tab.queue;
   for (int i = tid; i < ORD_WAVES * 256; i += 1024) { (&h_before[0][0])[i] = 0; (&h_rest[0][0])[i] = 0; }
-  if (tid == 0) { empty_before_s = 0; n_empty_s = 0; }
+  if (tid == 0) { empty_before_s = 0; n_empty_s = 0; L.overflow_s = 0; }
   if (bid == 0) {
     if (tid < 9) queue[tid] = 0;
     if (tab.counts_out && tid < tab.V)
@@ -422,15 +442,93 @@
   const int n_it = (T + 1023) / 1024, n_items = tab.V * n_it;
   const int k_lo = bid * items_per_wg, k_hi = min(n_items, k_lo + items_per_wg);
   uint32_t empties_before = 0, empties_all = 0;
-  for (int k0 = 0; k0 < n_items; k0 += ORD_CHUNK) {
+  const int Ts = gsr_bin_stride(T);
+  const size_t tot_off = (size_t)tab.rows * Ts;
+  auto range_of = [&L, wv](int k, uint32_t cap, uint32_t c) -> uint2 {
+    const uint32_t s = L.wt[k][wv] + bin_wave_scan_incl(c) - c;
+    const uint32_t a = min(s, cap), b = min(s + c, cap);
+    return b > a ? make_uint2(a, b) : make_uint2(0u, 0u);
+  };
+  uint2 mine[ORD_KEEP];
+  uint32_t mine_e[ORD_KEEP], mine_c[ORD_KEEP];
+#pragma unroll
+  for (int j = 0; j < ORD_KEEP; ++j) { mine[j] = make_uint2(0u, 0u); mine_e[j] = 0u; mine_c[j] = 0u; }
+  const bool kept = FROM_TOTALS && k_hi - k_lo <= ORD_KEEP;
+  bool recount = true;
+  if constexpr (FROM_TOTALS) {
+    for (int k0 = 0; k0 < n_items; k0 += ORD_CHUNK) {
+      uint32_t c[ORD_CHUNK];
+#pragma unroll
+      for (int u = 0; u < ORD_CHUNK; ++u) {
+        const int k = k0 + u, t = (k % n_it) * 1024 + tid;
+        c[u] = 0u;
+        if (k < n_items && t < T && !tab.v[k / n_it].fused_alias) c[u] = tab.v[k / n_it].tile_rows[tot_off + t];
+      }
+#pragma unroll
+      for (int u = 0; u < ORD_CHUNK; ++u) {
+        if (k0 + u >= n_items) break;
+        const int k = k0 + u, t = (k % n_it) * 1024 + tid;
+        const uint32_t inc = bin_wave_scan_incl(c[u]);
+        if (lane == 63) L.wt[k][wv] = inc;
+#pragma unroll
+        for (int j = 0; j < ORD_KEEP; ++j) if (k == k_lo + j) { mine_e[j] = inc - c[u]; mine_c[j] = c[u]; }
+        const uint32_t bucket = 255u - min((c[u] + 7u) >> 3, 255u);
+        if (bucket != 255u) atomicAdd(k < k_lo ? &h_before[wv][bucket] : &h_rest[wv][bucket], 1u);
+        const uint32_t ne = (uint32_t)__popcll(__ballot(t < T && !tab.v[k / n_it].fused_alias && bucket == 255u));
+        empties_all += ne;
+        if (k < k_lo) empties_before += ne;
+      }
+    }
+    __syncthreads();
+    uint32_t* wtf = &L.wt[0][0];
+    const int per_view = n_it * ORD_WAVES;
+    for (int vi = wv; vi < tab.V; vi += ORD_WAVES) {
+      uint32_t carry = 0;
+      for (int e0 = 0; e0 < per_view; e0 += 64) {
+        const int e = e0 + lane;
+        const uint32_t x = e < per_view ? wtf[vi * per_view + e] : 0u;
+        const uint32_t inc = bin_wave_scan_incl(x);
+        if (e < per_view) wtf[vi * per_view + e] = carry + inc - x;
+        carry += (uint32_t)__builtin_amdgcn_readlane((int)inc, 63);
+      }
+      if (lane == 0 && carry > tab.v[vi].list_cap) L.overflow_s = 1u;
+    }
+    __syncthreads();
+    recount = L.overflow_s != 0u;
+    if (recount) {
+      for (int i = tid; i < ORD_WAVES * 256; i += 1024) { (&h_before[0][0])[i] = 0; (&h_rest[0][0])[i] = 0; }
+      empties_before = 0; empties_all = 0;
+      __syncthreads();
+    } else {
+#pragma unroll
+      for (int j = 0; j < ORD_KEEP; ++j)
+        if (k_lo + j < k_hi) {
+          const uint32_t cap = tab.v[(k_lo + j) / n_it].list_cap, s = L.wt[k_lo + j][wv] + mine_e[j];
+          const uint32_t a = min(s, cap), b = min(s + mine_c[j], cap);
+          mine[j] = b > a ? make_uint2(a, b) : make_uint2(0u, 0u);
+        }
+    }
+  }
+  for (int k0 = 0; recount && k0 < n_items; k0 += ORD_CHUNK) {
     uint2 r[ORD_CHUNK];
     bool live[ORD_CHUNK];
+    uint32_t c[ORD_CHUNK];
 #pragma unroll
     for (int u = 0; u < ORD_CHUNK; ++u) {
       const int k = k0 + u, t = (k % n_it) * 1024 + tid;
-      r[u] = make_uint2(0u, 0u);
+      r[u] = make_uint2(0u, 0u); c[u] = 0u;
       live[u] = k < n_items && t < T && !tab.v[k / n_it].fused_alias;
-      if (live[u]) r[u] = tab.v[k / n_it].ranges[t];
+      if constexpr (FROM_TOTALS) { if (live[u]) c[u] = tab.v[k / n_it].tile_rows[tot_off + t]; }
+      else if (live[u]) r[u] = tab.v[k / n_it].ranges[t];
+    }
+    if constexpr (FROM_TOTALS) {
+#pragma unroll
+      for (int u = 0; u < ORD_CHUNK; ++u)
+        if (k0 + u < n_items) {
+          r[u] = range_of(k0 + u, tab.v[(k0 + u) / n_it].list_cap, c[u]);
+#pragma unroll
+          for (int j = 0; j < ORD_KEEP; ++j) if (k0 + u == k_lo + j) mine[j] = r[u];
+        }
     }
 #pragma unroll
     for (int u = 0; u < ORD_CHUNK; ++u) {
@@ -486,11 +584,22 @@
   __syncthreads();
   for (int k0 = k_lo; k0 < k_hi; k0 += ORD_CHUNK) {
     uint2 r[ORD_CHUNK];
+    uint32_t c[ORD_CHUNK];
 #pragma unroll
     for (int u = 0; u < ORD_CHUNK; ++u) {
       const int k = k0 + u, t = (k % n_it) * 1024 + tid;
-      r[u] = make_uint2(0u, 0u);
-      if (k < k_hi && t < T && !tab.v[k / n_it].fused_alias) r[u] = tab.v[k / n_it].ranges[t];
+      r[u] = make_uint2(0u, 0u); c[u] = 0u;
+      if (!kept && k < k_hi && t < T && !tab.v[k / n_it].fused_alias) {
+        if constexpr (FROM_TOTALS) c[u] = tab.v[k / n_it].tile_rows[tot_off + t];
+        else r[u] = tab.v[k / n_it].ranges[t];
+      }
+    }
+    if constexpr (FROM_TOTALS) {
+#pragma unroll
+      for (int u = 0; u < ORD_CHUNK; ++u) {
+        if (kept) { if (u < ORD_KEEP) r[u] = mine[u]; }
+        else if (k0 + u < k_hi) r[u] = range_of(k0 + u, tab.v[(k0 + u) / n_it].list_cap, c[u]);
+      }
     }
 #pragma unroll
     for (int u = 0; u < ORD_CHUNK; ++u) {
@@ -498,7 +607,7 @@
       if (k < k_hi && t < T && !tab.v[k / n_it].fused_alias) {
         if (r[u].y <= r[u].x) {
           r[u] = make_uint2(0u, 0u);
-          if (!tab.v[k / n_it].shares_lists) tab.v[k / n_it].ranges[t] = r[u];
+          if (!FROM_TOTALS && !tab.v[k / n_it].shares_lists) tab.v[k / n_it].ranges[t] = r[u];
         }
         const uint32_t bucket = 255u - min((r[u].y - r[u].x + 7u) >> 3, 255u);
         uint32_t slot;
@@ -520,7 +629,7 @@
 
 __global__ __launch_bounds__(1024) void tile_order_kernel(GsrBinViews tab, int items_per_wg) {
   __shared__ TileOrderLds L;
-  tile_order_body(tab, items_per_wg, (int)blockIdx.x, L);
+  tile_order_body<false>(tab, items_per_wg, (int)blockIdx.x, L);
 }
 
 __global__ __launch_bounds__(BIN_THREADS) void bin_count_kernel(int P, GsrBinViews tab) {
@@ -632,157 +741,67 @@
   }
   if (nbig) __syncthreads();
   uint32_t* __restrict__ row = vw.tile_rows + (size_t)blockIdx.x * Ts;
-  for (int t = tid; t < Ts; t += BIN_THREADS) row[t] = t < T ? s_cnt[t] : 0u;
-  if (blockIdx.x == 0 && tid < 64) vw.block_hist[tid] = 0u;
-}
-
-__global__ __launch_bounds__(GSR_BLOCK) void bin_colprefix_kernel(GsrBinViews tab) {
-  const GsrBinView& vw = tab.v[blockIdx.y];
-  if (vw.shares_lists) return;
-  const int Ts = gsr_bin_stride(tab.T), rows = tab.rows, t = blockIdx.x * GSR_BLOCK + threadIdx.x;
-  if (t >= Ts) return;
-  uint32_t* __restrict__ m = vw.tile_rows;
-  uint32_t run = 0;
-  int r = 0;
-  for (; r + 8 <= rows; r += 8) {
-    uint32_t v[8];
-#pragma unroll
-    for (int u = 0; u < 8; ++u) v[u] = m[(size_t)(r + u) * Ts + t];
-#pragma unroll
-    for (int u = 0; u < 8; ++u) { m[(size_t)(r + u) * Ts + t] = run; run += v[u]; }
-  }
-  for (; r < rows; ++r) { const uint32_t v = m[(size_t)r * Ts + t]; m[(size_t)r * Ts + t] = run; run += v; }
-  m[(size_t)rows * Ts + t] = run;
-}
-
-__global__ __launch_bounds__(GSR_BLOCK) void bin_colprefix_scan_kernel(GsrBinViews tab) {
-  const GsrBinView& vw = tab.v[blockIdx.y];
-  if (vw.shares_lists) return;
-  __shared__ uint32_t s_w[GSR_BLOCK / 64];
-  __shared__ uint32_t s_base;
-  const int T = tab.T, Ts = gsr_bin_stride(T), rows = tab.rows, tid = threadIdx.x, lane = tid & 63, wv = tid >> 6;
-  const int t = blockIdx.x * GSR_BLOCK + tid;
-  uint32_t* __restrict__ m = vw.tile_rows;
-  uint32_t run = 0;
-  if (t < Ts) {
-    int r = 0;
-    for (; r + 8 <= rows; r += 8) {
-      uint32_t v[8];
-#pragma unroll
-      for (int u = 0; u < 8; ++u) v[u] = m[(size_t)(r + u) * Ts + t];
-#pragma unroll
-      for (int u = 0; u < 8; ++u) { m[(size_t)(r + u) * Ts + t] = run; run += v[u]; }
-    }
-    for (; r < rows; ++r) { const uint32_t v = m[(size_t)r * Ts + t]; m[(size_t)r * Ts + t] = run; run += v; }
-    m[(size_t)rows * Ts + t] = run;
-  }
-  uint32_t inc = run;
-#pragma unroll
-  for (int d = 1; d < 64; d <<= 1) {
-    const uint32_t o = __shfl_up(inc, d, 64);
-    if (lane >= d) inc += o;
-  }
-  if (lane == 63) s_w[wv] = inc;
-  __syncthreads();
-  uint32_t before = 0, total = 0;
-#pragma unroll
-  for (int w = 0; w < GSR_BLOCK / 64; ++w) { if (w < wv) before += s_w[w]; total += s_w[w]; }
-  uint32_t* __restrict__ words = vw.block_hist;
-  if (tid == 0) __hip_atomic_store(&words[blockIdx.x], 0x80000000u | total, __ATOMIC_RELAXED, __HIP_MEMORY_SCOPE_AGENT);
-  if (wv == 0) {
-    uint32_t mine = 0;
-    if (lane < (int)blockIdx.x) {
-      uint32_t w;
-      do { w = __hip_atomic_load(&words[lane], __ATOMIC_RELAXED, __HIP_MEMORY_SCOPE_AGENT); } while (!(w & 0x80000000u));
-      mine = w & 0x7fffffffu;
-    }
-#pragma unroll
-    for (int k = 32; k >= 1; k >>= 1) mine += __shfl_xor(mine, k, 64);
-    if (lane == 0) s_base = mine;
-  }
-  __syncthreads();
-  const uint32_t start = s_base + before + inc - run, cap = vw.D;
-  if (t < T) vw.ranges[t] = make_uint2(min(start, cap), min(start + run, cap));
-}
-
-__device__ __forceinline__ void bin_scan_view(const GsrBinViews& tab, const GsrBinView& vw, int prefixed, uint32_t* s_wave, uint32_t* s_carry) {
-  const int T = tab.T, Ts = gsr_bin_stride(T), rows = tab.rows, tid = threadIdx.x, lane = tid & 63, wv = tid >> 6;
-  uint32_t* __restrict__ m = vw.tile_rows;
-  const uint32_t cap = vw.D;
-  if (tid == 0) *s_carry = 0;
-  __syncthreads();
-  for (int q0 = 0; q0 < Ts / 4; q0 += BIN_THREADS) {
-    const int q = q0 + tid;
-    const bool live = q < Ts / 4;
-    uint4 tot = make_uint4(0u, 0u, 0u, 0u);
-    if (live) {
-      if (prefixed) tot = *reinterpret_cast<const uint4*>(m + (size_t)rows * Ts + 4 * q);
-      else {
-        for (int r0 = 0; r0 < rows; r0 += BIN_ROW_CHUNK) {
-          uint4 v[BIN_ROW_CHUNK];
-#pragma unroll
-          for (int r = 0; r < BIN_ROW_CHUNK; ++r)
-            v[r] = r0 + r < rows ? *reinterpret_cast<const uint4*>(m + (size_t)(r0 + r) * Ts + 4 * q) : make_uint4(0u, 0u, 0u, 0u);
-#pragma unroll
-          for (int r = 0; r < BIN_ROW_CHUNK; ++r)
-            if (r0 + r < rows) {
-              *reinterpret_cast<uint4*>(m + (size_t)(r0 + r) * Ts + 4 * q) = tot;
-              tot.x += v[r].x; tot.y += v[r].y; tot.z += v[r].z; tot.w += v[r].w;
-            }
-        }
-      }
-    }
-    const uint32_t mine = tot.x + tot.y + tot.z + tot.w;
-    uint32_t inc = mine;
-#pragma unroll
-    for (int d = 1; d < 64; d <<= 1) {
-      const uint32_t o = __shfl_up(inc, d, 64);
-      if (lane >= d) inc += o;
-    }
-    if (lane == 63) s_wave[wv] = inc;
-    __syncthreads();
-    uint32_t start = *s_carry + inc - mine;
-    for (int w = 0; w < wv; ++w) start += s_wave[w];
-    if (live) {
-      const uint32_t c[4] = {tot.x, tot.y, tot.z, tot.w};
-      uint32_t st_ = start;
-#pragma unroll
-      for (int k = 0; k < 4; ++k) {
-        if (4 * q + k < T) vw.ranges[4 * q + k] = make_uint2(min(st_, cap), min(st_ + c[k], cap));
-        st_ += c[k];
-      }
-    }
-    __syncthreads();
-    if (tid == BIN_THREADS - 1) *s_carry = start + mine;
-    __syncthreads();
-  }
-}
-
-__global__ __launch_bounds__(BIN_THREADS) void bin_scan_kernel(GsrBinViews tab, int prefixed) {
-  __shared__ uint32_t s_wave[BIN_THREADS / 64];
-  __shared__ uint32_t s_carry;
-  const GsrBinView& vw = tab.v[blockIdx.x];
-  if (vw.shares_lists) return;
-  bin_scan_view(tab, vw, prefixed, s_wave, &s_carry);
+  uint32_t* __restrict__ total = vw.tile_rows + (size_t)tab.rows * Ts;
+  uint32_t base[BIN_SCAN_MAX];
+#pragma unroll
+  for (int j = 0; j < BIN_SCAN_MAX; ++j) {
+    const int t = j * BIN_THREADS + tid;
+    const uint32_t cnt = t < T ? s_cnt[t] : 0u;
+    base[j] = cnt ? __hip_atomic_fetch_add(&total[t], cnt, __ATOMIC_RELAXED, __HIP_MEMORY_SCOPE_AGENT) : 0u;
+  }
+#pragma unroll
+  for (int j = 0; j < BIN_SCAN_MAX; ++j) { const int t = j * BIN_THREADS + tid; if (t < Ts) row[t] = base[j]; }
+}
+
+__device__ __forceinline__ void bin_scan_totals(uint32_t* s, int T, uint32_t cap, uint2* __restrict__ ranges, uint32_t* s_wave) {
+  const int tid = threadIdx.x, lane = tid & 63, wv = tid >> 6;
+  const int c = (T + BIN_THREADS - 1) / BIN_THREADS;
+  __syncthreads();
+  uint32_t v[BIN_SCAN_MAX], sum = 0;
+#pragma unroll
+  for (int k = 0; k < BIN_SCAN_MAX; ++k) {
+    const int t = tid * c + k;
+    v[k] = (k < c && t < T) ? s[t] : 0u;
+    sum += v[k];
+  }
+  const uint32_t inc = bin_wave_scan_incl(sum);
+  if (lane == 63) s_wave[wv] = inc;
+  __syncthreads();
+  const uint32_t winc = bin_wave_scan_incl(lane < BIN_THREADS / 64 ? s_wave[lane] : 0u);
+  const int wvu = __builtin_amdgcn_readfirstlane(wv);
+  uint32_t run = inc - sum + (wvu ? (uint32_t)__builtin_amdgcn_readlane((int)winc, wvu - 1) : 0u);
+#pragma unroll
+  for (int k = 0; k < BIN_SCAN_MAX; ++k) {
+    const int t = tid * c + k;
+    if (k < c && t < T) {
+      const uint32_t a = min(run, cap), b = min(run + v[k], cap);
+      s[t] = a;
+      if (ranges) ranges[t] = b > a ? make_uint2(a, b) : make_uint2(0u, 0u);
+      run += v[k];
+    }
+  }
+  __syncthreads();
 }
 
 __global__ __launch_bounds__(BIN_THREADS) void bin_emit_kernel(int P, GsrBinViews tab, int order_wgs, int items_per_wg) {
   extern __shared__ uint32_t s_cur[];
   if ((int)blockIdx.x >= tab.rows) {
     __shared__ TileOrderLds L;
-    if (blockIdx.y == 0) tile_order_body(tab, items_per_wg, (int)blockIdx.x - tab.rows, L);
+    if (blockIdx.y == 0) tile_order_body<true>(tab, items_per_wg, (int)blockIdx.x - tab.rows, L);
     return;
   }
   (void)order_wgs;
   __shared__ uint2 s_big[BIN_BIG_MAX];
   __shared__ uint64_t s_bigkey[BIN_BIG_MAX];
   __shared__ uint32_t s_nbig;
+  __shared__ uint32_t s_wave[BIN_THREADS / 64];
   const GsrBinView& vw = tab.v[blockIdx.y];
   const int T = tab.T, Ts = gsr_bin_stride(T), gx = tab.gx, tid = threadIdx.x, lane = tid & 63, wv = tid >> 6;
   const int g0 = (int)blockIdx.x * GSR_BIN_G;
   if (vw.shares_lists) return;
   const uint32_t cap = vw.D;
   const uint32_t* __restrict__ row = vw.tile_rows + (size_t)blockIdx.x * Ts;
+  const uint32_t* __restrict__ total = vw.tile_rows + (size_t)tab.rows * Ts;
   const uint32_t* __restrict__ cut = vw.depth_cut;
   const bool cut_l = cut && tab.cut_lds;
   const uint32_t* s_cut = s_cur + T;
@@ -807,7 +826,13 @@
     if (g < P) { rc[q] = vw.rect[g]; ek[q] = vw.ekey[g]; }
   }
   if (tid == 0) s_nbig = 0;
-  for (int t = tid; t < T; t += BIN_THREADS) s_cur[t] = vw.ranges[t].x + row[t];
+  uint32_t base[BIN_SCAN_MAX];
+#pragma unroll
+  for (int j = 0; j < BIN_SCAN_MAX; ++j) { const int t = j * BIN_THREADS + tid; base[j] = t < T ? row[t] : 0u; }
+  for (int t = tid; t < T; t += BIN_THREADS) s_cur[t] = total[t];
+  bin_scan_totals(s_cur, T, cap, blockIdx.x == 0 ? vw.ranges : nullptr, s_wave);
+#pragma unroll
+  for (int j = 0; j < BIN_SCAN_MAX; ++j) { const int t = j * BIN_THREADS + tid; if (t < T) s_cur[t] += base[j]; }
   __syncthreads();
   if (cut_l) {
     const int gyc = (T / gx + 3) >> 2;
@@ -1275,23 +1300,7 @@
       hipLaunchKernelGGL(bin_count_kernel, dim3(tab.rows, tab.V), dim3(BIN_THREADS), lds, st, P, tab);
     }
     GSR_HIP_CHECK(hipGetLastError());
-    const int prefixed = tab.rows > BIN_DIRECT_ROWS ? 1 : 0;
-    const int col_wgs = (gsr_bin_stride(tab.T) + GSR_BLOCK - 1) / GSR_BLOCK;
-    const bool chained = prefixed && col_wgs <= 64;
-    if (chained) {
-      GSR_PROF("bin_colprefix", st);
-      hipLaunchKernelGGL(bin_colprefix_scan_kernel, dim3(col_wgs, tab.V), dim3(GSR_BLOCK), 0, st, tab);
-    } else if (prefixed) {
-      GSR_PROF("bin_colprefix", st);
-      hipLaunchKernelGGL(bin_colprefix_kernel, dim3(col_wgs, tab.V), dim3(GSR_BLOCK), 0, st, tab);
-    }
-    GSR_HIP_CHECK(hipGetLastError());
     const int n_items = tab.V * ((tab.T + 1023) / 1024);
-    if (!chained) {
-      GSR_PROF("bin_scan", st);
-      hipLaunchKernelGGL(bin_scan_kernel, dim3(tab.V), dim3(BIN_THREADS), 0, st, tab, prefixed);
-    }
-    GSR_HIP_CHECK(hipGetLastError());
     int order_wgs = 0, per_wg = 1;
     {
       order_wgs = n_items < ORD_MAX_WG ? n_items : ORD_MAX_WG;
diff --git a/gs-dynamics_amd/csrc/gsr_common.h b/gs-dynamics_amd/csrc/gsr_common.h
--- a/gs-dynamics_amd/csrc/gsr_common.h
+++ b/gs-dynamics_amd/csrc/gsr_common.h
@@ -149,6 +149,7 @@
   uint2* block_hash;
   const float4* cmp_rec; const uint2* cmp_rect; const uint2* cmp_ekey; const uint32_t* cmp_tiles;
   uint8_t* used; uint32_t* tracked;
+  uint32_t* bin_totals; int bin_T;
   int skip;
 };
 struct GsrPreViews {
@@ -171,6 +172,7 @@
   const uint2* ekey;
   float4* rec_w;
   uint32_t* tile_rows;
+  uint32_t list_cap;
   const uint32_t* depth_cut;
 };
 struct GsrBinViews {
@@ -612,12 +614,6 @@
 }
 #define BIN_THREADS 1024
 #define BIN_PER_THREAD (GSR_BIN_G / BIN_THREADS)
-#ifndef BIN_DIRECT_ROWS
-#define BIN_DIRECT_ROWS 32
-#endif
-#ifndef BIN_ROW_CHUNK
-#define BIN_ROW_CHUNK 16
-#endif
 #define BIN_BIG_AREA 64
 #define BIN_BIG_MAX 1024
 
diff --git a/gs-dynamics_amd/csrc/gsr_preprocess_fwd_kernel.inc b/gs-dynamics_amd/csrc/gsr_preprocess_fwd_kernel.inc
--- a/gs-dynamics_amd/csrc/gsr_preprocess_fwd_kernel.inc
+++ b/gs-dynamics_amd/csrc/gsr_preprocess_fwd_kernel.inc
@@ -15,6 +15,8 @@
   uint32_t* __restrict__ block_sums = vw.block_sums;
   __shared__ uint32_t s_wave_sum[GSR_BLOCK / GSR_WAVE];
   const int i = blockIdx.x * GSR_BLOCK + threadIdx.x;
+  if (vw.bin_totals)
+    for (int t = i; t < vw.bin_T; t += (int)gridDim.x * GSR_BLOCK) vw.bin_totals[t] = 0u;
   __shared__ float4 s_rec[GSR_BLOCK / GSR_WAVE][256];
   const PreOut po = preprocess_gaussian<GSR_PFWD_AA>(tab, vw, i, P, s_rec[threadIdx.x >> 6], blockIdx.y == 0, W, H, gx, gy, mod, sh_degree, M, means3D, scales, rotations,
                                         opacities, colors_precomp, shs, cov3D_precomp, tight_lists);
```

Result: no change. 5633, median of 3 (+0.2%).
